# jmhb0/view_neti

Hardware: AMD Instinct MI355X
Metric: TI train steps/sec (SD-1.5 512^2 bs=4 per GPU) (higher is better)
Workload: dtype f16; 1 GPU; learnable_mode 0, sd15 shapes, 512x512 fp16, bs=4/GPU, grad_accum 1, full train step (VAE+16xCLIP+UNet fwd/bwd+AdamW); global_batch=4, parallelism=dp1, rccl_ranks=1, hipgraph=True

## Files before the change

### include/vneti.h

```cpp
#ifndef VNETI_H
#define VNETI_H
#include <stddef.h>
#include <stdint.h>

#ifdef __cplusplus
extern "C" {
#endif

#define VNETI_ABI_VERSION 1

int vneti_version(void);
int vneti_precision(void);
int vneti_last_error(char* buf, size_t n);

typedef struct vneti_gemm_desc {
  const void* A;
  const void* B;
  void* C;
  long long lda, ldb, ldc;
  int M, N, K;
  int batch;
  long long strideA, strideB, strideC;
  const float* bias;
  const void* rowadd;
  long long ld_rowadd;
  int rows_per_group;
  const void* resid;
  long long ldr;
  float alpha;
  int act;
  int out_f32;
  int conv_mode;
  int Hi, Wi, Ci, Ho, Wo, stride, pad_t, pad_l, ups;
  long long ldx;
  int tile_hint;
  void* workspace;
  long long workspace_bytes;
  int split_k;
  const void* gate_src;
  long long ld_gate;
  int gate_act;
  void* C2;
  long long ldc2;
  int act2;
  void* gn_sums;
  int gn_hw, gn_cpg, gn_groups, gn_slots;
  int geglu;
  int conv_korder;
} vneti_gemm_desc;

int vneti_gemm_f16(const vneti_gemm_desc* d, void* stream);
int vneti_gemm_select_tile(int M, int N, int batch);
int vneti_gemm_select_split(int M, int N, int K, int batch, int tile_hint, long long workspace_bytes);

int vneti_im2col3x3_small(const void* x, int x_is_f32, long long sb, long long sc, long long sy,
                          long long sx, void* out, int Bn, int C, int Hi, int Wi, int Ho, int Wo,
                          int stride, int pad_t, int pad_l, void* stream);

int vneti_conv3x3_in(const void* x, int x_is_f32, long long sb, long long sc, long long sy, long long sx,
                     const void* w_packed, const float* bias, void* out, long long ldo, int Bn, int C, int H, int W,
                     int Co, void* gn_sums, int gn_groups, int gn_slots, void* stream);

int vneti_transpose_f16(const void* in, long long ld_in, long long stride_in, void* out,
                        long long ld_out, long long stride_out, int rows, int cols, int batch,
                        void* stream);
#define VNETI_TRANSPOSE_MAX 4
typedef struct vneti_transpose_desc {
  const void* inp;
  long long ld_in, stride_in;
  void* out;
  long long ld_out, stride_out;
  int rows, cols, batch, _pad;
} vneti_transpose_desc;
int vneti_transpose_f16_multi(const vneti_transpose_desc* descs, int n, void* stream);

long long vneti_groupnorm_ws_floats(int Bn, int HW, int C, int G);
int vneti_groupnorm_fwd(const void* x, long long ldx, void* y, long long ldy, const float* gamma,
                        const float* beta, float* mean, float* rstd, float* ws, int Bn, int HW,
                        int C, int G, float eps, int silu, void* stream);
int vneti_groupnorm_fwd_sums(const void* x, long long ldx, void* y, long long ldy, const float* gamma,
                             const float* beta, const void* sums, int slots, float* mean, float* rstd,
                             int Bn, int HW, int C, int G, float eps, int silu, void* stream);
int vneti_groupnorm_fwd_2l(const void* x, long long ldx, void* y, long long ldy, const float* gamma,
                           const float* beta, void* sums, int slots, float* mean, float* rstd, int Bn, int HW,
                           int C, int G, float eps, int silu, void* stream);
int vneti_groupnorm_bwd_2l(const void* dy, long long lddy, const void* x, long long ldx, const float* gamma,
                           const float* beta, const float* mean, const float* rstd, void* dx, long long lddx,
                           const void* dx_accum, long long ldacc, void* sums, int slots, float* ws, int Bn,
                           int HW, int C, int G, int silu, void* stream);
int vneti_groupnorm_bwd(const void* dy, long long lddy, const void* x, long long ldx,
                        const float* gamma, const float* beta, const float* mean,
                        const float* rstd, void* dx, long long lddx, const void* dx_accum,
                        long long ldacc, float* ws, int Bn, int HW, int C, int G, int silu,
                        void* stream);

int vneti_layernorm_fwd(const void* x, int x_is_f32, long long ldx, void* y, long long ldy,
                        const float* gamma, const float* beta, float* mean, float* rstd, int rows,
                        int C, float eps, void* stream);
int vneti_layernorm_bwd(const void* dy, int dy_is_f32, long long lddy, const void* x,
                        int x_is_f32, long long ldx, const float* gamma, const float* mean,
                        const float* rstd, void* dx, int dx_is_f32, long long lddx,
                        const void* dx_accum, long long ldacc, void* dx_f16_copy, long long ldcopy,
                        int rows, int C, void* stream);

int vneti_attn_fwd(const void* Q, long long ldq, const void* K, long long ldk, const void* V,
                   long long ldv, void* O, long long ldo, float* lse, int Bn, int H, int Nq,
                   int Nk, int D, float scale, int causal, void* stream);
int vneti_attn_bwd_delta(const void* dO, long long lddo, const void* O, long long ldo,
                         float* delta, int Bn, int H, int Nq, int D, void* stream);
int vneti_attn_bwd_dq(const void* Q, long long ldq, const void* K, long long ldk, const void* V,
                      long long ldv, const void* dO, long long lddo, const float* lse, float* delta,
                      const void* O, long long ldo, void* dQ, long long lddq, int Bn, int H, int Nq,
                      int Nk, int D, float scale, int causal, void* stream);
int vneti_attn_bwd_dkv(const void* Q, long long ldq, const void* K, long long ldk, const void* V,
                       long long ldv, const void* dO, long long lddo, const float* lse,
                       const float* delta, void* dK, long long lddk, void* dV, long long lddv,
                       int Bn, int H, int Nq, int Nk, int D, float scale, int causal, float* ws,
                       long long ws_floats, void* stream);
int vneti_attn_bwd_small(const void* Q, long long ldq, const void* K, long long ldk, const void* V, long long ldv,
                         const void* dO, long long lddo, const void* O, long long ldo, const float* lse, void* dQ,
                         long long lddq, void* dK, long long lddk, void* dV, long long lddv, int Bn, int H, int N, int D,
                         float scale, int causal, void* stream);
int vneti_softmax_rows_f16(void* x, long long ld, int rows, int cols, void* stream);

int vneti_add_f16(const void* a, long long lda, const void* b, long long ldb, void* out,
                  long long ldo, int rows, int cols, void* stream);
int vneti_geglu_fwd(const void* p, long long ldp, void* out, long long ldo, int rows, int C4,
                    void* stream);
int vneti_geglu_bwd(const void* dy, long long lddy, const void* p, long long ldp, void* dp,
                    long long lddp, int rows, int C4, void* stream);
int vneti_act_fwd_f16(const void* x, void* y, long long n, int act, void* stream);
int vneti_act_bwd_f16(const void* dy, const void* x, void* dx, long long n, int act, void* stream);
int vneti_timestep_embedding(const void* t, void* out, int Bn, int dim, void* stream);
int vneti_sum2x2_f16(const void* in, long long ldi, void* out, long long ldo, int Bn, int H, int W,
                     int C, void* stream);
int vneti_rng_fill_normal(void* out_f32, long long n, const void* state, unsigned stream_id,
                          void* stream);
int vneti_rng_fill_randint(void* out_i64, int n, int high, const void* state, unsigned stream_id,
                           void* stream);
int vneti_rng_advance(void* state, void* stream);
int vneti_nested_dropout_mask(float* mask, int nl, int Bn, int hidden, float prob, const void* state,
                              unsigned stream_id, void* stream);
int vneti_sample_add_noise(const void* moments, long long ldm, const float* eps,
                           const float* noise, const void* timesteps_i64,
                           const float* alphas_cumprod, float scaling, int v_prediction,
                           float* latents, float* noisy, float* target, int Bn, int Lc, int HW,
                           void* stream);
int vneti_latent_sample(const void* moments, long long ldm, const float* eps, float scaling, float* latents, int Bn,
                        int Lc, int HW, void* stream);
int vneti_add_noise(const float* latents, const float* noise, const void* timesteps_i64, const float* alphas_cumprod,
                    int v_prediction, float* noisy, float* target, int Bn, int Lc, int HW, void* stream);
int vneti_cfg_sampler_step(const void* pred, long long ldp, float* x, float* m_prev, float* x_in, int Bn,
                           int Lc, int HW, float guidance, float alpha_t, float sigma_t, float cx,
                           float c0, float c1, int v_prediction, void* stream);
int vneti_cfg_sampler_step_table(const void* pred, long long ldp, float* x, float* m_prev, float* x_in,
                                 int Bn, int Lc, int HW, float guidance, const float* coef_table,
                                 const int* step, int v_prediction, void* stream);
int vneti_cfg_sampler_step_noise(const void* pred, long long ldp, float* x, float* m_prev, float* x_in,
                                 const float* noise, int Bn, int Lc, int HW, float guidance, float alpha_t,
                                 float sigma_t, float cx, float c0, float c1, float cn, int v_prediction, void* stream);
int vneti_cfg_sampler_step_noise_table(const void* pred, long long ldp, float* x, float* m_prev, float* x_in, int Bn,
                                       int Lc, int HW, float guidance, const float* coef_table,
                                       const float* noise_table, const int* step, int v_prediction, void* stream);
int vneti_table_fill_i64(void* dst_i64, int n, const void* table_i64, const int* step, void* stream);
int vneti_counter_advance(int* counter, void* stream);
int vneti_conv1x1_nchw_f32(const float* x, const float* W, const float* bias, float* out, int Bn, int Ci,
                           int Co, int HW, float in_scale, void* stream);
int vneti_image_postprocess(const void* img, long long ldi, float* out, long long n_pix, int channels,
                            void* stream);
int vneti_mse_loss_grad(const void* pred, long long ldp, const float* target, void* dpred,
                        long long lddp, float* loss_sum, const float* loss_scale, int Bn, int Lc,
                        int HW, void* stream);
#define VNETI_OPT_CHECK 1
#define VNETI_OPT_APPLY 2
#define VNETI_OPT_FINISH 4
#define VNETI_OPT_ALL 7
int vneti_adamw_flat(float* p, const float* g, float* m, float* v, long long n, const float* hyper,
                     float* scaler, int* step, int growth_interval, int phases, void* stream);
int vneti_adamw_segments(float* p, const float* g, float* m, float* v, long long seg_len, int n_seg,
                         int* seg_step, const int* active, int n_active, const float* hyper,
                         float* scaler, int* step, int growth_interval, int phases, void* stream);

long long vneti_mapper_num_params(int enc_dim, int hidden, int D, int has_bypass);
long long vneti_mapper_save_floats(int R, int enc_dim, int hidden);
long long vneti_mapper_rowgrad_floats(int R, int hidden, int D, int has_bypass);
int vneti_mapper_fwd(const float* params, const int* slot, long long slot_stride, const float* data,
                     int nfeat, const float* w_enc,
                     const float* hidden_mask, float norm_scale, float* word, float* bypass,
                     float* save, int R, int enc_dim, int hidden, int D, int has_bypass, const float* enc_in,
                     void* stream);
int vneti_mapper_fwd_slots(const float* params, const int* slots, long long slot_stride, int Bn, const float* data,
                           int nfeat, const float* w_enc, const float* hidden_mask, float norm_scale, float* word,
                           float* bypass, float* save, int R, int enc_dim, int hidden, int D, int has_bypass,
                           const float* enc_in, void* stream);
int vneti_mapper_bwd(const float* params, const int* slot, long long slot_stride,
                     const float* hidden_mask, float norm_scale,
                     const float* word, const float* dword_src, const int* dword_rows,
                     long long ld_src, const float* dbypass, const float* save, float* rowgrads,
                     float* grads, int accumulate, int R, int enc_dim, int hidden, int D,
                     int has_bypass, float* denc, void* stream);
long long vneti_mapper_legacy_input_params(int enc_dim, int pe_dim);
int vneti_mapper_legacy_input_fwd(const float* params_in, const int* slot, long long slot_stride,
                                  const void* timesteps_i64, const float* w_pe, float* enc_out, int nl, int Bn,
                                  int enc_dim, int pe_dim, void* stream);
int vneti_mapper_legacy_input_fwd_slots(const float* params_in, const int* slots, long long slot_stride,
                                        const void* timesteps_i64, const float* w_pe, float* enc_out, int nl, int Bn,
                                        int enc_dim, int pe_dim, void* stream);
int vneti_mapper_legacy_input_bwd(const void* timesteps_i64, const float* w_pe, const float* denc, float* grads_in,
                                  const int* slot, long long slot_stride, int accumulate, int nl, int Bn, int enc_dim,
                                  int pe_dim, void* stream);
int vneti_text_embed(const float* tok_emb, const float* pos_emb, const void* ids_i64,
                     const int* pos_obj, const float* word_obj, const int* pos_view,
                     const float* word_view, float* X, int nl, int Bn, int L, int D, void* stream);
int vneti_text_final_fwd(const float* last, const float* gamma, const float* beta, float eps,
                         const int* pos_obj, const float* bypass_obj, float alpha_obj,
                         int unconstrained_obj, const int* pos_view, const float* bypass_view,
                         float alpha_view, int unconstrained_view, float* norm_terms, void* ctx_k,
                         void* ctx_v, int nl, int Bn, int L, int D, void* stream);
int vneti_text_final_bwd(const float* last, const float* gamma, float eps, const int* pos_obj,
                         const float* bypass_obj, float alpha_obj, int unconstrained_obj,
                         float* dbypass_obj, const int* pos_view, const float* bypass_view,
                         float alpha_view, int unconstrained_view, float* dbypass_view,
                         const float* norm_terms, const void* dctx_k, const void* dctx_v, float* dX,
                         int nl, int Bn, int L, int D, void* stream);
int vneti_mapper_inputs(const void* timesteps_i64, const float* view_params, int nv, float* data,
                        int nl, int Bn, void* stream);
int vneti_cast_f32_f16(const float* x, void* y, long long n, void* stream);


int vneti_img_resample_ksize(int in_size, int out_size, int filter);
int vneti_img_resample_coeffs(int in_size, int out_size, int filter, int* bounds, int* kk, void* stream);
int vneti_img_resample_pass(const void* in, int in_w, void* out, int out_h, int out_w, const int* bounds,
                            const int* kk, int ksize, int horizontal, void* stream);
int vneti_img_crop(const void* in, int in_w, int top, int left, void* out, int h, int w, int flip, void* stream);
int vneti_img_enhance(void* img, int h, int w, int mode, float alpha, void* scratch8, void* stream);
int vneti_img_hue(void* img, int h, int w, int shift, void* stream);
int vneti_img_blur5(const void* in, void* out, float* tmp, int h, int w, const float* k5_host, void* stream);
int vneti_img_affine_nearest(const void* in, void* out, int h, int w, const int* a6_host, int fill, void* stream);
int vneti_img_to_f32_chw(const void* img, float* out, int h, int w, void* stream);

int vneti_comm_unique_id(void* id128);
int vneti_comm_init(const void* id128, int rank, int world, void** comm);
// ... 20 lines not shown
```

### view_neti_amd/csrc/gemm8.hip

```cpp
#include <type_traits>

#include "common.h"
#include "gemm_args.h"

namespace {

constexpr int BM = 256, NT = 512;
constexpr int HALF_BYTES = 128 * 128;
constexpr int GN_IMG = 5;

#define VN_WAIT_VM(n) asm volatile("s_waitcnt vmcnt(" #n ")" ::: "memory")
#define VN_WAIT_LGKM0() asm volatile("s_waitcnt lgkmcnt(0)" ::: "memory")

template <int BN, int EPI, bool CONV, bool HALO = false>
__global__ __launch_bounds__(NT) void gemm8_kernel(GemmArgs g) {
  static_assert(BN == 256 || BN == 128, "tile width");
  static_assert(!HALO || (BN == 128 && CONV), "the halo-patch loop exists for the 256x128 convolution tile");
  constexpr int PATCH_STRIDE = 41 * 1024;
  constexpr bool H42 = HALO && BN == 128;
  constexpr int NJB = BN / 128;
  constexpr int HB_BYTES = (BN / 2) * 128;
  constexpr int HB_DMA = BN / 128;
  constexpr int NBUF = BN == 256 ? 2 : 3;
  constexpr int BUF_BYTES = 2 * HALF_BYTES + 2 * HB_BYTES;
  constexpr int CS_LD = BN + 8;
  constexpr int CS_BYTES = BM * CS_LD * 2;
  constexpr int LOOP_BYTES = HALO ? 2 * PATCH_STRIDE + 3 * 2 * HB_BYTES : NBUF * BUF_BYTES;
  constexpr int LDS_BYTES = CS_BYTES > LOOP_BYTES ? CS_BYTES : LOOP_BYTES;
  constexpr int GN_NG = BN / 4 + 2;
  const half_t* const e_gate = EPI == 2 ? g.gate_src : nullptr;
  half_t* const e_C2 = EPI == 2 ? g.C2 : nullptr;
  const int e_geglu = EPI == 2 ? g.geglu : 0;
  const int e_act = EPI == 2 ? g.act : 0;
  float* const e_gn_sums = EPI >= 1 ? g.gn_sums : nullptr;
  const half_t* const e_rowadd = EPI >= 1 ? g.rowadd : nullptr;
  const int e_conv = CONV ? g.conv_mode : 0;
  constexpr int GN_BYTES = EPI == 0 ? 0 : GN_IMG * GN_NG * 4 * 8;
  __shared__ __attribute__((aligned(16))) char smem[LDS_BYTES + GN_BYTES];

  const int tid = threadIdx.x;
  const int lane = tid & 63;
  const int wave = __builtin_amdgcn_readfirstlane(tid >> 6);
  const int wr = wave >> 2, wc = wave & 3;

  int nblk = g.tiles_m * g.tiles_n;
  int bid = blockIdx.x;
  {
    int q = nblk >> 3, r = nblk & 7, xcd = bid & 7, idx = bid >> 3;
    bid = (xcd < r ? xcd * (q + 1) : r * (q + 1) + (xcd - r) * q) + idx;
  }
  const int tile_m = bid / g.tiles_n;
  const int tile_n = bid - tile_m * g.tiles_n;
  const int m0 = tile_m * BM;
  const int n0 = tile_n * BN;
  const int bz = blockIdx.y;
  const int kz = blockIdx.z;
  int hb = 0, hty = 0, htx = 0, row0 = m0;
  if constexpr (HALO) {
    const int tpr = g.Wo >> 4, tpi = (g.Ho >> 4) * tpr;
    hb = tile_m / tpi;
    const int rem = tile_m - hb * tpi;
    hty = rem / tpr;
    htx = rem - hty * tpr;
    row0 = (hb * g.Ho + hty * 16) * g.Wo + htx * 16;
  }
  auto rowmem = [&](const int r) { return HALO ? row0 + (r >> 4) * g.Wo + (r & 15) : m0 + r; };

  const half_t* Ab = g.A + (long long)bz * g.strideA;
  const half_t* Bb = g.B + (long long)bz * g.strideB;
  const __amdgpu_buffer_rsrc_t rsA = vn_make_rsrc(Ab, g.a_bytes);
  const __amdgpu_buffer_rsrc_t rsB = vn_make_rsrc(Bb, g.b_bytes);

  const int lrow = tid >> 3;
  const int gchunk = (tid & 7) ^ ((lrow >> 1) & 7);
  const float rcp_hw = CONV ? 1.0f / (float)(g.Ho * g.Wo) : 0.f, rcp_wo = CONV ? 1.0f / (float)g.Wo : 0.f;
  int a_base[4];
  uint32_t a_mask[4];
#pragma unroll
  for (int r = 0; r < (HALO ? 0 : 4); ++r) {
    const int m = m0 + (r >> 1) * 128 + (r & 1) * 64 + lrow;
    const bool ok = m < g.M;
    if constexpr (!CONV) {
      a_base[r] = (int)((long long)m * g.lda * 2) + gchunk * 16;
      a_mask[r] = ok ? 1u : 0u;
    } else {
      const int hw = g.Ho * g.Wo;
      int b = (int)((float)m * rcp_hw);
      int rem = m - b * hw;
      if (rem < 0) { b -= 1; rem += hw; } else if (rem >= hw) { b += 1; rem -= hw; }
      int oy = (int)((float)rem * rcp_wo);
      int ox = rem - oy * g.Wo;
      if (ox < 0) { oy -= 1; ox += g.Wo; } else if (ox >= g.Wo) { oy += 1; ox -= g.Wo; }
      const int py = e_conv == 1 ? oy * g.stride - g.pad_t : oy + g.pad_t;
      const int px = e_conv == 1 ? ox * g.stride - g.pad_l : ox + g.pad_l;
      a_base[r] = ((b * g.Hi + py) * g.Wi + px) * g.ldx2 + gchunk * 16;
      const int sgn = e_conv == 1 ? 1 : -1;
      uint32_t colbits = 0, mask = 0;
#pragma unroll
      for (int d = 0; d < 3; ++d) colbits |= ((unsigned)(px + sgn * d) < (unsigned)g.Wi ? 1u : 0u) << d;
#pragma unroll
      for (int d = 0; d < 3; ++d) mask |= ((unsigned)(py + sgn * d) < (unsigned)g.Hi ? colbits : 0u) << (3 * d);
      a_mask[r] = ok ? mask : 0u;
    }
  }
  uint32_t b_base[4];
#pragma unroll
  for (int r = 0; r < 4; ++r) {
    const int n = n0 + (r >> 1) * (BN / 2) + (r & 1) * 64 + lrow;
    b_base[r] = (n < g.N) ? (uint32_t)((long long)n * g.ldb * 2) + gchunk * 16 : VN_OOB;
  }

  const int nk_total = g.K / 64;
  const int kt_begin = kz * g.kt_per_split;
  const int kt_end = min(nk_total, kt_begin + g.kt_per_split);
  const int T = kt_end - kt_begin;

  int a_kt[2] = {kt_begin, kt_begin}, b_kt[2] = {kt_begin, kt_begin};
  int a_tap[2], a_ci0[2];
  {
    int tap = 0, ci0 = 0;
    if constexpr (CONV) {
      if (g.korder) {
        ci0 = (kt_begin / 9) * 64;
        tap = kt_begin - (kt_begin / 9) * 9;
      } else {
        tap = (kt_begin * 64) / g.Ci;
        ci0 = kt_begin * 64 - tap * g.Ci;
      }
    }
    a_tap[0] = a_tap[1] = tap;
    a_ci0[0] = a_ci0[1] = ci0;
  }
  const int tap_step = (e_conv == 2 ? -1 : 1) * g.ldx2;
  uint32_t nxt[4];
  auto prepA = [&](const int h) {
    const bool live = a_kt[h] < kt_end;
    int soff;
    uint32_t tapbit;
    if constexpr (!CONV) {
      soff = a_kt[h] * 128;
      tapbit = live ? 1u : 0u;
    } else {
      const int tap = a_tap[h];
      const int dy = (tap * 11) >> 5;
      const int dx = tap - 3 * dy;
      soff = (dy * g.Wi + dx) * tap_step + a_ci0[h] * 2;
      tapbit = live ? (1u << tap) : 0u;
      if (g.korder) {
        a_tap[h] += 1;
        if (a_tap[h] == 9) {
          a_tap[h] = 0;
          a_ci0[h] += 64;
        }
      } else {
        a_ci0[h] += 64;
        if (a_ci0[h] == g.Ci) {
          a_ci0[h] = 0;
          a_tap[h] += 1;
        }
      }
    }
#pragma unroll
    for (int j = 0; j < 2; ++j) {
      nxt[j] = (a_mask[2 * h + j] & tapbit) ? (uint32_t)(a_base[2 * h + j] + soff) : VN_OOB;
    }
    a_kt[h] += 1;
  };
  auto prepB = [&](const int h) {
    const bool live = b_kt[h] < kt_end;
    const uint32_t soff = (uint32_t)b_kt[h] * 128u, dead = live ? 0u : VN_OOB;
    if constexpr (BN == 256) {
#pragma unroll
      for (int j = 0; j < 2; ++j) nxt[j] = (b_base[2 * h + j] + soff) | dead;
    } else {
      nxt[2 + h] = (b_base[2 * h] + soff) | dead;
    }
    b_kt[h] += 1;
  };
  auto issueA = [&](const int h, const int buf) {
    char* dst = smem + buf * BUF_BYTES + h * HALF_BYTES + wave * 1024;
#pragma unroll
    for (int j = 0; j < 2; ++j)
      dma16(rsA, dst + j * 8192, nxt[j]);
  };
  auto issueB = [&](const int h, const int buf) {
    char* dst = smem + buf * BUF_BYTES + 2 * HALF_BYTES + h * HB_BYTES + wave * 1024;
    if constexpr (BN == 256) {
#pragma unroll
// ... 254 lines not shown
    issueB(0, 1);
    prepA(0);
    issueA(0, 1);
    prepB(1);
    issueB(1, 1);
    prepA(1);
    VN_WAIT_VM(10);
    __builtin_amdgcn_s_barrier();
    __builtin_amdgcn_sched_barrier(0);
    readB0(0);
    VN_WAIT_LGKM0();
    __builtin_amdgcn_sched_barrier(0);
    if (wr == 1) __builtin_amdgcn_s_barrier();
    __builtin_amdgcn_sched_barrier(0);

    int cur = 0;
    for (int t = 0; t < T; ++t) {
      readA(0);
      issueA(1, cur ^ 1);
      VN_PHASE_SYNC();
      VN_MMA(0, 0, bf0, prepB(0));
      VN_PHASE_END();
      readB1();
      issueB(0, cur);
      VN_PHASE_SYNC();
      VN_MMA(0, 1, bf1, prepA(0));
      VN_PHASE_END();
      readA(1);
      issueA(0, cur);
      VN_PHASE_SYNC();
      VN_MMA(1, 0, bf0, prepB(1));
      VN_PHASE_END();
      readB0(BUF_BYTES);
      issueB(1, cur);
      VN_PHASE_SYNC();
      VN_MMA(1, 1, bf1, prepA(1));
      VN_PHASE_END();
      cur ^= 1;
#pragma unroll
      for (int s = 0; s < 2; ++s) {
        rdA[s] ^= BUF_BYTES;
        rdB[s] ^= BUF_BYTES;
      }
    }
  } else {
#pragma unroll
    for (int t0 = 0; t0 < 2; ++t0) {
      prepA(0);
      prepB(0);
      prepB(1);
      issueA(0, t0);
      issueB(0, t0);
      issueB(1, t0);
      prepA(1);
      issueA(1, t0);
    }
    prepA(0);
    prepB(0);
    prepB(1);
    VN_WAIT_VM(8);
    __builtin_amdgcn_s_barrier();
    __builtin_amdgcn_sched_barrier(0);
    if (wr == 1) __builtin_amdgcn_s_barrier();
    __builtin_amdgcn_sched_barrier(0);
    int stg = 2;
    for (int t = 0; t < T; ++t) {
      readB0(0);
      readB1();
      readA(0);
      issueA(0, stg);
      issueB(0, stg);
      issueB(1, stg);
      VN_SYNC(10);
      VN_MMA2(0, prepA(1));
      VN_PHASE_END();
      readA(1);
      issueA(1, stg);
      VN_SYNC(8);
      VN_MMA2(1, (prepA(0), prepB(0), prepB(1)));
      VN_PHASE_END();
      stg = stg == 2 ? 0 : stg + 1;
#pragma unroll
      for (int s = 0; s < 2; ++s) {
        rdA[s] = rdA[s] >= 2 * BUF_BYTES ? rdA[s] - 2 * BUF_BYTES : rdA[s] + BUF_BYTES;
        rdB[s] = rdB[s] >= 2 * BUF_BYTES ? rdB[s] - 2 * BUF_BYTES : rdB[s] + BUF_BYTES;
      }
    }
#undef VN_MMA2
#undef VN_SYNC
  }
  if (wr == 0) __builtin_amdgcn_s_barrier();
  asm volatile("s_waitcnt vmcnt(0) lgkmcnt(0)" ::: "memory");
  __syncthreads();
#undef VN_MMA
#undef VN_PHASE_SYNC
#undef VN_PHASE_END

  if (g.ksplit > 1) {
    float* ws = g.ws + ((long long)(kz * g.batch + bz) * g.M) * g.N;
    const __amdgpu_buffer_rsrc_t rsW = vn_make_rsrc(ws, 0x7fffffffu);
#pragma unroll
    for (int h = 0; h < 2; ++h)
#pragma unroll
      for (int j = 0; j < 2; ++j)
#pragma unroll
        for (int i = 0; i < 4; ++i)
#pragma unroll
          for (int jb = 0; jb < NJB; ++jb) {
            const int m = rowmem(acc_row(h, i));
            const int n = n0 + acc_col(h, j, jb);
            if (m < g.M && n < g.N) {
              float* p = ws + (long long)m * g.N + n;
              if (n + 4 <= g.N && (g.N & 3) == 0) {
                vn_st16_wt(rsW, (uint32_t)(((long long)m * g.N + n) * 4), acc[h][j][i][jb]);
              } else {
                for (int e = 0; e < 4 && n + e < g.N; ++e) p[e] = acc[h][j][i][jb][e];
              }
            }
          }
    return;
  }

  if (e_gn_sums && !(HALO && g.gn_hw == g.Ho * g.Wo)) {
    vn_u64* gacc = reinterpret_cast<vn_u64*>(smem + LDS_BYTES);
    for (int i = tid; i < GN_IMG * GN_NG * 4; i += NT) gacc[i] = 0;
  }
  {
    const int nsw = ((frow >> 3) & 1) << 2;
#pragma unroll
    for (int h = 0; h < 2; ++h)
#pragma unroll
      for (int i = 0; i < 4; ++i)
#pragma unroll
        for (int j = 0; j < 2; ++j)
#pragma unroll
          for (int jb = 0; jb < NJB; ++jb) {
            const int ml = acc_row(h, i);
            const int nl = acc_col(h, j, jb) ^ nsw;
            half4 o;
#pragma unroll
            for (int e = 0; e < 4; ++e)
              o[e] = (half_t)apply_act(acc[h][j][i][jb][e] * g.alpha + bv[H42 ? h : 0][j][jb][e], e_act);
            *reinterpret_cast<half4*>(smem + ((size_t)ml * CS_LD + nl) * 2) = o;
          }
  }
  __syncthreads();

  half_t* Cb = reinterpret_cast<half_t*>(g.C) + (long long)bz * g.strideC;
  const __amdgpu_buffer_rsrc_t rsC = vn_make_rsrc(Cb, 0x7fffffffu);
  const __amdgpu_buffer_rsrc_t rsC2 = vn_make_rsrc(e_C2, e_C2 ? 0x7fffffffu : 0u);
  const half_t* Rb = reinterpret_cast<const half_t*>(g.resid);
  if (Rb) Rb += (long long)bz * g.strideC;
  constexpr int CPR = BN / 8;
  constexpr int U = EPI == 2 ? 2 : (EPI == 1 ? 4 : (BN == 256 ? 8 : 4));
  static_assert(NT % CPR == 0 && CPR <= 32 && (BM * CPR) % NT == 0, "a thread keeps one 8-column chunk over all its rows");
  vn_u64* gacc = reinterpret_cast<vn_u64*>(smem + LDS_BYTES);
  const bool gn = e_gn_sums != nullptr;
  const float rcp_gnhw = gn ? 1.0f / (float)g.gn_hw : 0.f, rcp_rpg = e_rowadd ? 1.0f / (float)g.rows_per_group : 0.f;
  const int gn_img0 = gn ? row0 / g.gn_hw : 0, gn_g0t = gn ? n0 / g.gn_cpg : 0;
  const int c = (tid % CPR) * 8;
  const int n = n0 + c;
  const int gn_glo = gn ? n / g.gn_cpg : 0;
  const int gn_split = gn ? (gn_glo + 1) * g.gn_cpg - n : 8;
  int gn_img = -1;
  float s_lo = 0.f, q_lo = 0.f, s_hi = 0.f, q_hi = 0.f;
  auto gn_flush = [&]() {
    const int iref = __builtin_amdgcn_readfirstlane(gn_img);
    const bool uni = __all(gn_img == iref) && iref >= 0;
    if (uni) {
#pragma unroll
      for (int off = 32; off >= CPR; off >>= 1) {
        s_lo += __shfl_xor(s_lo, off);
        q_lo += __shfl_xor(q_lo, off);
        s_hi += __shfl_xor(s_hi, off);
        q_hi += __shfl_xor(q_hi, off);
      }
    }
    if (gn_img >= 0 && (!uni || lane < CPR)) {
      vn_u64* a = gacc + ((gn_img - gn_img0) * GN_NG + (gn_glo - gn_g0t)) * 4;
      vn_fx_add2(a, s_lo, q_lo);
      if (gn_split < 8) vn_fx_add2(a + 4, s_hi, q_hi);
    }
    s_lo = q_lo = s_hi = q_hi = 0.f;
  };
  const bool full_chunk = n + 8 <= g.N;
  const bool swap_halves = ((tid / CPR) >> 3) & 1;
  const __amdgpu_buffer_rsrc_t rsR = vn_make_rsrc(Rb, Rb ? 0x7fffffffu : 0u);
  const __amdgpu_buffer_rsrc_t rsRA = vn_make_rsrc(e_rowadd, e_rowadd ? 0x7fffffffu : 0u);
  const __amdgpu_buffer_rsrc_t rsG = vn_make_rsrc(e_gate, e_gate ? 0x7fffffffu : 0u);
  const int r_first = tid / CPR;
  constexpr int RPP = NT / CPR;
  const bool gn_one = HALO && gn && g.gn_hw == g.Ho * g.Wo;
  const bool ra_one = HALO && EPI >= 1 && e_rowadd && g.rows_per_group == g.Ho * g.Wo;
  half8 av_tile = half8{0, 0, 0, 0, 0, 0, 0, 0};
  if (ra_one) av_tile = as_half8(vn_buf_load16(rsRA, full_chunk ? (uint32_t)(((long long)hb * g.ld_rowadd + n) * 2) : VN_OOB));
  if (gn_one) gn_img = hb;
  for (int it0 = 0; it0 < BM / RPP; it0 += U) {
    half8 cv[U], rv[U], av[U], gv[U], gv2[U];
#pragma unroll
    for (int u = 0; u < U; ++u) {
      const int r = r_first + RPP * (it0 + u);
      const int m = rowmem(r);
      const bool ok = m < g.M && full_chunk;
      u32x4 t = *reinterpret_cast<const u32x4*>(smem + ((size_t)r * CS_LD + c) * 2);
      if (swap_halves) t = u32x4{t[2], t[3], t[0], t[1]};
      cv[u] = as_half8(t);
      if (Rb) rv[u] = as_half8(vn_buf_load16(rsR, ok ? (uint32_t)(((long long)m * g.ldr + n) * 2) : VN_OOB));
      if (EPI >= 1) {
        if (ra_one) {
          av[u] = av_tile;
        } else if (e_rowadd) {
          int grp = (int)((float)m * rcp_rpg);
          const int rem = m - grp * g.rows_per_group;
          grp += rem >= g.rows_per_group ? 1 : (rem < 0 ? -1 : 0);
          av[u] = as_half8(vn_buf_load16(rsRA, ok ? (uint32_t)(((long long)grp * g.ld_rowadd + n) * 2) : VN_OOB));
        }
      }
      if (EPI == 2 && e_gate) {
        const long long go = (long long)m * g.ld_gate + (e_geglu == 2 ? 2 * n : n);
        gv[u] = as_half8(vn_buf_load16_once(rsG, ok ? (uint32_t)(go * 2) : VN_OOB));
        gv2[u] = as_half8(vn_buf_load16_once(rsG, (ok && e_geglu == 2) ? (uint32_t)(go * 2 + 16) : VN_OOB));
      }
    }
#pragma unroll
    for (int u = 0; u < U; ++u) {
      const int r = r_first + RPP * (it0 + u);
      const int m = rowmem(r);
      const bool valid = m < g.M && n < g.N;
      if (gn && !gn_one) {
        int img = gn_img;
        if (valid) {
          img = (int)((float)m * rcp_gnhw);
          const int rem = m - img * g.gn_hw;
          img += rem >= g.gn_hw ? 1 : (rem < 0 ? -1 : 0);
        }
        if (__any(img != gn_img)) {
          gn_flush();
          gn_img = img;
        }
      }
      if (!valid) continue;
      half8 v = cv[u];
      if (full_chunk) {
        if (EPI >= 1 && e_rowadd) {
          v = vn_add8(v, av[u]);
        }
        if (Rb) {
          v = vn_add8(v, rv[u]);
        }
        if (e_geglu == 2) {
#pragma unroll
          for (int c2 = 0; c2 < 2; ++c2) {
            const half8 pre = c2 == 0 ? gv[u] : gv2[u];
            half8 o;
#pragma unroll
            for (int e = 0; e < 4; ++e) {
              const float d = (float)v[4 * c2 + e], hh = (float)pre[e], gg = (float)pre[4 + e];
              float cdf, xpdf;
              vn_gelu_parts(gg, cdf, xpdf);
              o[e] = (half_t)(d * gg * cdf);
              o[4 + e] = (half_t)(d * hh * (cdf + xpdf));
            }
            vn_st16_wt(rsC, (uint32_t)(((long long)m * g.ldc + 2 * n + 8 * c2) * 2), o);
          }
          continue;
        }
        if (e_gate) {
#pragma unroll
          for (int e = 0; e < 8; ++e) v[e] = (half_t)((float)v[e] * act_grad((float)gv[u][e], g.gate_act));
        }
        if (e_geglu == 1 || (e_C2 && e_geglu == 0)) vn_st16_wt_saved(rsC, (uint32_t)(((long long)m * g.ldc + n) * 2), v);
        else vn_st16_wt(rsC, (uint32_t)(((long long)m * g.ldc + n) * 2), v);
        if (e_geglu == 1) {
          half4 o2;
#pragma unroll
          for (int e = 0; e < 4; ++e) o2[e] = (half_t)((float)v[e] * vn_gelu_erf((float)v[4 + e]));
          *reinterpret_cast<half4*>(e_C2 + (long long)m * g.ldc2 + (n >> 1)) = o2;
        }
        if (gn) {
          {
            const half2v one2 = {(half_t)1.f, (half_t)1.f};
#pragma unroll
            for (int e = 0; e < 8; e += 2) {
              const half2v p2 = {v[e], v[e + 1]};
              if (e < gn_split) {
                s_lo = VN_FDOT2(p2, one2, s_lo);
                q_lo = VN_FDOT2(p2, p2, q_lo);
              } else {
                s_hi = VN_FDOT2(p2, one2, s_hi);
                q_hi = VN_FDOT2(p2, p2, q_hi);
              }
            }
          }
        }
        if (e_C2 && e_geglu == 0) {
          half8 o2;
#pragma unroll
          for (int e = 0; e < 8; ++e) o2[e] = (half_t)apply_act((float)v[e], g.act2);
          vn_st16_wt(rsC2, (uint32_t)(((long long)m * g.ldc2 + n) * 2), o2);
        }
      } else {
        const half_t* radd = e_rowadd ? e_rowadd + (long long)(m / g.rows_per_group) * g.ld_rowadd + n : nullptr;
        for (int e = 0; e < 8 && n + e < g.N; ++e) {
          float x = (float)v[e];
          if (radd) x = (float)(half_t)(x + (float)radd[e]);
          if (Rb) x = (float)(half_t)(x + (float)Rb[(long long)m * g.ldr + n + e]);
          if (e_gate) x = (float)(half_t)(x * act_grad((float)e_gate[(long long)m * g.ld_gate + n + e], g.gate_act));
          Cb[(long long)m * g.ldc + n + e] = (half_t)x;
          if (e_C2) e_C2[(long long)m * g.ldc2 + n + e] = (half_t)apply_act((float)(half_t)x, g.act2);
          if (gn) {
            const float xs = (float)(half_t)x;
            if (e < gn_split) {
              s_lo += xs;
              q_lo += xs * xs;
            } else {
              s_hi += xs;
              q_hi += xs * xs;
            }
          }
        }
      }
    }
  }
  if (gn_one) {
    float v4[4] = {s_lo, q_lo, s_hi, q_hi};
#pragma unroll
    for (int k = 0; k < 4; ++k) {
      v4[k] += __shfl_xor(v4[k], 32);
      v4[k] += __shfl_xor(v4[k], 16);
    }
    static_assert(CPR == 16 || !HALO, "the halo tile is 128 columns wide");
    float* tab = reinterpret_cast<float*>(smem + LDS_BYTES);
    if (lane < 16) *reinterpret_cast<f32x4*>(tab + (wave * 16 + lane) * 4) = f32x4{v4[0], v4[1], v4[2], v4[3]};
    __syncthreads();
    if (tid < 32) {
      const int col = tid >> 1, half = tid & 1;
      float sv = 0.f, qv = 0.f;
#pragma unroll
      for (int w8 = 0; w8 < 8; ++w8) {
        sv += tab[(w8 * 16 + col) * 4 + 2 * half];
        qv += tab[(w8 * 16 + col) * 4 + 2 * half + 1];
      }
      const int nc = n0 + col * 8;
      const int glo = nc / g.gn_cpg;
      const int split = (glo + 1) * g.gn_cpg - nc;
      if (nc < g.N && (half == 0 || split < 8)) {
        const int slot = tile_m % g.gn_slots;
        vn_u64* dst = reinterpret_cast<vn_u64*>(e_gn_sums) + (((long long)hb * g.gn_slots + slot) * g.gn_G + glo + half) * 4;
        vn_fx_add2(dst, sv, qv);
      }
    }
  } else if (gn) {
    gn_flush();
    __syncthreads();
    const int slot = tile_m % g.gn_slots;
    for (int i = tid; i < GN_IMG * GN_NG; i += NT) {
      const vn_u64* src = gacc + 4 * i;
      if ((src[0] | src[1] | src[2] | src[3]) == 0) continue;
      const int img = gn_img0 + i / GN_NG, grp = gn_g0t + i % GN_NG;
      vn_u64* dst = reinterpret_cast<vn_u64*>(e_gn_sums) + (((long long)img * g.gn_slots + slot) * g.gn_G + grp) * 4;
#pragma unroll
      for (int w = 0; w < 4; ++w) atomicAdd(dst + w, src[w]);
    }
  }
}

inline int epilogue_level8(const GemmArgs& g) {
  if (g.gate_src || g.C2 || g.geglu || g.act) return 2;
  return (g.gn_sums || g.rowadd) ? 1 : 0;
}

}

int vneti_launch_gemm8(void* gemm_args, int bn, int halo, hipStream_t st) {
  GemmArgs& g = *reinterpret_cast<GemmArgs*>(gemm_args);
  if (g.out_f32 || (g.conv_mode && (g.ups || (g.conv_mode == 2 && g.stride == 2))) ||
      (g.M >= (1 << 24) && (g.conv_mode || g.rowadd || g.gn_sums)))
    return VNETI_EUNSUP;
  if (halo && (bn != 128 || g.conv_mode < 1 || g.conv_mode > 2 || g.stride != 1 || g.pad_t != 1 || g.pad_l != 1 || g.Hi != g.Ho ||
               g.Wi != g.Wo || (g.Ho & 15) || (g.Wo & 15) || (g.Ci & 63) || g.K != 9 * g.Ci || !g.korder ||
               g.batch != 1 || g.M != (g.M / (g.Ho * g.Wo)) * g.Ho * g.Wo))
    return VNETI_EUNSUP;
  if (halo && g.ksplit > 1) {
    const int nchunk = g.Ci / 64, cps = cdiv(nchunk, g.ksplit);
    g.kt_per_split = 9 * cps;
    g.ksplit = cdiv(nchunk, cps);
  }
  g.tiles_m = cdiv(g.M, BM);
  g.tiles_n = cdiv(g.N, bn);
  const dim3 grid(g.tiles_m * g.tiles_n, g.batch, g.ksplit), block(NT);
  const int epi = epilogue_level8(g);
#define VN_GO(E, C)                                                                        \
  do {                                                                                     \
    if (bn == 256) hipLaunchKernelGGL((gemm8_kernel<256, E, C>), grid, block, 0, st, g);   \
    else hipLaunchKernelGGL((gemm8_kernel<128, E, C>), grid, block, 0, st, g);             \
  } while (0)
#define VN_GO_HALO(E) hipLaunchKernelGGL((gemm8_kernel<128, E, true, true>), grid, block, 0, st, g)
  if (halo) {
    if (epi == 2) VN_GO_HALO(2); else if (epi == 1) VN_GO_HALO(1); else VN_GO_HALO(0);
  } else if (g.conv_mode) {
    if (epi == 2) VN_GO(2, true); else if (epi == 1) VN_GO(1, true); else VN_GO(0, true);
  } else {
    if (epi == 2) VN_GO(2, false); else if (epi == 1) VN_GO(1, false); else VN_GO(0, false);
  }
#undef VN_GO
#undef VN_GO_HALO
  return vneti_check_launch("gemm8_kernel");
}
```

### view_neti_amd/csrc/gemm_args.h

```cpp
#pragma once
#include "common.h"

namespace {

struct GemmArgs {
  const half_t* A;
  const half_t* B;
  void* C;
  const float* bias;
  const half_t* rowadd;
  const void* resid;
  float* ws;
  const half_t* gate_src;
  half_t* C2;
  long long ld_gate, ldc2;
  int gate_act, act2;
  float* gn_sums;
  int gn_hw, gn_cpg, gn_G, gn_slots;
  int geglu;
  long long lda, ldb, ldc, ld_rowadd, ldr;
  long long strideA, strideB, strideC;
  uint32_t a_bytes, b_bytes;
  int M, N, K;
  int rows_per_group;
  float alpha;
  int act;
  int out_f32;
  int batch, ksplit, kt_per_split;
  int conv_mode;
  int Hi, Wi, Ci, Ho, Wo, stride, pad_t, pad_l, ups;
  int ldx2;
  int korder;
  int tiles_m, tiles_n;
};

__device__ __forceinline__ float apply_act(float v, int act) {
  switch (act) {
    case 1: return vn_silu(v);
    case 2: return vn_quick_gelu(v);
    case 3: return vn_gelu_erf(v);
    default: return v;
  }
}
__device__ __forceinline__ float act_grad(float f, int act) {
  if (act == 2) {
    float s = vn_sigmoid(1.702f * f);
    return s * (1.f + 1.702f * f * (1.f - s));
  } else if (act == 3) {
    return vn_gelu_erf_grad(f);
  }
  float s = vn_sigmoid(f);
  return s * (1.f + f * (1.f - s));
}

__device__ __forceinline__ int lds_off(int row, int chunk) {
  return row * 128 + ((chunk ^ ((row >> 1) & 7)) << 4);
}

__device__ __forceinline__ void dma16(__amdgpu_buffer_rsrc_t rs, char* lds_dst, uint32_t off) {
#if defined(__HIP_DEVICE_COMPILE__)
  __builtin_amdgcn_raw_ptr_buffer_load_lds(rs, (__attribute__((address_space(3))) void*)lds_dst, 16, off, 0, 0, 0);
#else
  (void)rs; (void)lds_dst; (void)off;
#endif
}

}

int vneti_launch_gemm8(void* gemm_args, int bn, int halo, hipStream_t st);
```

### view_neti_amd/csrc/gemm_conv.hip

```cpp
#include "common.h"
#include "gemm_args.h"
#include "../../include/vneti.h"

namespace {

template <int BM, int BN, int WM, int WN, bool F32OUT, bool DMA, int NSTG = 2, int EPI = 2, bool CONV = true>
__global__ __launch_bounds__((BM / WM) * (BN / WN) * 64) void gemm_kernel(
    const half_t* pA, const half_t* pB, uint32_t p_a_bytes, uint32_t p_b_bytes, int p_lda, int p_ldb, int pM, int pN, int pK,
    int p_tiles_m, int p_tiles_n, int p_split_conv , const GemmArgs gfull) {
  GemmArgs g = gfull;
  g.A = pA;
  g.B = pB;
  g.a_bytes = p_a_bytes;
  g.b_bytes = p_b_bytes;
  g.lda = p_lda;
  g.ldb = p_ldb;
  g.M = pM;
  g.N = pN;
  g.K = pK;
  g.tiles_m = p_tiles_m;
  g.tiles_n = p_tiles_n;
  g.kt_per_split = p_split_conv & 0xffff;
  g.ksplit = (p_split_conv >> 16) & 0xff;
  g.conv_mode = p_split_conv >> 24;
  static_assert(NSTG == 2 || ((NSTG == 3 || NSTG == 4) && DMA), "the LDS rings are LDS-DMA only");
  const half_t* const e_gate = EPI == 2 ? g.gate_src : nullptr;
  half_t* const e_C2 = EPI == 2 ? g.C2 : nullptr;
  const int e_geglu = EPI == 2 ? g.geglu : 0;
  const int e_act = EPI == 2 ? g.act : 0;
  float* const e_gn_sums = EPI >= 1 ? g.gn_sums : nullptr;
  const half_t* const e_rowadd = EPI >= 1 ? g.rowadd : nullptr;
  const int e_conv = CONV ? g.conv_mode : 0;
  constexpr int NWM = BM / WM, NWN = BN / WN;
  constexpr int NT = NWM * NWN * 64;
  constexpr int RSTEP = NT / 8;
  constexpr int A_IT = BM / RSTEP, B_IT = BN / RSTEP;
  constexpr int STAGE_BYTES = (BM + BN) * 128;
  constexpr int CS_LD = F32OUT ? (BN + 4) : (BN + 8);
  constexpr int CS_BYTES = BM * CS_LD * (F32OUT ? 4 : 2);
  constexpr int LDS_BYTES = (NSTG * STAGE_BYTES > CS_BYTES) ? NSTG * STAGE_BYTES : CS_BYTES;
  constexpr int GN_IMG = 5, GN_NG = BN / 4 + 2;
  constexpr int GN_BYTES = (F32OUT || EPI == 0) ? 0 : GN_IMG * GN_NG * 4 * 8;
  __shared__ __attribute__((aligned(16))) char smem[LDS_BYTES + GN_BYTES];

  const int tid = threadIdx.x;
  const int lane = tid & 63;
  const int wave = __builtin_amdgcn_readfirstlane(tid >> 6);
  const int wm0 = (wave / NWN) * WM;
  const int wn0 = (wave % NWN) * WN;

  int nblk = g.tiles_m * g.tiles_n;
  int bid = blockIdx.x;
  {
    int q = nblk >> 3, r = nblk & 7, xcd = bid & 7, idx = bid >> 3;
    bid = (xcd < r ? xcd * (q + 1) : r * (q + 1) + (xcd - r) * q) + idx;
  }
  const int tile_m = bid / g.tiles_n;
  const int tile_n = bid - tile_m * g.tiles_n;
  const int m0 = tile_m * BM;
  const int n0 = tile_n * BN;
  const int bz = blockIdx.y;
  const int kz = blockIdx.z;

  const half_t* Ab = g.A + (long long)bz * g.strideA;
  const half_t* Bb = g.B + (long long)bz * g.strideB;
  __amdgpu_buffer_rsrc_t rsA = vn_make_rsrc(Ab, g.a_bytes);
  __amdgpu_buffer_rsrc_t rsB = vn_make_rsrc(Bb, g.b_bytes);

  const int lrow = tid >> 3;
  const int gchunk = DMA ? ((tid & 7) ^ ((lrow >> 1) & 7)) : (tid & 7);

  const float rcp_hw = CONV ? __builtin_amdgcn_rcpf((float)(g.Ho * g.Wo)) : 0.f, rcp_wo = CONV ? __builtin_amdgcn_rcpf((float)g.Wo) : 0.f;
  int a_off[A_IT];
  int a_py[A_IT], a_px[A_IT], a_bh[A_IT];
#pragma unroll
  for (int i = 0; i < A_IT; ++i) {
    int m = m0 + lrow + RSTEP * i;
    bool ok = m < g.M;
    if (e_conv == 0) {
      a_off[i] = ok ? (int)((long long)m * g.lda * 2) + gchunk * 16 : -1;
      a_py[i] = a_px[i] = a_bh[i] = 0;
    } else {
      int rem, ox;
      const int b = vn_divmod(m, g.Ho * g.Wo, rcp_hw, rem);
      const int oy = vn_divmod(rem, g.Wo, rcp_wo, ox);
      a_bh[i] = ok ? b * g.Hi : -1;
      if (e_conv == 1) {
        a_py[i] = oy * g.stride - g.pad_t;
        a_px[i] = ox * g.stride - g.pad_l;
      } else {
        a_py[i] = oy + g.pad_t;
        a_px[i] = ox + g.pad_l;
      }
      a_off[i] = ((b * g.Hi + a_py[i]) * g.Wi + a_px[i]) * g.ldx2 + gchunk * 16;
    }
  }
  int b_off[B_IT];
#pragma unroll
  for (int i = 0; i < B_IT; ++i) {
    int n = n0 + lrow + RSTEP * i;
    b_off[i] = (n < g.N) ? (int)((long long)n * g.ldb * 2) + gchunk * 16 : -1;
  }

  u32x4 ra[DMA ? 1 : A_IT], rb[DMA ? 1 : B_IT];

  auto a_offset = [&](int i, int k0, int dy, int dx, int tapoff) -> uint32_t {
    if (e_conv == 0) return a_off[i] < 0 ? VN_OOB : (uint32_t)(a_off[i] + k0 * 2);
    bool ok = a_bh[i] >= 0;
    if (e_conv == 1 && !g.ups) {
      int iy = a_py[i] + dy, ix = a_px[i] + dx;
      ok = ok && (unsigned)iy < (unsigned)g.Hi && (unsigned)ix < (unsigned)g.Wi;
      return ok ? (uint32_t)(a_off[i] + tapoff) : VN_OOB;
    }
    int iy, ix;
    if (e_conv == 1) {
      iy = a_py[i] + dy;
      ix = a_px[i] + dx;
      ok = ok && (unsigned)iy < (unsigned)(2 * g.Hi) && (unsigned)ix < (unsigned)(2 * g.Wi);
      iy >>= 1;
      ix >>= 1;
    } else {
      int ty = a_py[i] - dy, tx = a_px[i] - dx;
      ok = ok && ty >= 0 && tx >= 0;
      if (g.stride == 2) {
        ok = ok && ((ty | tx) & 1) == 0;
        ty >>= 1;
        tx >>= 1;
      }
      iy = ty;
      ix = tx;
      ok = ok && iy < g.Hi && ix < g.Wi;
    }
    return ok ? (uint32_t)(((a_bh[i] + iy) * g.Wi + ix) * g.ldx2 + tapoff) : VN_OOB;
  };

  uint32_t a_cur[A_IT], b_cur[B_IT];
#pragma unroll
  for (int i = 0; i < B_IT; ++i) b_cur[i] = b_off[i] < 0 ? VN_OOB : (uint32_t)b_off[i];

  auto issue = [&](int kt, int stage, bool first) {
    const int k0 = kt * 64;
    bool recompute = first;
    int dy = 0, dx = 0, tapoff = 0;
    if (e_conv != 0) {
      int tap, ci0;
      if (g.korder) {
        const int chunk = kt / 9;
        tap = kt - chunk * 9;
        ci0 = chunk << 6;
        recompute = true;
      } else {
        tap = k0 / g.Ci;
        ci0 = k0 - tap * g.Ci;
        recompute = recompute || ci0 == 0;
      }
      if (recompute) {
        dy = tap / 3;
        dx = tap - dy * 3;
        tapoff = (e_conv == 1 && !g.ups) ? ((dy * g.Wi + dx) * g.ldx2 + ci0 * 2) : (ci0 * 2 + gchunk * 16);
      }
    }
    if (recompute) {
#pragma unroll
      for (int i = 0; i < A_IT; ++i) a_cur[i] = a_offset(i, k0, dy, dx, tapoff);
      if (first) {
#pragma unroll
        for (int i = 0; i < B_IT; ++i) b_cur[i] += (uint32_t)k0 * 2;
      }
    }
    if constexpr (DMA) {
      char* As = smem + stage * STAGE_BYTES;
      char* Bs = As + BM * 128;
#pragma unroll
      for (int i = 0; i < A_IT; ++i) dma16(rsA, As + (wave * 8 + RSTEP * i) * 128, a_cur[i]);
#pragma unroll
      for (int i = 0; i < B_IT; ++i) dma16(rsB, Bs + (wave * 8 + RSTEP * i) * 128, b_cur[i]);
    } else {
#pragma unroll
      for (int i = 0; i < A_IT; ++i) ra[i] = vn_buf_load16(rsA, a_cur[i]);
#pragma unroll
      for (int i = 0; i < B_IT; ++i) rb[i] = vn_buf_load16(rsB, b_cur[i]);
    }
#pragma unroll
    for (int i = 0; i < A_IT; ++i) a_cur[i] += 128;
// ... 73 lines not shown
    for (int kt = kt_begin; kt < kt_end; ++kt) {
      const int st_next = st == 2 ? 0 : st + 1;
      const int st_new = st_next == 2 ? 0 : st_next + 1;
      if (kt + 2 < kt_end) issue(kt + 2, st_new, false);
      load_frags(1, st, 1);
      mma(0);
      if (kt + 2 < kt_end) asm volatile("s_waitcnt vmcnt(%0) lgkmcnt(0)" ::"n"(PER) : "memory");
      else asm volatile("s_waitcnt vmcnt(0) lgkmcnt(0)" ::: "memory");
      __builtin_amdgcn_s_barrier();
      if (kt + 1 < kt_end) load_frags(0, st_next, 0);
      mma(1);
      st = st_next;
    }
    __syncthreads();
  } else if constexpr (NSTG == 4) {
    constexpr int PER = A_IT + B_IT;
    auto wait_landed = [&](int later) {
      if (later >= 2) asm volatile("s_waitcnt vmcnt(%0) lgkmcnt(0)" ::"n"(2 * PER) : "memory");
      else if (later == 1) asm volatile("s_waitcnt vmcnt(%0) lgkmcnt(0)" ::"n"(PER) : "memory");
      else asm volatile("s_waitcnt vmcnt(0) lgkmcnt(0)" ::: "memory");
    };
    issue(kt_begin, 0, true);
    if (kt_begin + 1 < kt_end) issue(kt_begin + 1, 1, false);
    if (kt_begin + 2 < kt_end) issue(kt_begin + 2, 2, false);
    wait_landed(kt_end - kt_begin - 1);
    __builtin_amdgcn_s_barrier();
    load_frags(0, 0, 0);
    int st = 0;
    for (int kt = kt_begin; kt < kt_end; ++kt) {
      const int st_next = (st + 1) & 3;
      if (kt + 3 < kt_end) issue(kt + 3, (st + 3) & 3, false);
      load_frags(1, st, 1);
      mma(0);
      wait_landed(kt_end - kt - 2);
      __builtin_amdgcn_s_barrier();
      if (kt + 1 < kt_end) load_frags(0, st_next, 0);
      mma(1);
      st = st_next;
    }
    __syncthreads();
  } else {
    issue(kt_begin, 0, true);
    store_lds(0);
    if constexpr (DMA) asm volatile("s_waitcnt vmcnt(0)" ::: "memory");
    __syncthreads();

    for (int kt = kt_begin; kt < kt_end; ++kt) {
      const int cur = (kt - kt_begin) & 1;
      if (kt + 1 < kt_end) issue(kt + 1, cur ^ 1, false);
      load_frags(0, cur, 0);
      load_frags(1, cur, 1);
      mma(0);
      mma(1);
      if (kt + 1 < kt_end) store_lds(cur ^ 1);
      if constexpr (DMA) asm volatile("s_waitcnt vmcnt(0)" ::: "memory");
      __syncthreads();
    }
  }

  if (g.ksplit > 1) {
    float* ws = g.ws + ((long long)(kz * g.batch + bz) * g.M) * g.N;
    const __amdgpu_buffer_rsrc_t rsW = vn_make_rsrc(ws, 0x7fffffffu);
#pragma unroll
    for (int i = 0; i < MI16; ++i)
#pragma unroll
      for (int j = 0; j < NI16; ++j) {
        const int m = m0 + wm0 + i * 16 + frow;
        const int n = n0 + wn0 + j * 16 + 4 * fq;
        if (m < g.M && n < g.N) {
          float* p = ws + (long long)m * g.N + n;
          if (n + 4 <= g.N && (g.N & 3) == 0) {
            vn_st16_wt(rsW, (uint32_t)(((long long)m * g.N + n) * 4), acc[i][j]);
          } else {
            for (int e = 0; e < 4 && n + e < g.N; ++e) p[e] = acc[i][j][e];
          }
        }
      }
    return;
  }

  if constexpr (!F32OUT) {
    if (e_gn_sums) {
      vn_u64* gacc = reinterpret_cast<vn_u64*>(smem + LDS_BYTES);
      for (int i = tid; i < GN_IMG * GN_NG * 4; i += NT) gacc[i] = 0;
    }
  }
  if constexpr (!BIAS_EARLY) load_bias();
#pragma unroll
  for (int i = 0; i < MI16; ++i) {
#pragma unroll
    for (int j = 0; j < NI16; ++j) {
      const int ml = wm0 + i * 16 + frow;
      const int nl = wn0 + j * 16 + 4 * fq;
      float v[4];
#pragma unroll
      for (int e = 0; e < 4; ++e) {
        float x = acc[i][j][e] * g.alpha + bv[j][e];
        v[e] = apply_act(x, e_act);
      }
      if constexpr (F32OUT) {
        f32x4 o = {v[0], v[1], v[2], v[3]};
        *reinterpret_cast<f32x4*>(smem + ((size_t)ml * CS_LD + nl) * 4) = o;
      } else {
        half4 o = {(half_t)v[0], (half_t)v[1], (half_t)v[2], (half_t)v[3]};
        *reinterpret_cast<half4*>(smem + ((size_t)ml * CS_LD + nl) * 2) = o;
      }
    }
  }
  __syncthreads();

  if constexpr (F32OUT) {
    float* Cb = reinterpret_cast<float*>(g.C) + (long long)bz * g.strideC;
    const __amdgpu_buffer_rsrc_t rsC = vn_make_rsrc(Cb, 0x7fffffffu);
    const float* Rb = reinterpret_cast<const float*>(g.resid);
    if (Rb) Rb += (long long)bz * g.strideC;
    constexpr int CPR = BN / 4;
    for (int idx = tid; idx < BM * CPR; idx += NT) {
      int r = idx / CPR, c = (idx - r * CPR) * 4;
      int m = m0 + r, n = n0 + c;
      if (m >= g.M || n >= g.N) continue;
      f32x4 v = *reinterpret_cast<const f32x4*>(smem + ((size_t)r * CS_LD + c) * 4);
      if (n + 4 <= g.N) {
        if (Rb) {
          f32x4 rr = *reinterpret_cast<const f32x4*>(Rb + (long long)m * g.ldr + n);
          v += rr;
        }
        vn_st16_wt(rsC, (uint32_t)(((long long)m * g.ldc + n) * 4), v);
      } else {
        for (int e = 0; e < 4 && n + e < g.N; ++e) {
          float x = v[e];
          if (Rb) x += Rb[(long long)m * g.ldr + n + e];
          Cb[(long long)m * g.ldc + n + e] = x;
        }
      }
    }
  } else {
    half_t* Cb = reinterpret_cast<half_t*>(g.C) + (long long)bz * g.strideC;
    const __amdgpu_buffer_rsrc_t rsC = vn_make_rsrc(Cb, 0x7fffffffu);
    const __amdgpu_buffer_rsrc_t rsC2 = vn_make_rsrc(e_C2, e_C2 ? 0x7fffffffu : 0u);
    const half_t* Rb = reinterpret_cast<const half_t*>(g.resid);
    if (Rb) Rb += (long long)bz * g.strideC;
    constexpr int CPR = BN / 8;
    static_assert(NT % CPR == 0 && CPR <= 32 && (BM * CPR) % NT == 0, "a thread keeps one 8-column chunk over all its rows");
    vn_u64* gacc = reinterpret_cast<vn_u64*>(smem + LDS_BYTES);
    const bool gn = e_gn_sums != nullptr;
    const float rcp_gnhw = gn ? __builtin_amdgcn_rcpf((float)g.gn_hw) : 0.f;
    const float rcp_rpg = e_rowadd ? __builtin_amdgcn_rcpf((float)g.rows_per_group) : 0.f;
    const int gn_img0 = gn ? m0 / g.gn_hw : 0, gn_g0t = gn ? n0 / g.gn_cpg : 0;
    const int gn_c = n0 + (tid % CPR) * 8;
    const int gn_glo = gn ? gn_c / g.gn_cpg : 0;
    const int gn_split = gn ? (gn_glo + 1) * g.gn_cpg - gn_c : 8;
    int gn_img = -1;
    float s_lo = 0.f, q_lo = 0.f, s_hi = 0.f, q_hi = 0.f;
    auto gn_flush = [&]() {
      const int iref = __builtin_amdgcn_readfirstlane(gn_img);
      const bool uni = __all(gn_img == iref) && iref >= 0;
      if (uni) {
#pragma unroll
        for (int off = 32; off >= CPR; off >>= 1) {
          s_lo += __shfl_xor(s_lo, off);
          q_lo += __shfl_xor(q_lo, off);
          s_hi += __shfl_xor(s_hi, off);
          q_hi += __shfl_xor(q_hi, off);
        }
      }
      if (gn_img >= 0 && (!uni || lane < CPR)) {
        vn_u64* a = gacc + ((gn_img - gn_img0) * GN_NG + (gn_glo - gn_g0t)) * 4;
        vn_fx_add2(a, s_lo, q_lo);
        if (gn_split < 8) vn_fx_add2(a + 4, s_hi, q_hi);
      }
      s_lo = q_lo = s_hi = q_hi = 0.f;
    };
    for (int idx = tid; idx < BM * CPR; idx += NT) {
      int r = idx / CPR, c = (idx - r * CPR) * 8;
      int m = m0 + r, n = n0 + c;
      const bool valid = m < g.M && n < g.N;
      if (gn) {
        int gn_rem;
        const int img = valid ? vn_divmod(m, g.gn_hw, rcp_gnhw, gn_rem) : gn_img;
        if (__any(img != gn_img)) {
          gn_flush();
          gn_img = img;
        }
      }
      if (!valid) continue;
      half8 v = as_half8(*reinterpret_cast<const u32x4*>(smem + ((size_t)r * CS_LD + c) * 2));
      int ra_rem;
      const half_t* radd = e_rowadd ? e_rowadd + (long long)vn_divmod(m, g.rows_per_group, rcp_rpg, ra_rem) * g.ld_rowadd + n : nullptr;
      if (n + 8 <= g.N) {
        if (radd) {
          half8 t = *reinterpret_cast<const half8*>(radd);
          v = vn_add8(v, t);
        }
        if (Rb) {
          half8 rr = *reinterpret_cast<const half8*>(Rb + (long long)m * g.ldr + n);
          v = vn_add8(v, rr);
        }
        if (e_geglu == 2) {
          const half_t* pp = e_gate + (long long)m * g.ld_gate + 2 * n;
#pragma unroll
          for (int c2 = 0; c2 < 2; ++c2) {
            const half8 pre = *reinterpret_cast<const half8*>(pp + 8 * c2);
            half8 o;
#pragma unroll
            for (int e = 0; e < 4; ++e) {
              const float d = (float)v[4 * c2 + e], hh = (float)pre[e], gg = (float)pre[4 + e];
              float cdf, xpdf;
              vn_gelu_parts(gg, cdf, xpdf);
              o[e] = (half_t)(d * gg * cdf);
              o[4 + e] = (half_t)(d * hh * (cdf + xpdf));
            }
            vn_st16_wt(rsC, (uint32_t)(((long long)m * g.ldc + 2 * n + 8 * c2) * 2), o);
          }
          continue;
        }
        if (e_gate) {
          half8 pre = *reinterpret_cast<const half8*>(e_gate + (long long)m * g.ld_gate + n);
#pragma unroll
          for (int e = 0; e < 8; ++e) v[e] = (half_t)((float)v[e] * act_grad((float)pre[e], g.gate_act));
        }
        if (e_geglu == 1 || (e_C2 && e_geglu == 0)) vn_st16_wt_saved(rsC, (uint32_t)(((long long)m * g.ldc + n) * 2), v);
        else vn_st16_wt(rsC, (uint32_t)(((long long)m * g.ldc + n) * 2), v);
        if (e_geglu == 1) {
          half4 o2;
#pragma unroll
          for (int e = 0; e < 4; ++e) o2[e] = (half_t)((float)v[e] * vn_gelu_erf((float)v[4 + e]));
          *reinterpret_cast<half4*>(e_C2 + (long long)m * g.ldc2 + (n >> 1)) = o2;
        }
        if (gn) {
#pragma unroll
          for (int e = 0; e < 8; ++e) {
            const float x = (float)v[e];
            if (e < gn_split) {
              s_lo += x;
              q_lo += x * x;
            } else {
              s_hi += x;
              q_hi += x * x;
            }
          }
        }
        if (e_C2 && e_geglu == 0) {
          half8 o2;
#pragma unroll
          for (int e = 0; e < 8; ++e) o2[e] = (half_t)apply_act((float)v[e], g.act2);
          vn_st16_wt(rsC2, (uint32_t)(((long long)m * g.ldc2 + n) * 2), o2);
        }
      } else {
        for (int e = 0; e < 8 && n + e < g.N; ++e) {
          float x = (float)v[e];
          if (radd) x = (float)(half_t)(x + (float)radd[e]);
          if (Rb) x = (float)(half_t)(x + (float)Rb[(long long)m * g.ldr + n + e]);
          if (e_gate) x = (float)(half_t)(x * act_grad((float)e_gate[(long long)m * g.ld_gate + n + e], g.gate_act));
          Cb[(long long)m * g.ldc + n + e] = (half_t)x;
          if (e_C2) e_C2[(long long)m * g.ldc2 + n + e] = (half_t)apply_act((float)(half_t)x, g.act2);
          if (gn) {
            const float xs = (float)(half_t)x;
            if (e < gn_split) {
              s_lo += xs;
              q_lo += xs * xs;
            } else {
              s_hi += xs;
              q_hi += xs * xs;
            }
          }
        }
      }
    }
    if (gn) {
      gn_flush();
      __syncthreads();
      const int slot = tile_m % g.gn_slots;
      for (int i = tid; i < GN_IMG * GN_NG; i += NT) {
        const vn_u64* src = gacc + 4 * i;
        if ((src[0] | src[1] | src[2] | src[3]) == 0) continue;
        const int img = gn_img0 + i / GN_NG, grp = gn_g0t + i % GN_NG;
        vn_u64* dst = reinterpret_cast<vn_u64*>(e_gn_sums) + (((long long)img * g.gn_slots + slot) * g.gn_G + grp) * 4;
#pragma unroll
        for (int w = 0; w < 4; ++w) atomicAdd(dst + w, src[w]);
      }
    }
  }
}

__global__ __launch_bounds__(256) void splitk_reduce_kernel(
    float* p_ws, void* pC, const float* p_bias, const void* p_resid, const half_t* p_rowadd, int pM, int pN, int p_batch,
    int p_ksplit, int p_ldc, int p_ldr, const GemmArgs gfull) {
  GemmArgs g = gfull;
  g.ws = p_ws;
  g.C = pC;
  g.bias = p_bias;
  g.resid = p_resid;
  g.rowadd = p_rowadd;
  g.M = pM;
  g.N = pN;
  g.batch = p_batch;
  g.ksplit = p_ksplit;
  g.ldc = p_ldc;
  g.ldr = p_ldr;
  const unsigned n4 = (unsigned)(g.N + 3) / 4;
  const unsigned gid = blockIdx.x * 256u + threadIdx.x;
  const unsigned total = (unsigned)g.batch * (unsigned)g.M * n4;
  if (gid >= total) return;
  const unsigned row = gid / n4;
  const int c = (int)(gid - row * n4) * 4;
  const int bz = g.batch > 1 ? (int)(row / (unsigned)g.M) : 0;
  const int m = (int)(row - (unsigned)bz * (unsigned)g.M);
  const int ne = min(4, g.N - c);
  const long long zstride = (long long)g.batch * g.M * g.N;
  const float* p0 = g.ws + ((long long)bz * g.M + m) * g.N + c;
  if ((g.N & 3) == 0 && ((g.ldc | g.ldr | g.ld_rowadd | g.ld_gate | g.ldc2) & 3) == 0) {
    const long long co = (long long)bz * g.strideC + (long long)m * g.ldc + c;
    const long long ro = (long long)bz * g.strideC + (long long)m * g.ldr + c;
    f32x4 bv = {0.f, 0.f, 0.f, 0.f}, rf = {0.f, 0.f, 0.f, 0.f};
    half4 rh = {0, 0, 0, 0}, ra = {0, 0, 0, 0}, gt = {0, 0, 0, 0};
    if (g.bias) bv = *reinterpret_cast<const f32x4*>(g.bias + c);
    if (g.resid) {
      if (g.out_f32) rf = *reinterpret_cast<const f32x4*>(reinterpret_cast<const float*>(g.resid) + ro);
      else rh = *reinterpret_cast<const half4*>(reinterpret_cast<const half_t*>(g.resid) + ro);
    }
    if (g.rowadd) ra = *reinterpret_cast<const half4*>(g.rowadd + (long long)(m / g.rows_per_group) * g.ld_rowadd + c);
    if (g.gate_src) gt = *reinterpret_cast<const half4*>(g.gate_src + (long long)m * g.ld_gate + c);
    f32x4 v = {0.f, 0.f, 0.f, 0.f};
    int z = 0;
    for (; z + 4 <= g.ksplit; z += 4) {
      const f32x4 t0 = *reinterpret_cast<const f32x4*>(p0 + (z + 0) * zstride);
      const f32x4 t1 = *reinterpret_cast<const f32x4*>(p0 + (z + 1) * zstride);
      const f32x4 t2 = *reinterpret_cast<const f32x4*>(p0 + (z + 2) * zstride);
      const f32x4 t3 = *reinterpret_cast<const f32x4*>(p0 + (z + 3) * zstride);
      v += t0;
      v += t1;
      v += t2;
      v += t3;
    }
    for (; z < g.ksplit; ++z) v += *reinterpret_cast<const f32x4*>(p0 + z * zstride);
    float x[4];
#pragma unroll
    for (int e = 0; e < 4; ++e) {
      x[e] = v[e] * g.alpha;
      if (g.bias) x[e] += bv[e];
      x[e] = apply_act(x[e], g.act);
    }
    if (g.out_f32) {
      f32x4 o = {x[0], x[1], x[2], x[3]};
      if (g.resid) o += rf;
      vn_st16_wt(vn_make_rsrc(g.C, 0x7fffffffu), (uint32_t)(co * 4), o);
    } else {
      half4 o, o2;
#pragma unroll
      for (int e = 0; e < 4; ++e) {
        float y = (float)(half_t)x[e];
        if (g.rowadd) y = (float)(half_t)(y + (float)ra[e]);
        if (g.resid) y = (float)(half_t)(y + (float)rh[e]);
        if (g.gate_src) y = (float)(half_t)(y * act_grad((float)gt[e], g.gate_act));
        o[e] = (half_t)y;
        o2[e] = (half_t)apply_act((float)(half_t)y, g.act2);
      }
      *reinterpret_cast<half4*>(reinterpret_cast<half_t*>(g.C) + co) = o;
      if (g.C2) *reinterpret_cast<half4*>(g.C2 + (long long)m * g.ldc2 + c) = o2;
    }
    return;
  }
  float v[4] = {0.f, 0.f, 0.f, 0.f};
  for (int z = 0; z < g.ksplit; ++z) {
    const float* p = p0 + z * zstride;
    for (int e = 0; e < ne; ++e) v[e] += p[e];
  }
  for (int e = 0; e < ne; ++e) {
    float x = v[e] * g.alpha;
    if (g.bias) x += g.bias[c + e];
    x = apply_act(x, g.act);
    if (g.out_f32) {
      if (g.resid) x += reinterpret_cast<const float*>(g.resid)[(long long)bz * g.strideC + (long long)m * g.ldr + c + e];
      reinterpret_cast<float*>(g.C)[(long long)bz * g.strideC + (long long)m * g.ldc + c + e] = x;
    } else {
      x = (float)(half_t)x;
      if (g.rowadd) x = (float)(half_t)(x + (float)g.rowadd[(long long)(m / g.rows_per_group) * g.ld_rowadd + c + e]);
      if (g.resid)
        x = (float)(half_t)(x + (float)reinterpret_cast<const half_t*>(g.resid)[(long long)bz * g.strideC + (long long)m * g.ldr + c + e]);
      if (g.gate_src) x = (float)(half_t)(x * act_grad((float)g.gate_src[(long long)m * g.ld_gate + c + e], g.gate_act));
      reinterpret_cast<half_t*>(g.C)[(long long)bz * g.strideC + (long long)m * g.ldc + c + e] = (half_t)x;
      if (g.C2) g.C2[(long long)m * g.ldc2 + c + e] = (half_t)apply_act((float)(half_t)x, g.act2);
    }
  }
}

inline int epilogue_level(const GemmArgs& g) {
  if (g.gate_src || g.C2 || g.geglu || g.act) return 2;
  return (g.gn_sums || g.rowadd) ? 1 : 0;
}

template <int BM, int BN, int WM, int WN, bool F32OUT, bool DMA, int NSTG>
void launch_variant(const GemmArgs& g, dim3 grid, hipStream_t st) {
  const dim3 block((BM / WM) * (BN / WN) * 64);
#define VN_GO(E, C)                                                                                                        \
  hipLaunchKernelGGL((gemm_kernel<BM, BN, WM, WN, F32OUT, DMA, NSTG, E, C>), grid, block, 0, st, g.A, g.B, g.a_bytes, g.b_bytes, \
                     (int)g.lda, (int)g.ldb, g.M, g.N, g.K, g.tiles_m, g.tiles_n, g.kt_per_split | (g.ksplit << 16) | (g.conv_mode << 24), g)
  if constexpr (F32OUT) {
    if (g.conv_mode) { if (g.act) VN_GO(2, true); else VN_GO(0, true); }
    else { if (g.act) VN_GO(2, false); else VN_GO(0, false); }
  } else {
    const int epi = epilogue_level(g);
    if (g.conv_mode) { if (epi == 2) VN_GO(2, true); else if (epi == 1) VN_GO(1, true); else VN_GO(0, true); }
    else { if (epi == 2) VN_GO(2, false); else if (epi == 1) VN_GO(1, false); else VN_GO(0, false); }
  }
#undef VN_GO
}

inline void launch_reduce(const GemmArgs& g, hipStream_t st) {
  if (g.ksplit > 1) {
    long long total = (long long)g.batch * g.M * ((g.N + 3) / 4);
    hipLaunchKernelGGL(splitk_reduce_kernel, dim3((unsigned)cdivl(total, 256)), dim3(256), 0, st, g.ws, g.C, g.bias, g.resid,
                       g.rowadd, g.M, g.N, g.batch, g.ksplit, (int)g.ldc, (int)g.ldr, g);
  }
}

template <int BM, int BN, int WM, int WN, bool DMA>
int launch_cfg(GemmArgs& g, bool f32out, hipStream_t st) {
  g.tiles_m = cdiv(g.M, BM);
  g.tiles_n = cdiv(g.N, BN);
  dim3 grid(g.tiles_m * g.tiles_n, g.batch, g.ksplit);
  if (f32out) launch_variant<BM, BN, WM, WN, true, DMA, 2>(g, grid, st);
  else launch_variant<BM, BN, WM, WN, false, DMA, 2>(g, grid, st);
  launch_reduce(g, st);
  return vneti_check_launch("gemm_kernel");
}

template <int BM, int BN, int WM, int WN, int NSTG = 3>
int launch_cfg_ring(GemmArgs& g, bool f32out, hipStream_t st) {
  g.tiles_m = cdiv(g.M, BM);
  g.tiles_n = cdiv(g.N, BN);
  dim3 grid(g.tiles_m * g.tiles_n, g.batch, g.ksplit);
  if (f32out) launch_variant<BM, BN, WM, WN, true, true, NSTG>(g, grid, st);
  else launch_variant<BM, BN, WM, WN, false, true, NSTG>(g, grid, st);
  launch_reduce(g, st);
  return vneti_check_launch("gemm_kernel");
}

template <int BM, int BN, int WM, int WN, bool DMA>
int launch_cfg_f16(GemmArgs& g, hipStream_t st) {
  g.tiles_m = cdiv(g.M, BM);
  g.tiles_n = cdiv(g.N, BN);
  dim3 grid(g.tiles_m * g.tiles_n, g.batch, g.ksplit);
  launch_variant<BM, BN, WM, WN, false, DMA, 2>(g, grid, st);
  launch_reduce(g, st);
  return vneti_check_launch("gemm_kernel");
}

struct TileDims {
  int bm, bn;
};
constexpr int kMaxTile = 18;
constexpr TileDims kTiles[kMaxTile + 1] = {{0, 0},     {128, 128}, {128, 64},  {64, 64},  {256, 128}, {256, 256}, {256, 128}, {256, 128},
                                          {256, 128}, {128, 128}, {128, 128}, {128, 64},  {64, 64},   {128, 128}, {128, 64},  {64, 64},
                                          {256, 256}, {256, 128}, {256, 128}};

int select_tile(int M, int N, int batch) {
  long long t256 = (long long)cdiv(M, 256) * cdiv(N, 128) * batch;
  long long t128 = (long long)cdiv(M, 128) * cdiv(N, 128) * batch;
  long long t12864 = (long long)cdiv(M, 128) * cdiv(N, 64) * batch;
  if (N <= 64) return (M >= 2048) ? 2 : 3;
  (void)t256;
  if (t128 >= 384) return 1;
  if (t12864 >= 384) return 2;
  return 3;
}

int select_ksplit(int M, int N, int K, int batch, int tile, long long ws_floats) {
  if (ws_floats <= 0) return 1;
  const int nk = K / 64;
  long long tiles = (long long)cdiv(M, kTiles[tile].bm) * cdiv(N, kTiles[tile].bn) * batch;
  if (tiles >= 256 || nk < 16) return 1;
  int s = (int)(512 / tiles);
  if (s > nk / 8) s = nk / 8;
  if (s > 16) s = 16;
  while (s > 1 && (long long)s * batch * M * N > ws_floats) --s;
  return s < 2 ? 1 : s;
}

}

extern "C" int vneti_gemm_select_tile(int M, int N, int batch) { return select_tile(M, N, batch > 0 ? batch : 1); }

extern "C" int vneti_gemm_select_split(int M, int N, int K, int batch, int tile_hint, long long workspace_bytes) {
  if (batch <= 0) batch = 1;
  int cfg = tile_hint >= 100 ? tile_hint - 100 : tile_hint;
  if (cfg == 0) cfg = select_tile(M, N, batch);
  if (cfg < 1 || cfg > kMaxTile || K % 64 != 0) return -1;
  int ks = select_ksplit(M, N, K, batch, cfg, workspace_bytes / 4);
  const int nk = K / 64;
  if (ks > nk) ks = nk;
  if (ks < 1) ks = 1;
  return cdiv(nk, cdiv(nk, ks));
}

extern "C" int vneti_gemm_f16(const vneti_gemm_desc* d, void* stream) {
  VN_REQUIRE(d != nullptr, "gemm: null descriptor");
  VN_REQUIRE(d->A && d->B && d->C, "gemm: null operand pointer");
  VN_REQUIRE(d->M > 0 && d->N > 0 && d->K > 0, "gemm: bad shape M=%d N=%d K=%d", d->M, d->N, d->K);
  VN_REQUIRE(d->K % 64 == 0, "gemm: K=%d must be a multiple of 64", d->K);
  VN_REQUIRE(d->ldb % 8 == 0, "gemm: ldb=%lld must be a multiple of 8", d->ldb);
  int batch = d->batch > 0 ? d->batch : 1;
  GemmArgs g;
  memset(&g, 0, sizeof(g));
  g.A = (const half_t*)d->A;
  g.B = (const half_t*)d->B;
  g.C = d->C;
  g.bias = d->bias;
  g.rowadd = (const half_t*)d->rowadd;
  g.resid = d->resid;
  g.gate_src = (const half_t*)d->gate_src;
  g.ld_gate = d->ld_gate;
  g.gate_act = d->gate_act;
  g.C2 = (half_t*)d->C2;
  g.ldc2 = d->ldc2;
  g.act2 = d->act2;
  g.gn_sums = (float*)d->gn_sums;
  g.gn_hw = d->gn_hw;
  g.gn_cpg = d->gn_cpg;
  g.gn_G = d->gn_groups;
  g.gn_slots = d->gn_slots;
  g.geglu = d->geglu;
  g.lda = d->lda;
  g.ldb = d->ldb;
  g.ldc = d->ldc;
  g.ld_rowadd = d->ld_rowadd;
  g.ldr = d->ldr;
  g.strideA = d->strideA;
  g.strideB = d->strideB;
  g.strideC = d->strideC;
  g.M = d->M;
  g.N = d->N;
  g.K = d->K;
  g.batch = batch;
  g.rows_per_group = d->rows_per_group > 0 ? d->rows_per_group : 1;
  g.alpha = d->alpha;
  g.act = d->act;
  g.out_f32 = d->out_f32 ? 1 : 0;
  g.conv_mode = d->conv_mode;
  long long a_bytes;
  if (d->conv_mode == 0) {
    VN_REQUIRE(d->lda % 8 == 0, "gemm: lda=%lld must be a multiple of 8", d->lda);
    a_bytes = ((long long)(d->M - 1) * d->lda + d->K) * 2;
  } else {
    VN_REQUIRE(d->conv_mode == 1 || d->conv_mode == 2, "gemm: bad conv_mode %d", d->conv_mode);
    VN_REQUIRE(d->Ci > 0 && d->Ci % 64 == 0, "conv: Ci=%d must be a multiple of 64", d->Ci);
    VN_REQUIRE(d->K == 9 * d->Ci, "conv: K=%d must equal 9*Ci=%d", d->K, 9 * d->Ci);
    VN_REQUIRE(d->stride == 1 || d->stride == 2, "conv: stride %d unsupported", d->stride);
    VN_REQUIRE(d->Ho > 0 && d->Wo > 0 && d->M % (d->Ho * d->Wo) == 0, "conv: M=%d not a multiple of Ho*Wo", d->M);
    VN_REQUIRE(d->ldx % 8 == 0, "conv: ldx must be a multiple of 8");
    VN_REQUIRE(!(d->ups && d->conv_mode != 1), "conv: fused upsample only in forward gather mode");
    VN_REQUIRE(!(d->ups && d->stride != 1), "conv: fused upsample needs stride 1");
    g.Hi = d->Hi;
    g.Wi = d->Wi;
    g.Ci = d->Ci;
    g.Ho = d->Ho;
    g.Wo = d->Wo;
    g.stride = d->stride;
    g.pad_t = d->pad_t;
    g.pad_l = d->pad_l;
    g.ups = d->ups;
    g.ldx2 = (int)(d->ldx * 2);
    VN_REQUIRE(!d->conv_korder || d->Ci % 64 == 0, "conv: conv_korder=1 needs Ci=%d to be a multiple of 64", d->Ci);
    g.korder = d->conv_korder ? 1 : 0;
    long long nb = d->M / (d->Ho * d->Wo);
    a_bytes = nb * d->Hi * d->Wi * d->ldx * 2;
  }
  long long b_bytes = ((long long)(d->N - 1) * d->ldb + d->K) * 2;
  VN_REQUIRE(a_bytes < 0x7fffffffLL && b_bytes < 0x7fffffffLL, "gemm: operand larger than 2 GiB");
  g.a_bytes = (uint32_t)a_bytes;
  g.b_bytes = (uint32_t)b_bytes;
  if (!d->out_f32) {
    VN_REQUIRE(d->ldc % 8 == 0 || d->N < 8, "gemm: ldc=%lld must be a multiple of 8", d->ldc);
  }
  VN_REQUIRE_OUT("gemm C", vn_out_bytes(d->M, d->ldc, d->N, d->out_f32 ? 4 : 2, batch, d->strideC));
  if (d->C2) VN_REQUIRE_OUT("gemm C2", vn_out_bytes(d->M, d->ldc2, d->geglu == 1 ? d->N / 2 : d->N, 2));
  hipStream_t st = (hipStream_t)stream;
  bool f32 = d->out_f32 != 0;
  VN_REQUIRE(!(f32 && d->rowadd), "gemm: rowadd is only supported for f16 output");
  if (d->gate_src || d->C2) {
    VN_REQUIRE(!f32 && batch == 1, "gemm: gate/C2 epilogues need f16 output and batch 1");
    VN_REQUIRE(!d->gate_src || (d->gate_act >= 1 && d->gate_act <= 3 && d->ld_gate % 8 == 0), "gemm: bad gate arguments");
    VN_REQUIRE(!d->C2 || (d->act2 >= 0 && d->act2 <= 3 && d->ldc2 % 8 == 0), "gemm: bad C2 arguments");
  }

  if (d->geglu) {
    VN_REQUIRE(d->geglu == 1 || d->geglu == 2, "gemm: geglu must be 0, 1 or 2");
    VN_REQUIRE(!f32 && batch == 1 && d->N % 8 == 0, "gemm: geglu needs f16 output, batch 1 and N %% 8 == 0");
    VN_REQUIRE(d->split_k == 1, "gemm: geglu needs split_k = 1 (it lives in the fused epilogue)");
    VN_REQUIRE(!d->gn_sums, "gemm: geglu and gn_sums are exclusive");
    if (d->geglu == 1) {
      VN_REQUIRE(d->C2 && d->ldc2 % 4 == 0 && !d->gate_src, "gemm: geglu forward needs C2 ([M][N/2]) and no gate");
    } else {
      VN_REQUIRE(d->gate_src && d->ld_gate % 8 == 0 && !d->C2 && !d->resid && !d->rowadd,
                 "gemm: geglu backward needs gate_src ([M][2N] saved pre-activation) and a plain epilogue");
      VN_REQUIRE(d->ldc % 8 == 0, "gemm: geglu backward writes [M][2N]: ldc %% 8");
    }
  }
  if (d->gn_sums) {
    VN_REQUIRE(!f32 && batch == 1, "gemm: gn_sums needs f16 output and batch 1");
    VN_REQUIRE(d->gn_hw >= 64 && d->gn_cpg >= 4 && d->gn_groups > 0 && d->gn_slots > 0 && d->N == d->gn_cpg * d->gn_groups &&
                   d->M % d->gn_hw == 0 && (d->gn_cpg >= 8 || d->gn_cpg == 4),
               "gemm: bad gn_sums geometry hw=%d cpg=%d G=%d", d->gn_hw, d->gn_cpg, d->gn_groups);
    VN_REQUIRE(d->split_k == 1, "gemm: gn_sums needs split_k = 1 (the statistics live in the fused epilogue)");
  }

  int cfg = d->tile_hint;
  bool dma = true;
  if (cfg >= 100) {
    dma = false;
    cfg -= 100;
  }
  if (cfg == 0) cfg = select_tile(d->M, d->N, batch);
  VN_REQUIRE(cfg >= 1 && cfg <= kMaxTile, "gemm: unknown tile_hint %d", d->tile_hint);
  if (cfg == 18 &&
      (d->conv_mode < 1 || d->conv_mode > 2 || d->stride != 1 || d->ups || d->pad_t != 1 || d->pad_l != 1 || d->Hi != d->Ho ||
       d->Wi != d->Wo || (d->Ho & 15) || (d->Wo & 15) || (d->Ci & 63) || !d->conv_korder || batch != 1 || f32))
    cfg = 17;
  if (cfg == 18 && d->gn_sums && (d->gn_cpg & 1)) cfg = 17;
  if ((cfg == 16 || cfg == 17) && (!dma || (d->conv_mode && (d->ups || (d->conv_mode == 2 && d->stride == 2))) ||
                    (d->gn_sums && (d->gn_cpg & 1)) ||
                    (d->M >= (1 << 24) && (d->conv_mode || d->rowadd || d->gn_sums)))) cfg = cfg == 16 ? 5 : 7;
  if ((cfg == 5 || cfg == 16) && f32) cfg = 4;
  if (cfg == 17 && f32) cfg = 7;
  if ((cfg == 6 || cfg == 7) && !dma) cfg = 4;
  if (cfg >= 10 && !dma) cfg = kTiles[cfg].bm == 128 ? (kTiles[cfg].bn == 128 ? 1 : 2) : 3;
  long long ws_floats = d->workspace ? d->workspace_bytes / 4 : 0;
  int ks = d->split_k;
  if (ks == 0) ks = select_ksplit(d->M, d->N, d->K, batch, cfg, ws_floats);
  if (ks < 1) ks = 1;
  const int nk = d->K / 64;
  if (ks > nk) ks = nk;
  if (ks > 1) {
    VN_REQUIRE(d->workspace && (long long)ks * batch * d->M * d->N <= ws_floats,
               "gemm: split_k=%d needs %lld workspace bytes", ks, (long long)ks * batch * d->M * d->N * 4);
    VN_REQUIRE(batch == 1 || (d->strideC != 0), "gemm: batched split-K needs strideC");
    VN_REQUIRE((long long)batch * d->M * ((d->N + 3) / 4) < 0x7fffffffLL, "gemm: split-K output larger than 2^31 chunks");
    VN_REQUIRE_OUT("gemm split-K workspace", (long long)ks * batch * d->M * d->N * 4);
  }
  if (cfg == 18 && ks > d->Ci / 64) ks = d->Ci / 64;
  g.ksplit = ks;
  g.kt_per_split = cdiv(nk, ks);
  g.ksplit = cdiv(nk, g.kt_per_split);
  VN_REQUIRE(g.ksplit <= 255 && g.kt_per_split <= 0xffff, "gemm: split_k=%d / K=%d out of range", g.ksplit, d->K);
  g.ws = (float*)d->workspace;

#define LAUNCH(BM, BN, WM, WN) \
  return dma ? launch_cfg<BM, BN, WM, WN, true>(g, f32, st) : launch_cfg<BM, BN, WM, WN, false>(g, f32, st)
  switch (cfg) {
    case 1: LAUNCH(128, 128, 64, 64);
    case 2: LAUNCH(128, 64, 64, 32);
    case 3: LAUNCH(64, 64, 32, 32);
    case 4: LAUNCH(256, 128, 64, 64);
    case 6: return launch_cfg_ring<256, 128, 64, 64>(g, f32, st);
    case 7: return launch_cfg_ring<256, 128, 64, 32>(g, f32, st);
    case 8: LAUNCH(256, 128, 64, 32);
    case 9: LAUNCH(128, 128, 64, 32);
    case 10: return launch_cfg_ring<128, 128, 64, 32>(g, f32, st);
    case 11: return launch_cfg_ring<128, 64, 64, 32>(g, f32, st);
    case 12: return launch_cfg_ring<64, 64, 32, 32>(g, f32, st);
    case 13: return launch_cfg_ring<128, 128, 64, 32, 4>(g, f32, st);
    case 14: return launch_cfg_ring<128, 64, 64, 32, 4>(g, f32, st);
    case 15: return launch_cfg_ring<64, 64, 32, 32, 4>(g, f32, st);
    case 16:
    case 17:
    case 18: {
      const int rc = vneti_launch_gemm8(&g, cfg == 16 ? 256 : 128, cfg == 18 ? 1 : 0, st);
      if (rc != VNETI_OK) return rc;
      launch_reduce(g, st);
      return vneti_check_launch("gemm8_kernel");
    }
    default:
      return dma ? launch_cfg_f16<256, 256, 64, 64, true>(g, st) : launch_cfg_f16<256, 256, 64, 64, false>(g, st);
  }
#undef LAUNCH
}
```

### view_neti_amd/csrc/norms.hip

```cpp
#include "common.h"
#include "../../include/vneti.h"

namespace {

#ifndef GN_APPLY_U
#define GN_APPLY_U 4
#endif
struct GNGeom {
  int Bn, HW, C, G, cpg, CC, TX, TY, rps, nslab;
  double inv_n;
};

__device__ __forceinline__ void vn_mean_rstd(double s0, double s1, double inv_n, float eps, float& m, float& r) {
  const double mu = s0 * inv_n;
  const double var = s1 * inv_n - mu * mu;
  const float v = fmaxf((float)var, 0.f) + eps;
  float y = __builtin_amdgcn_rsqf(v);
  y = y * (1.5f - 0.5f * v * y * y);
  m = (float)mu;
  r = y;
}

__device__ __forceinline__ void gn_thread_coords(const GNGeom& g, int& tx, int& ty, bool& active) {
  int tid = threadIdx.x;
// ... 748 lines not shown
                                   const float* beta, float* mean, float* rstd, float* ws, int Bn, int HW,
                                   int C, int G, float eps, int silu, void* stream) {
  GNGeom g;
  VN_REQUIRE(gn_geom(g, Bn, HW, C, G) == 0, "groupnorm: unsupported shape B=%d HW=%d C=%d G=%d", Bn, HW, C, G);
  VN_REQUIRE(x && y && gamma && beta && mean && rstd && ws, "groupnorm_fwd: null pointer");
  VN_REQUIRE(ldx % 8 == 0 && ldy % 8 == 0, "groupnorm_fwd: ld must be a multiple of 8");
  VN_REQUIRE_OUT("groupnorm_fwd", vn_out_bytes((long long)Bn * HW, ldy, C, 2));
  hipStream_t st = (hipStream_t)stream;
  if (gn_use_small(Bn, HW, C, G, false)) {
    if (silu)
      hipLaunchKernelGGL((gn_small_kernel<false, true>), dim3(G, Bn), dim3(512), 0, st, HW, C, G, (const half_t*)x, ldx,
                         (const half_t*)nullptr, 0LL, gamma, beta, mean, rstd, eps, (half_t*)y, ldy,
                         (const half_t*)nullptr, 0LL, g.inv_n);
    else
      hipLaunchKernelGGL((gn_small_kernel<false, false>), dim3(G, Bn), dim3(512), 0, st, HW, C, G, (const half_t*)x, ldx,
                         (const half_t*)nullptr, 0LL, gamma, beta, mean, rstd, eps, (half_t*)y, ldy,
                         (const half_t*)nullptr, 0LL, g.inv_n);
    return vneti_check_launch("groupnorm_fwd");
  }
  dim3 grid(g.nslab, Bn);
  hipLaunchKernelGGL((gn_stats_kernel<false, false>), grid, dim3(256), 0, st, g, (const half_t*)x, ldx,
                     (const half_t*)nullptr, 0LL, gamma, beta, (const float*)nullptr, (const float*)nullptr, ws);
  hipLaunchKernelGGL((gn_finalize_kernel<false>), dim3(Bn), dim3(256), 0, st, g, (const float*)ws, eps, mean, rstd);
  if (silu)
    hipLaunchKernelGGL((gn_apply_kernel<false, true>), grid, dim3(256), 0, st, g, (const half_t*)x, ldx,
                       (const half_t*)nullptr, 0LL, gamma, beta, (const float*)mean, (const float*)rstd,
                       (const float*)nullptr, (const float*)nullptr, (half_t*)y, ldy, (const half_t*)nullptr, 0LL);
  else
    hipLaunchKernelGGL((gn_apply_kernel<false, false>), grid, dim3(256), 0, st, g, (const half_t*)x, ldx,
                       (const half_t*)nullptr, 0LL, gamma, beta, (const float*)mean, (const float*)rstd,
                       (const float*)nullptr, (const float*)nullptr, (half_t*)y, ldy, (const half_t*)nullptr, 0LL);
  return vneti_check_launch("groupnorm_fwd");
}

extern "C" int vneti_groupnorm_fwd_sums(const void* x, long long ldx, void* y, long long ldy, const float* gamma,
                                        const float* beta, const void* sums_v, int slots, float* mean, float* rstd,
                                        int Bn, int HW, int C, int G, float eps, int silu, void* stream) {
  const float* sums = reinterpret_cast<const float*>(sums_v);
  GNGeom g;
  VN_REQUIRE(gn_geom(g, Bn, HW, C, G) == 0, "groupnorm: unsupported shape B=%d HW=%d C=%d G=%d", Bn, HW, C, G);
  VN_REQUIRE(x && y && gamma && beta && sums && mean && rstd && slots > 0, "groupnorm_fwd_sums: null pointer");
  VN_REQUIRE(ldx % 8 == 0 && ldy % 8 == 0, "groupnorm_fwd_sums: ld % 8 != 0");
  VN_REQUIRE_OUT("groupnorm_fwd_sums", vn_out_bytes((long long)Bn * HW, ldy, C, 2));
  hipStream_t st = (hipStream_t)stream;
  dim3 grid(g.nslab, Bn);
  if (silu)
    hipLaunchKernelGGL((gn_apply_kernel<false, true, true>), grid, dim3(256), 0, st, g, (const half_t*)x, ldx,
                       (const half_t*)nullptr, 0LL, gamma, beta, (const float*)nullptr, (const float*)nullptr,
                       (const float*)nullptr, (const float*)nullptr, (half_t*)y, ldy, (const half_t*)nullptr, 0LL,
                       sums, slots, eps, mean, rstd);
  else
    hipLaunchKernelGGL((gn_apply_kernel<false, false, true>), grid, dim3(256), 0, st, g, (const half_t*)x, ldx,
                       (const half_t*)nullptr, 0LL, gamma, beta, (const float*)nullptr, (const float*)nullptr,
                       (const float*)nullptr, (const float*)nullptr, (half_t*)y, ldy, (const half_t*)nullptr, 0LL,
                       sums, slots, eps, mean, rstd);
  return vneti_check_launch("groupnorm_fwd_sums");
}

extern "C" int vneti_groupnorm_fwd_2l(const void* x, long long ldx, void* y, long long ldy, const float* gamma,
                                      const float* beta, void* sums_v, int slots, float* mean, float* rstd, int Bn, int HW,
                                      int C, int G, float eps, int silu, void* stream) {
  float* sums = reinterpret_cast<float*>(sums_v);
  GNGeom g;
  VN_REQUIRE(gn_geom(g, Bn, HW, C, G) == 0, "groupnorm: unsupported shape B=%d HW=%d C=%d G=%d", Bn, HW, C, G);
  VN_REQUIRE(x && y && gamma && beta && mean && rstd && sums && slots > 0, "groupnorm_fwd_2l: null pointer");
  VN_REQUIRE(ldx % 8 == 0 && ldy % 8 == 0, "groupnorm_fwd_2l: ld must be a multiple of 8");
  VN_REQUIRE_OUT("groupnorm_fwd_2l", vn_out_bytes((long long)Bn * HW, ldy, C, 2));
  if (gn_use_small(Bn, HW, C, G, false))
    return vneti_groupnorm_fwd(x, ldx, y, ldy, gamma, beta, mean, rstd, sums, Bn, HW, C, G, eps, silu, stream);
  hipStream_t st = (hipStream_t)stream;
  dim3 grid(g.nslab, Bn);
  hipLaunchKernelGGL((gn_stats_kernel<false, false, true>), grid, dim3(256), 0, st, g, (const half_t*)x, ldx,
                     (const half_t*)nullptr, 0LL, gamma, beta, (const float*)nullptr, (const float*)nullptr, sums, slots);
  return vneti_groupnorm_fwd_sums(x, ldx, y, ldy, gamma, beta, sums, slots, mean, rstd, Bn, HW, C, G, eps, silu, stream);
}

extern "C" int vneti_groupnorm_bwd_2l(const void* dy, long long lddy, const void* x, long long ldx, const float* gamma,
                                      const float* beta, const float* mean, const float* rstd, void* dx, long long lddx,
                                      const void* dx_accum, long long ldacc, void* sums_v, int slots, float* ws, int Bn,
                                      int HW, int C, int G, int silu, void* stream);

extern "C" int vneti_groupnorm_bwd(const void* dy, long long lddy, const void* x, long long ldx,
                                   const float* gamma, const float* beta, const float* mean, const float* rstd,
                                   void* dx, long long lddx, const void* dx_accum, long long ldacc, float* ws,
                                   int Bn, int HW, int C, int G, int silu, void* stream) {
  GNGeom g;
  VN_REQUIRE(gn_geom(g, Bn, HW, C, G) == 0, "groupnorm: unsupported shape B=%d HW=%d C=%d G=%d", Bn, HW, C, G);
  VN_REQUIRE(dy && x && gamma && beta && mean && rstd && dx && ws, "groupnorm_bwd: null pointer");
  VN_REQUIRE(ldx % 8 == 0 && lddy % 8 == 0 && lddx % 8 == 0 && ldacc % 8 == 0, "groupnorm_bwd: ld % 8 != 0");
  VN_REQUIRE_OUT("groupnorm_bwd", vn_out_bytes((long long)Bn * HW, lddx, C, 2));
  hipStream_t st = (hipStream_t)stream;
  if (gn_use_small(Bn, HW, C, G, true)) {
    if (silu)
      hipLaunchKernelGGL((gn_small_kernel<true, true>), dim3(G, Bn), dim3(512), 0, st, HW, C, G, (const half_t*)x, ldx,
                         (const half_t*)dy, lddy, gamma, beta, const_cast<float*>(mean), const_cast<float*>(rstd), 0.f,
                         (half_t*)dx, lddx, (const half_t*)dx_accum, ldacc, g.inv_n);
    else
      hipLaunchKernelGGL((gn_small_kernel<true, false>), dim3(G, Bn), dim3(512), 0, st, HW, C, G, (const half_t*)x, ldx,
                         (const half_t*)dy, lddy, gamma, beta, const_cast<float*>(mean), const_cast<float*>(rstd), 0.f,
                         (half_t*)dx, lddx, (const half_t*)dx_accum, ldacc, g.inv_n);
    return vneti_check_launch("groupnorm_bwd");
  }
  dim3 grid(g.nslab, Bn);
  float* c1 = ws + (long long)Bn * g.nslab * 2 * G;
  float* c2 = c1 + (long long)Bn * G;
  if (silu)
    hipLaunchKernelGGL((gn_stats_kernel<true, true>), grid, dim3(256), 0, st, g, (const half_t*)x, ldx,
                       (const half_t*)dy, lddy, gamma, beta, mean, rstd, ws);
  else
    hipLaunchKernelGGL((gn_stats_kernel<true, false>), grid, dim3(256), 0, st, g, (const half_t*)x, ldx,
                       (const half_t*)dy, lddy, gamma, beta, mean, rstd, ws);
  hipLaunchKernelGGL((gn_finalize_kernel<true>), dim3(Bn), dim3(256), 0, st, g, (const float*)ws, 0.f, c1, c2);
  if (silu)
    hipLaunchKernelGGL((gn_apply_kernel<true, true>), grid, dim3(256), 0, st, g, (const half_t*)x, ldx,
                       (const half_t*)dy, lddy, gamma, beta, mean, rstd, (const float*)c1, (const float*)c2,
                       (half_t*)dx, lddx, (const half_t*)dx_accum, ldacc);
  else
    hipLaunchKernelGGL((gn_apply_kernel<true, false>), grid, dim3(256), 0, st, g, (const half_t*)x, ldx,
                       (const half_t*)dy, lddy, gamma, beta, mean, rstd, (const float*)c1, (const float*)c2,
                       (half_t*)dx, lddx, (const half_t*)dx_accum, ldacc);
  return vneti_check_launch("groupnorm_bwd");
}

extern "C" int vneti_groupnorm_bwd_2l(const void* dy, long long lddy, const void* x, long long ldx, const float* gamma,
                                      const float* beta, const float* mean, const float* rstd, void* dx, long long lddx,
                                      const void* dx_accum, long long ldacc, void* sums_v, int slots, float* ws, int Bn,
                                      int HW, int C, int G, int silu, void* stream) {
  float* sums = reinterpret_cast<float*>(sums_v);
  GNGeom g;
  VN_REQUIRE(gn_geom(g, Bn, HW, C, G) == 0, "groupnorm: unsupported shape B=%d HW=%d C=%d G=%d", Bn, HW, C, G);
  VN_REQUIRE(dy && x && gamma && beta && mean && rstd && dx && sums && slots > 0, "groupnorm_bwd_2l: null pointer");
  VN_REQUIRE(ldx % 8 == 0 && lddy % 8 == 0 && lddx % 8 == 0 && ldacc % 8 == 0, "groupnorm_bwd_2l: ld % 8 != 0");
  VN_REQUIRE_OUT("groupnorm_bwd_2l", vn_out_bytes((long long)Bn * HW, lddx, C, 2));
  if (gn_use_small(Bn, HW, C, G, true))
    return vneti_groupnorm_bwd(dy, lddy, x, ldx, gamma, beta, mean, rstd, dx, lddx, dx_accum, ldacc, ws, Bn, HW, C, G, silu,
                               stream);
  hipStream_t st = (hipStream_t)stream;
  dim3 grid(g.nslab, Bn);
#define GN_BWD_2L(S)                                                                                                     \
  hipLaunchKernelGGL((gn_stats_kernel<true, S, true>), grid, dim3(256), 0, st, g, (const half_t*)x, ldx, (const half_t*)dy, \
                     lddy, gamma, beta, mean, rstd, sums, slots);                                                         \
  hipLaunchKernelGGL((gn_apply_kernel<true, S, true>), grid, dim3(256), 0, st, g, (const half_t*)x, ldx, (const half_t*)dy, \
                     lddy, gamma, beta, mean, rstd, (const float*)nullptr, (const float*)nullptr, (half_t*)dx, lddx,      \
                     (const half_t*)dx_accum, ldacc, (const float*)sums, slots, 0.f, (float*)nullptr, (float*)nullptr)
  if (silu) {
    GN_BWD_2L(true);
  } else {
    GN_BWD_2L(false);
  }
#undef GN_BWD_2L
  return vneti_check_launch("groupnorm_bwd_2l");
}

extern "C" int vneti_layernorm_fwd(const void* x, int x_is_f32, long long ldx, void* y, long long ldy,
                                   const float* gamma, const float* beta, float* mean, float* rstd, int rows,
                                   int C, float eps, void* stream) {
  VN_REQUIRE(x && y && gamma && beta, "layernorm_fwd: null pointer");
  VN_REQUIRE(rows > 0 && C > 0 && C % 8 == 0 && C <= 8 * 64 * LN_MAXC, "layernorm: unsupported C=%d", C);
  VN_REQUIRE(ldx % 8 == 0 && ldy % 8 == 0, "layernorm_fwd: ld % 8 != 0");
  VN_REQUIRE_OUT("layernorm_fwd", vn_out_bytes(rows, ldy, C, 2));
  hipStream_t st = (hipStream_t)stream;
  dim3 grid(cdiv(rows, 4));
#define LN_FWD(F, NCH)                                                                                        \
  hipLaunchKernelGGL((ln_fwd_kernel<F, NCH>), grid, dim3(256), 0, st, x, ldx, (half_t*)y, ldy, gamma, beta, mean, \
                     rstd, rows, C, eps)
  const int nc = cdiv(C / 8, 64);
  if (x_is_f32) {
    switch (nc) {
      case 1: LN_FWD(true, 1); break;
      case 2: LN_FWD(true, 2); break;
      case 3: LN_FWD(true, 3); break;
      default: LN_FWD(true, 4); break;
    }
  } else {
    switch (nc) {
      case 1: LN_FWD(false, 1); break;
      case 2: LN_FWD(false, 2); break;
      case 3: LN_FWD(false, 3); break;
      default: LN_FWD(false, 4); break;
    }
  }
#undef LN_FWD
  return vneti_check_launch("layernorm_fwd");
}

extern "C" int vneti_layernorm_bwd(const void* dy, int dy_is_f32, long long lddy, const void* x, int x_is_f32,
                                   long long ldx, const float* gamma, const float* mean, const float* rstd,
                                   void* dx, int dx_is_f32, long long lddx, const void* dx_accum, long long ldacc,
                                   void* dx_f16_copy, long long ldcopy, int rows, int C, void* stream) {
  VN_REQUIRE(dy && x && gamma && mean && rstd && dx, "layernorm_bwd: null pointer");
  VN_REQUIRE(ldcopy % 8 == 0, "layernorm_bwd: ldcopy % 8 != 0");
  VN_REQUIRE(rows > 0 && C > 0 && C % 8 == 0 && C <= 8 * 64 * LN_MAXC, "layernorm: unsupported C=%d", C);
  VN_REQUIRE(ldx % 8 == 0 && lddy % 8 == 0 && lddx % 8 == 0 && ldacc % 8 == 0, "layernorm_bwd: ld % 8 != 0");
  VN_REQUIRE_OUT("layernorm_bwd", vn_out_bytes(rows, lddx, C, dx_is_f32 ? 4 : 2));
  if (dx_f16_copy) VN_REQUIRE_OUT("layernorm_bwd f16 copy", vn_out_bytes(rows, ldcopy, C, 2));
  hipStream_t st = (hipStream_t)stream;
  dim3 grid(cdiv(rows, 4));
  const int nc = cdiv(C / 8, 64);
#define LN_BWD_N(A, B, Cc, NCH)                                                                                         \
  hipLaunchKernelGGL((ln_bwd_kernel<A, B, Cc, NCH>), grid, dim3(256), 0, st, dy, lddy, x, ldx, gamma, mean, rstd, dx, \
                     lddx, dx_accum, ldacc, (half_t*)dx_f16_copy, ldcopy, rows, C)
#define LN_BWD(A, B, Cc)                      \
  switch (nc) {                               \
    case 1: LN_BWD_N(A, B, Cc, 1); break;     \
    case 2: LN_BWD_N(A, B, Cc, 2); break;     \
    case 3: LN_BWD_N(A, B, Cc, 3); break;     \
    default: LN_BWD_N(A, B, Cc, 4); break;    \
  }
  int key = (dy_is_f32 ? 4 : 0) | (x_is_f32 ? 2 : 0) | (dx_is_f32 ? 1 : 0);
  switch (key) {
    case 0: LN_BWD(false, false, false); break;
    case 1: LN_BWD(false, false, true); break;
    case 2: LN_BWD(false, true, false); break;
    case 3: LN_BWD(false, true, true); break;
    case 4: LN_BWD(true, false, false); break;
    case 5: LN_BWD(true, false, true); break;
    case 6: LN_BWD(true, true, false); break;
    default: LN_BWD(true, true, true); break;
  }
#undef LN_BWD
#undef LN_BWD_N
  return vneti_check_launch("layernorm_bwd");
}

extern "C" int vneti_softmax_rows_f16(void* x, long long ld, int rows, int cols, void* stream) {
  VN_REQUIRE(x && rows > 0 && cols > 0 && cols % 8 == 0 && cols <= 8 * 256 * SM_MAXC && ld % 8 == 0,
             "softmax_rows: unsupported cols=%d ld=%lld", cols, ld);
  hipLaunchKernelGGL(softmax_rows_kernel, dim3(rows), dim3(256), 0, (hipStream_t)stream, (half_t*)x, ld, cols);
  return vneti_check_launch("softmax_rows");
}
```

### view_neti_amd/engine/schedule.py

```python
from __future__ import annotations

from functools import partial
from typing import Dict, List

import torch

from .. import lib, ops, packing


class T:

    __slots__ = ("v", "g", "gw", "rows", "cols", "children", "need_grad", "producer")

    def __init__(self, v, g=None, need_grad=True):
        self.v = v
        self.g = g
        self.gw = False
        self.rows, self.cols = v.shape
        self.children: List["T"] = []
        self.need_grad = need_grad
        self.producer = None


def rup(x, m):
    return (x + m - 1) // m * m


class Schedule:
    def __init__(self, batch: int, groups: int, eps: float, device: str = "cuda", need_backward: bool = True):
        self.B = batch
        self.groups = groups
        self.eps = eps
        self.dev = device
        self.need_backward = need_backward
        self.fwd_pre: List = []
        self.fwd: List = []
        self.bwd: List = []
        self.tape: List = []
        self.bytes = 0
        self._scratch: Dict[str, torch.Tensor] = {}
        self.temb_off: Dict[str, tuple] = {}
        self.temb_all = None
        self.gn_ws = self._buf((batch * 256 * 2 * groups + 2 * batch * groups,), torch.float32)
        self.ws = self._buf((16 * 2 ** 20,), torch.float32)
        self.ws_side = None
        self._side_stream = None
        self._gn_fusable: List[dict] = []
        self.gn_sums = None
        if ops._default_ws is None or ops._default_ws.device != torch.device(device, torch.cuda.current_device()):
            ops.set_default_gemm_workspace(torch.empty(16 * 2 ** 20, dtype=torch.float32, device=device))

    def _buf(self, shape, dtype=None, zero=False):
        dtype = dtype or lib.act_dtype()
        t = (torch.zeros if zero else torch.empty)(shape, dtype=dtype, device=self.dev)
        self.bytes += t.numel() * t.element_size()
        return t

    def _tmp(self, name, rows, cols, dtype=None):
        dtype = dtype or lib.act_dtype()
        """reusable scratch for backward temporaries (single stream => sequential lifetimes)."""
        key = f"{name}:{dtype}"
        n = rows * cols
        cur = self._scratch.get(key)
        if cur is None or cur.numel() < n:
            self._scratch[key] = self._buf((n,), dtype)
            cur = self._scratch[key]
        return cur[:n].view(rows, cols)

    def _w16(self, t):
        w = t.to(device=self.dev, dtype=lib.act_dtype()).contiguous()
        self.bytes += w.numel() * 2
        return w

    def _w32(self, t):
        w = t.to(device=self.dev, dtype=torch.float32).contiguous()
        self.bytes += w.numel() * 4
        return w

    def _grad(self, t: T):
        if t.g is None:
            t.g = self._buf((t.rows, t.cols))
        return t.g

    def _contrib(self, t: T, fn, extra=None):
        g = self._grad(t)
        if t.gw:
            if extra is not None:
                self.bwd.append(partial(ops.add, g, extra, g))
            self.bwd.append(self._tagged(partial(fn, g, g), fn))
        else:
            self.bwd.append(self._tagged(partial(fn, g, extra), fn))
            t.gw = True
            for c in t.children:
                c.gw = True

    @staticmethod
    def _tagged(p, fn):
        if hasattr(fn, "vn_cost"):
            p.vn_cost = fn.vn_cost
        return p

    def _contrib_gemm(self, t: T, A, Bm, **kw):
        g = self._grad(t)
        resid = g if t.gw else None
        self.bwd.append(partial(ops.gemm, A, Bm, g, resid=resid, **kw))
        if not t.gw:
            t.gw = True
            for c in t.children:
                c.gw = True

    _tile_cache: Dict[tuple, int] = {}
    _TILE_DIMS = {1: (128, 128), 2: (128, 64), 3: (64, 64), 4: (256, 128), 5: (256, 256), 6: (256, 128), 7: (256, 128),
                  8: (256, 128), 9: (128, 128), 10: (128, 128), 11: (128, 64), 12: (64, 64), 13: (128, 128), 14: (128, 64),
                  15: (64, 64), 16: (256, 256), 17: (256, 128), 18: (256, 128)}

    @staticmethod
    def _gemm_key(f):
        kw = f.keywords
        A, Bm, out = f.args[:3]
        conv = kw.get("conv")
        M = kw.get("M") or A.shape[-2]
        N = kw.get("N") or Bm.shape[-2]
        K = kw.get("K") or Bm.shape[-1]
        ck = (conv["mode"], conv["stride"], conv["ups"], conv["Hi"], conv["Wi"]) if conv else None
        return (M, N, K, kw.get("batch") or 1, ck, out.dtype == torch.float32, kw.get("geglu") or 0)

    def autotune(self, candidates=(1, 2, 3, 5, 6, 7, 8, 9, 10, 11, 12, 13, 14, 15, 16, 17, 18), reps=8):
        if not torch.cuda.is_available():
            return
        import os
        cold = None if os.environ.get("VNETI_AUTOTUNE_HOT") else torch.empty(160 * 2 ** 20, dtype=torch.float32, device=self.dev)
        if os.environ.get("VNETI_AUTOTUNE_CANDS"):
            candidates = tuple(int(x) for x in os.environ["VNETI_AUTOTUNE_CANDS"].split(","))
        cold_reps = int(os.environ.get("VNETI_AUTOTUNE_REPS", "9"))
        warm_a = bool(int(os.environ.get("VNETI_AUTOTUNE_WARM_A", "1")))
        cache = Schedule._tile_cache
        cache_path = os.environ.get("VNETI_AUTOTUNE_CACHE")
        if cache_path and os.path.exists(cache_path) and not cache:
            import ast
            import json
            for k, v in json.load(open(cache_path)).items():
                cache[ast.literal_eval(k)] = tuple(v)
        n_before = len(cache)
        from .. import parallel
        share = parallel.sharing_picks() and parallel._dist() is not None
        rank0 = (not share) or parallel._dist().get_rank() == 0
        if share and not rank0:
            cache.update(parallel.share_from_rank0(None))
        for lst in (self.fwd_pre, self.fwd, self.bwd):
            for idx, f in enumerate(lst):
                if getattr(f, "func", None) is not ops.gemm or f.keywords.get("tile_hint"):
                    continue
                key = self._gemm_key(f)
                conv = f.keywords.get("conv")
                try_cm = bool(conv) and not conv.get("ups") and not conv.get("korder") and \
                    not (conv["mode"] == 2 and conv["stride"] == 2) and conv["Ci"] % 64 == 0 and conv["Ci"] >= 128
                B_cm = None
                if key not in cache:
                    best, best_t = (0, 0, 0), float("inf")
                    M_, N_, K_ = key[:3]
                    halo_ok = try_cm and conv["mode"] in (1, 2) and conv["stride"] == 1 and conv["pad_t"] == 1 and conv["pad_l"] == 1 \
                        and conv["Ho"] % 16 == 0 and conv["Wo"] % 16 == 0 and conv["Hi"] == conv["Ho"] and conv["Wi"] == conv["Wo"]
                    variants = [(h, 0) for h in candidates if h != 18] + \
                        ([(h, 1) for h in candidates if h in (16, 17) or (h == 18 and halo_ok)] if try_cm else [])
                    if try_cm:
                        B_cm = packing._chunk_major(f.args[1], f.args[1].shape[0], conv["Ci"])
                    for h, ko in variants:
                        bm, bn = self._TILE_DIMS[h % 100]
                        tiles = -(-M_ // bm) * -(-N_ // bn) * key[3]
                        sks = (0, 1) + (tuple(x for x in (2, 3, 4, 6, 8, 12)
                                              if x * 8 <= K_ // 64 and tiles * x <= 1024 and x * key[3] * M_ * N_ <= 16 * 2 ** 20)
                                        if tiles < 256 else ())
                        if f.keywords.get("geglu"):
                            sks = (1,)
                        for sk in sks:
                            kw = dict(f.keywords)
                            kw["tile_hint"], kw["split_k"] = h, sk
                            args = f.args
                            if ko:
                                kw["conv"] = dict(conv, korder=1)
                                args = (f.args[0], B_cm) + tuple(f.args[2:])
                            ops.gemm(*args, **kw)
                            ops.gemm(*args, **kw)
                            if cold is None:
                                s, e = torch.cuda.Event(enable_timing=True), torch.cuda.Event(enable_timing=True)
                                s.record()
                                for _ in range(reps):
                                    ops.gemm(*args, **kw)
                                e.record()
                                e.synchronize()
                                t = s.elapsed_time(e)
                            else:
                                ts = []
                                for _ in range(cold_reps):
                                    cold.fill_(0)
                                    if warm_a:
                                        args[0].add_(0)
                                    s, e = torch.cuda.Event(enable_timing=True), torch.cuda.Event(enable_timing=True)
                                    s.record()
                                    ops.gemm(*args, **kw)
                                    e.record()
                                    e.synchronize()
                                    ts.append(s.elapsed_time(e))
                                t = sorted(ts)[len(ts) // 2]
                            if t < best_t:
                                best, best_t = (h, sk, ko), t
                    cache[key] = best
                pick = tuple(cache[key]) + (0,) * (3 - len(cache[key]))
                kw = dict(f.keywords)
                kw["tile_hint"], kw["split_k"] = pick[0], pick[1]
                if pick[2] and try_cm:
                    if B_cm is None:
                        B_cm = packing._chunk_major(f.args[1], f.args[1].shape[0], conv["Ci"])
                    kw["conv"] = dict(conv, korder=1)
                    self.bytes += B_cm.numel() * B_cm.element_size()
                    f_cm = partial(ops.gemm, f.args[0], B_cm, *f.args[2:], **f.keywords)
                    if getattr(f, "side", False):
                        f_cm.side = True
                    f = f_cm
                lst[idx] = self._rebound(f, ops.gemm, kw)
        if share and rank0:
            parallel.share_from_rank0(dict(cache))
        if cache_path and len(cache) != n_before and parallel.world_info()[0] == 0:
            import json
            tmp = f"{cache_path}.{os.getpid()}.tmp"
            with open(tmp, "w") as fh:
                json.dump({repr(k): list(v) for k, v in cache.items()}, fh)
            os.replace(tmp, cache_path)

    def bind_workspace(self):
        for lst in (self.fwd_pre, self.fwd, self.bwd):
            for idx, f in enumerate(lst):
                fn = getattr(f, "func", None)
                if fn is ops.gemm or fn is ops.attn_bwd_dkv:
                    kw = dict(f.keywords)
                    kw["workspace"] = self.ws_side if getattr(f, "side", False) else self.ws
                    lst[idx] = self._rebound(f, fn, kw)

    @staticmethod
    def _rebound(f, fn, kw):
        p = partial(fn, *f.args, **kw)
        if getattr(f, "side", False):
            p.side = True
        return p

    def _side(self, launch):
        launch.side = True
        if self.ws_side is None:
            self.ws_side = self._buf((4 * 2 ** 20,), torch.float32)
        return launch

    GN_SLOTS = 8

    def _produced(self, t: T):
        t.producer = len(self.fwd) - 1
        return t

    GN2_MAX = 512

    def _gn2_slice(self):
        if not hasattr(self, "_gn2_arena"):
            self._gn2_arena = self._buf((self.GN2_MAX, self.B, self.GN_SLOTS, self.groups, 4), torch.int64, zero=True)
            self._gn2_used = 0
        assert self._gn2_used < self.GN2_MAX
        self._gn2_used += 1
        return self._gn2_arena[self._gn2_used - 1]

    def fuse_gn_stats(self, fuse: bool = True):
        n = self._fuse_gn_stats() if fuse else 0
        if getattr(self, "_gn2_used", 0):
            self.fwd.insert(0, self._gn2_arena[:self._gn2_used].zero_)
        return n

    def _fuse_gn_stats(self):
        import os
        if os.environ.get("VNETI_NO_GN_FUSE"):
            return 0
        S, G, B = self.GN_SLOTS, self.groups, self.B
        todo = []
        for rec in self._gn_fusable:
            f = self.fwd[rec["prod"]]
            kw = f.keywords
            hw, Cc = rec["hw"], rec["C"]
            cpg = Cc // G
            if getattr(f, "func", None) is ops.conv3x3_in:
                if hw % 256 == 0 and cpg % 4 == 0 and 128 % cpg == 0 and kw.get("gn_sums") is None:
                    todo.append(rec)
                continue
            if getattr(f, "func", None) is not ops.gemm or kw.get("batch"):
                continue
            if kw.get("split_k") != 1:
                M_, N_, K_ = self._gemm_key(f)[:3]
                ws = kw.get("workspace")
                wsb = ws.numel() * ws.element_size() if ws is not None else 0
                if ops.gemm_select_split(M_, N_, K_, 1, kw.get("tile_hint") or 0, wsb) != 1:
                    continue
            if hw < 64 or not (cpg >= 8 or cpg == 4) or kw.get("gn_sums") is not None:
                continue
            todo.append(rec)
        if not todo:
            return 0
        self.gn_sums = self._buf((len(todo), B, S, G, 4), torch.int64, zero=True)
        for i, rec in enumerate(todo):
            sums = self.gn_sums[i]
            f = self.fwd[rec["prod"]]
            kw = dict(f.keywords)
            kw.update(gn_sums=sums, gn_hw=rec["hw"], gn_groups=G, gn_slots=S)
            if f.func is ops.gemm:
                kw.update(split_k=1)
            self.fwd[rec["prod"]] = self._rebound(f, f.func, kw)
            g = rec["gn"]
            self.fwd[rec["idx"]] = partial(ops.groupnorm_fwd_sums, rec["x"], rec["y"], g["gamma"], g["beta"], sums, S,
                                           g["mean"], g["rstd"], B, rec["hw"], rec["C"], G, rec["eps"], rec["silu"])
        arena = self.gn_sums
        self.fwd.insert(0, arena.zero_)
        self._gn_fusable = []
        return len(todo)

    def _gn(self, x: T, name, w, eps, silu):
        Cc = x.cols
        hw = x.rows // self.B
        rec = dict(kind="gn", x=x, gamma=self._w32(w[name + ".weight"]), beta=self._w32(w[name + ".bias"]),
                   mean=self._buf((self.B * self.groups,), torch.float32),
                   rstd=self._buf((self.B * self.groups,), torch.float32), silu=silu, hw=hw)
        y = self._buf((x.rows, Cc))
        import os
        if os.environ.get("VNETI_GN_3L"):
            self.fwd.append(partial(ops.groupnorm_fwd, x.v, y, rec["gamma"], rec["beta"], rec["mean"], rec["rstd"],
                                    self.gn_ws, self.B, hw, Cc, self.groups, eps, silu))
        else:
            self.fwd.append(partial(ops.groupnorm_fwd_2l, x.v, y, rec["gamma"], rec["beta"], self._gn2_slice(),
                                    self.GN_SLOTS, rec["mean"], rec["rstd"], self.B, hw, Cc, self.groups, eps, silu))
            if self.need_backward:
                rec["bsums"] = self._gn2_slice()
        if x.producer is not None:
            self._gn_fusable.append(dict(idx=len(self.fwd) - 1, prod=x.producer, gn=rec, x=x.v, y=y, hw=hw, C=Cc,
                                         eps=eps, silu=silu))
        return y, rec

    def _gn_bwd_fn(self, rec, dy):
        x = rec["x"]
        if "bsums" not in rec:
            fn = lambda out, accum: ops.groupnorm_bwd(dy, x.v, rec["gamma"], rec["beta"], rec["mean"], rec["rstd"], out,
                                                      self.gn_ws, self.B, rec["hw"], x.cols, self.groups,
                                                      rec["silu"], accum=accum)
        else:
            fn = lambda out, accum: ops.groupnorm_bwd_2l(dy, x.v, rec["gamma"], rec["beta"], rec["mean"], rec["rstd"], out,
                                                         rec["bsums"], self.GN_SLOTS, self.gn_ws, self.B, rec["hw"], x.cols,
                                                         self.groups, rec["silu"], accum=accum)
        fn.vn_cost = ("GroupNorm(+SiLU) bwd", 5.0 * self.B * rec["hw"] * x.cols * 2)
        return fn

    def _conv_desc(self, Hi, Wi, Ci, Ho, Wo, stride, pad, ups, ldx, mode=1):
        return dict(mode=mode, Hi=Hi, Wi=Wi, Ci=Ci, Ho=Ho, Wo=Wo, stride=stride, pad_t=pad, pad_l=pad, ups=ups,
                    ldx=ldx, korder=1 if (packing.KORDER_CM and Ci % 64 == 0) else 0)

    def _resnet(self, x: T, cin, cout, name, w, out_view, h, wd, need_dx=True):
        M = x.rows
        n1, gn1 = self._gn(x, name + "norm1", w, self.eps, True)
        w1 = self._w16(packing.conv3x3_fwd(w[name + "conv1.weight"]))
        b1 = self._w32(w[name + "conv1.bias"])
        radd = None
        if name in self.temb_off:
            off, n = self.temb_off[name]
            radd = self.temb_all[:, off:off + n]
        h1 = T(self._buf((M, cout)))
        self.fwd.append(partial(ops.gemm, n1, w1, h1.v, bias=b1, rowadd=radd, rows_per_group=h * wd, M=M,
                                conv=self._conv_desc(h, wd, cin, h, wd, 1, 1, 0, cin)))
        self._produced(h1)
        n2, gn2 = self._gn(h1, name + "norm2", w, self.eps, True)
        w2 = self._w16(packing.conv3x3_fwd(w[name + "conv2.weight"]))
        b2 = self._w32(w[name + "conv2.bias"])
        out = T(out_view if out_view is not None else self._buf((M, cout)))
        wsc = None
        if cin != cout:
            wsc = self._w16(w[name + "conv_shortcut.weight"].reshape(cout, cin))
            bsc = self._w32(w[name + "conv_shortcut.bias"])
            sc_buf = self._buf((M, cout))
            self.fwd.append(partial(ops.gemm, x.v, wsc, sc_buf, bias=bsc))
            resid = sc_buf
        else:
            resid = x.v
        self.fwd.append(partial(ops.gemm, n2, w2, out.v, bias=b2, resid=resid, M=M,
                                conv=self._conv_desc(h, wd, cout, h, wd, 1, 1, 0, cout)))
        self._produced(out)
        rec = dict(kind="resnet", x=x, out=out, h1=h1, gn1=gn1, gn2=gn2, cin=cin, cout=cout, h=h, wd=wd,
                   need_dx=need_dx, name=name)
        if self.need_backward and need_dx:
            rec["w2d"] = self._w16(packing.conv3x3_dgrad(w[name + "conv2.weight"]))
            rec["w1d"] = self._w16(packing.conv3x3_dgrad(w[name + "conv1.weight"]))
            if wsc is not None:
                rec["wscd"] = self._w16(w[name + "conv_shortcut.weight"].reshape(cout, cin).t())
        self.tape.append(rec)
        return out

    def _resnet_bwd(self, r):
        if not r["need_dx"]:
            return
        x, out, h, wd, cin, cout = r["x"], r["out"], r["h"], r["wd"], r["cin"], r["cout"]
        M = x.rows
        dout = out.g
        assert out.gw, f"resnet {r['name']}: output gradient was never produced"
        dn2 = self._tmp("dA", M, cout)
        self.bwd.append(partial(ops.gemm, dout, r["w2d"], dn2, M=M,
                                conv=self._conv_desc(h, wd, cout, h, wd, 1, 1, 0, dout.stride(0), mode=2)))
        dh1 = self._tmp("dB", M, cout)
        self.bwd.append(partial(self._gn_bwd_fn(r["gn2"], dn2), dh1, None))
        dn1 = self._tmp("dC", M, cin)
        self.bwd.append(partial(ops.gemm, dh1, r["w1d"], dn1, M=M,
                                conv=self._conv_desc(h, wd, cout, h, wd, 1, 1, 0, cout, mode=2)))
        if "wscd" in r:
            self._contrib_gemm(x, dout, r["wscd"])
            self._contrib(x, self._gn_bwd_fn(r["gn1"], dn1))
        else:
            self._contrib(x, self._gn_bwd_fn(r["gn1"], dn1), extra=dout)

    def _ln(self, xv, name, w):
        rows, Cc = xv.shape
        rec = dict(x=xv, gamma=self._w32(w[name + ".weight"]), beta=self._w32(w[name + ".bias"]),
                   mean=self._buf((rows,), torch.float32), rstd=self._buf((rows,), torch.float32))
        y = self._buf((rows, Cc))
        self.fwd.append(partial(ops.layernorm_fwd, xv, y, rec["gamma"], rec["beta"], rec["mean"], rec["rstd"], 1e-5))
        return y, rec

    def _ln_bwd(self, rec, dy, dx, accum, f16_copy=None):
        ops.layernorm_bwd(dy, rec["x"], rec["gamma"], rec["mean"], rec["rstd"], dx, accum=accum, f16_copy=f16_copy)

    def _downsample(self, x: T, Cc, name, w, out_view, h, wd, pad=1):
        M = x.rows // 4
        wf = self._w16(packing.conv3x3_fwd(w[name + "weight"]))
        b = self._w32(w[name + "bias"])
        out = T(out_view if out_view is not None else self._buf((M, Cc)))
        self.fwd.append(partial(ops.gemm, x.v, wf, out.v, bias=b, M=M,
                                conv=self._conv_desc(h, wd, Cc, h // 2, wd // 2, 2, pad, 0, x.v.stride(0))))
        self._produced(out)
        rec = dict(kind="down", x=x, out=out, C=Cc, h=h, wd=wd, pad=pad)
        if self.need_backward:
            rec["wd_"] = self._w16(packing.conv3x3_dgrad(w[name + "weight"]))
        self.tape.append(rec)
        return out

    def _downsample_bwd(self, r):
        x, out, Cc, h, wd = r["x"], r["out"], r["C"], r["h"], r["wd"]
        assert out.gw
        desc = self._conv_desc(h // 2, wd // 2, Cc, h, wd, 2, r["pad"], 0, out.g.stride(0), mode=2)
        self._contrib_gemm(x, out.g, r["wd_"], M=x.rows, conv=desc)

    def forward_pre(self):
        for f in self.fwd_pre:
            f()

    def forward_main(self):
        for f in self.fwd:
            f()

    def forward(self):
        self.forward_pre()
        self.forward_main()

    def _run(self, lst):
        side = None
        main = None
        for f in lst:
            if getattr(f, "side", False):
                if side is None:
                    if self._side_stream is None:
                        self._side_stream = torch.cuda.Stream()
                    side, main = self._side_stream, torch.cuda.current_stream()
                side.wait_stream(main)
                with torch.cuda.stream(side):
                    f()
            else:
                f()
        if side is not None:
            main.wait_stream(side)

    def backward(self):
        self._run(self.bwd)
```

### view_neti_amd/engine/unet.py

```python
from __future__ import annotations

from functools import partial
from typing import Dict

import torch

from .. import ops, packing
from .. import sd_config as sc
from .schedule import Schedule, T, rup as _rup


class UNetEngine(Schedule):
    def __init__(self, cfg: sc.UNetConfig, weights: Dict[str, torch.Tensor], batch: int, height: int, width: int,
                 ctx_len: int = 77, device: str = "cuda", need_backward: bool = True, autotune: bool = True,
                 fuse_gn: bool = True):
        super().__init__(batch, cfg.norm_num_groups, cfg.norm_eps, device, need_backward)
        self.cfg = cfg
        self.H, self.W = height, width
        self.L = ctx_len
        self.nl = cfg.n_cross_layers
        B, L, Dc = batch, ctx_len, cfg.cross_attention_dim
        self.x_in = self._buf((B, cfg.in_channels, height, width), torch.float32)
        self.timesteps = torch.zeros(B, dtype=torch.int64, device=device)
        self.ctx_k = self._buf((self.nl, B * L, Dc))
# ... 65 lines not shown
        while l0 < len(ws):
            n = 1
            while l0 + n < len(ws) and ws[l0 + n] == ws[l0]:
                n += 1
            Cc = ws[l0]
            run = dict(l0=l0, n=n, C=Cc, wk=self._buf((n, Cc, Dc)), wv=self._buf((n, Cc, Dc)),
                       k=self._buf((n, B * L, Cc)), v=self._buf((n, B * L, Cc)))
            if self.need_backward:
                run.update(wkd=self._buf((n, Dc, Cc)), wvd=self._buf((n, Dc, Cc)),
                           dk=self._buf((n, B * L, Cc)), dv=self._buf((n, B * L, Cc)))
            for j in range(n):
                self.kv_slot[l0 + j] = (run, j)
            self.kv_runs.append(run)
            l0 += n

    def _kv_fwd_ops(self):
        B, L, Dc = self.B, self.L, self.cfg.cross_attention_dim
        for run in self.kv_runs:
            l0, n, Cc = run["l0"], run["n"], run["C"]
            for ctx, wgt, out in ((self.ctx_k, run["wk"], run["k"]), (self.ctx_v, run["wv"], run["v"])):
                self.fwd_pre.append(partial(ops.gemm, ctx[l0], wgt[0], out[0], batch=n, strideA=B * L * Dc,
                                            strideB=Cc * Dc, strideC=B * L * Cc))

    def _kv_bwd_ops(self):
        B, L, Dc = self.B, self.L, self.cfg.cross_attention_dim
        for run in self.kv_runs:
            l0, n, Cc = run["l0"], run["n"], run["C"]
            for dsrc, wgt, dctx in ((run["dk"], run["wkd"], self.dctx_k), (run["dv"], run["wvd"], self.dctx_v)):
                self.bwd.append(partial(ops.gemm, dsrc[0], wgt[0], dctx[l0], batch=n, strideA=B * L * Cc,
                                        strideB=Dc * Cc, strideC=B * L * Dc))

    def _transformer(self, x: T, Cc, heads, name, w, layer_idx, out_view, h, wd, need_dx=True):
        cfg = self.cfg
        B, L, Dc = self.B, self.L, cfg.cross_attention_dim
        M, N = x.rows, h * wd
        D = Cc // heads
        scale = D ** -0.5
        t = name + "transformer_blocks.0."
        r = dict(kind="transformer", x=x, C=Cc, heads=heads, D=D, N=N, name=name, layer=layer_idx, need_dx=need_dx,
                 scale=scale)
        g, r["gn"] = self._gn(x, name + "norm", w, 1e-6, False)
        w_in = w[name + "proj_in.weight"].reshape(Cc, Cc)
        r["w_in"], b_in = self._w16(w_in), self._w32(w[name + "proj_in.bias"])
        h0 = self._buf((M, Cc))
        self.fwd.append(partial(ops.gemm, g, r["w_in"], h0, bias=b_in))
        n1, r["ln1"] = self._ln(h0, t + "norm1", w)
        wqkv = torch.cat([w[t + "attn1.to_q.weight"], w[t + "attn1.to_k.weight"], w[t + "attn1.to_v.weight"]], 0)
        r["wqkv"] = self._w16(wqkv)
        qkv = self._buf((M, 3 * Cc))
        self.fwd.append(partial(ops.gemm, n1, r["wqkv"], qkv))
        q, k, v = qkv[:, :Cc], qkv[:, Cc:2 * Cc], qkv[:, 2 * Cc:]
        o1 = self._buf((M, Cc))
        lse1 = self._buf((B, heads, N), torch.float32)
        self.fwd.append(partial(ops.attn_fwd, q, k, v, o1, lse1, B, heads, N, N, D, scale, False))
        r["wo1"], bo1 = self._w16(w[t + "attn1.to_out.0.weight"]), self._w32(w[t + "attn1.to_out.0.bias"])
        h1 = self._buf((M, Cc))
        self.fwd.append(partial(ops.gemm, o1, r["wo1"], h1, bias=bo1, resid=h0))
        n2, r["ln2"] = self._ln(h1, t + "norm2", w)
        r["wq2"] = self._w16(w[t + "attn2.to_q.weight"])
        run, slot = self.kv_slot[layer_idx]
        assert run["C"] == Cc, (name, layer_idx, Cc, run["C"])
        run["wk"][slot].copy_(w[t + "attn2.to_k.weight"])
        run["wv"][slot].copy_(w[t + "attn2.to_v.weight"])
        q2 = self._buf((M, Cc))
        k2, v2 = run["k"][slot], run["v"][slot]
        self.fwd.append(partial(ops.gemm, n2, r["wq2"], q2))
        o2 = self._buf((M, Cc))
        lse2 = self._buf((B, heads, N), torch.float32)
        self.fwd.append(partial(ops.attn_fwd, q2, k2, v2, o2, lse2, B, heads, N, L, D, scale, False))
        r["wo2"], bo2 = self._w16(w[t + "attn2.to_out.0.weight"]), self._w32(w[t + "attn2.to_out.0.bias"])
        h2 = self._buf((M, Cc))
        self.fwd.append(partial(ops.gemm, o2, r["wo2"], h2, bias=bo2, resid=h1))
        n3, r["ln3"] = self._ln(h2, t + "norm3", w)
        wff1_il = packing.geglu_interleave(w[t + "ff.net.0.proj.weight"])
        r["wff1"], bff1 = self._w16(wff1_il), self._w32(packing.geglu_interleave(w[t + "ff.net.0.proj.bias"]))
        r["wff2"], bff2 = self._w16(w[t + "ff.net.2.weight"]), self._w32(w[t + "ff.net.2.bias"])
        p = self._buf((M, 8 * Cc))
        gg = self._buf((M, 4 * Cc))
        self.fwd.append(partial(ops.gemm, n3, r["wff1"], p, bias=bff1, out2=gg, geglu=1, split_k=1))
        h3 = self._buf((M, Cc))
        self.fwd.append(partial(ops.gemm, gg, r["wff2"], h3, bias=bff2, resid=h2))
        r["w_out"], b_out = self._w16(w[name + "proj_out.weight"].reshape(Cc, Cc)), self._w32(w[name + "proj_out.bias"])
        out = T(out_view if out_view is not None else self._buf((M, Cc)))
        self.fwd.append(partial(ops.gemm, h3, r["w_out"], out.v, bias=b_out, resid=x.v))
        self._produced(out)
        r.update(out=out, h0=h0, h1=h1, h2=h2, qkv=qkv, o1=o1, lse1=lse1, q2=q2, k2=k2, v2=v2, o2=o2, lse2=lse2,
                 p=p)
        if self.need_backward:
            tr = lambda a: self._w16(a.t())
            run["wkd"][slot].copy_(w[t + "attn2.to_k.weight"].t())
            run["wvd"][slot].copy_(w[t + "attn2.to_v.weight"].t())
            r["w_outd"] = tr(w[name + "proj_out.weight"].reshape(Cc, Cc))
            r["wff2d"], r["wff1d"] = tr(w[t + "ff.net.2.weight"]), tr(wff1_il)
            r["wo2d"] = tr(w[t + "attn2.to_out.0.weight"])
            if need_dx:
                r["wq2d"] = tr(w[t + "attn2.to_q.weight"])
                r["wo1d"] = tr(w[t + "attn1.to_out.0.weight"])
                r["wqkvd"] = tr(wqkv)
                r["w_ind"] = tr(w_in)
        self.tape.append(r)
        return out

    def _transformer_bwd(self, r):
        B, L, Cc, heads, D, N = self.B, self.L, r["C"], r["heads"], r["D"], r["N"]
        x, out = r["x"], r["out"]
        M = x.rows
        dout = out.g
        assert out.gw, f"transformer {r['name']}: output gradient was never produced"
        li = r["layer"]
        bw = self.bwd
        dh3 = self._tmp("tA", M, Cc)
        bw.append(partial(ops.gemm, dout, r["w_outd"], dh3))
        dp = self._tmp("tC", M, 8 * Cc)
        bw.append(partial(ops.gemm, dh3, r["wff2d"], dp, gate=r["p"], gate_act=ops.ACT_GELU, geglu=2, split_k=1))
        dn3 = self._tmp("tD", M, Cc)
        bw.append(partial(ops.gemm, dp, r["wff1d"], dn3))
        dh2 = self._tmp("tE", M, Cc)
        bw.append(partial(self._ln_bwd, r["ln3"], dn3, dh2, dh3))
        do2 = self._tmp("tA", M, Cc)
        bw.append(partial(ops.gemm, dh2, r["wo2d"], do2))
        delta = self._tmp("tdelta", B * heads, N, torch.float32)
        dq2 = self._tmp("tD", M, Cc)
        if r["need_dx"]:
            bw.append(partial(ops.attn_bwd_dq, r["q2"], r["k2"], r["v2"], do2, r["lse2"], delta, dq2, B, heads, N, L, D,
                              r["scale"], False, O=r["o2"]))
        else:
            bw.append(partial(ops.attn_bwd_delta, do2, r["o2"], delta, B, heads, N, D))
        run, slot = self.kv_slot[li]
        dk2, dv2 = run["dk"][slot], run["dv"][slot]
        bw.append(partial(ops.attn_bwd_dkv, r["q2"], r["k2"], r["v2"], do2, r["lse2"], delta, dk2, dv2, B, heads, N, L,
                          D, r["scale"], False))
        if not r["need_dx"]:
            return
        dn2 = self._tmp("tA", M, Cc)
        bw.append(partial(ops.gemm, dq2, r["wq2d"], dn2))
        dh1 = self._tmp("tF", M, Cc)
        bw.append(partial(self._ln_bwd, r["ln2"], dn2, dh1, dh2))
        do1 = self._tmp("tA", M, Cc)
        bw.append(partial(ops.gemm, dh1, r["wo1d"], do1))
        qkv = r["qkv"]
        q, k, v = qkv[:, :Cc], qkv[:, Cc:2 * Cc], qkv[:, 2 * Cc:]
        dqkv = self._tmp("tC", M, 3 * Cc)
        dq, dk, dv = dqkv[:, :Cc], dqkv[:, Cc:2 * Cc], dqkv[:, 2 * Cc:]
        bw.append(partial(ops.attn_bwd_dq, q, k, v, do1, r["lse1"], delta, dq, B, heads, N, N, D, r["scale"], False,
                          O=r["o1"]))
        bw.append(partial(ops.attn_bwd_dkv, q, k, v, do1, r["lse1"], delta, dk, dv, B, heads, N, N, D, r["scale"],
                          False))
        dn1 = self._tmp("tD", M, Cc)
        bw.append(partial(ops.gemm, dqkv, r["wqkvd"], dn1))
        dh0 = self._tmp("tE", M, Cc)
        bw.append(partial(self._ln_bwd, r["ln1"], dn1, dh0, dh1))
        dg = self._tmp("tA", M, Cc)
        bw.append(partial(ops.gemm, dh0, r["w_ind"], dg))
        self._contrib(x, self._gn_bwd_fn(r["gn"], dg), extra=dout)

    def _upsample(self, x: T, Cc, name, w, out_view, h, wd):
        M = x.rows * 4
        wf = self._w16(packing.conv3x3_fwd(w[name + "weight"]))
        b = self._w32(w[name + "bias"])
        out = T(out_view if out_view is not None else self._buf((M, Cc)))
        self.fwd.append(partial(ops.gemm, x.v, wf, out.v, bias=b, M=M,
                                conv=self._conv_desc(h, wd, Cc, 2 * h, 2 * wd, 1, 1, 1, x.v.stride(0))))
        self._produced(out)
        rec = dict(kind="up", x=x, out=out, C=Cc, h=h, wd=wd)
        if self.need_backward:
            rec["wd_"] = self._w16(packing.conv3x3_dgrad(w[name + "weight"]))
        self.tape.append(rec)
        return out

    def _upsample_bwd(self, r):
        x, out, Cc, h, wd = r["x"], r["out"], r["C"], r["h"], r["wd"]
        assert out.gw and not x.gw
        M = out.rows
        dup = self._tmp("dA", M, Cc)
        self.bwd.append(partial(ops.gemm, out.g, r["wd_"], dup, M=M,
                                conv=self._conv_desc(2 * h, 2 * wd, Cc, 2 * h, 2 * wd, 1, 1, 0, out.g.stride(0), mode=2)))
        g = self._grad(x)
        self.bwd.append(partial(ops.sum2x2, dup, g, self.B, h, wd, Cc))
        x.gw = True

    def _build(self, w):
        cfg = self.cfg
        B, H, W = self.B, self.H, self.W
        boc = cfg.block_out_channels
        nlev = len(boc)
        nres = cfg.layers_per_block + 1
        self._time_ops()
        catT = {}
        for i in range(nlev):
            lvl = nlev - 1 - i
            m = B * (H >> lvl) * (W >> lvl)
            for j in range(nres):
                rin, skip, _ = sc.up_block_channels(cfg, i, j)
                catT[(i, j)] = T(self._buf((m, rin + skip)),
                                 self._buf((m, rin + skip)) if self.need_backward else None)

        def h_slot(key):
            rin = sc.up_block_channels(cfg, *key)[0]
            return catT[key].v[:, :rin]

        def adopt(t: T, key, part):
            rin = sc.up_block_channels(cfg, *key)[0]
            cat = catT[key]
            if cat.g is not None:
                t.g = cat.g[:, :rin] if part == "h" else cat.g[:, rin:]
            cat.children.append(t)
            return t

        skip_targets = list(reversed([(i, j) for i in range(nlev) for j in range(nres)]))
        nskip = [0]

        def next_skip():
            key = skip_targets[nskip[0]]
            nskip[0] += 1
            rin = sc.up_block_channels(cfg, *key)[0]
            return key, catT[key].v[:, rin:]

        M0 = B * H * W
        col = self._buf((M0, 64))
        w_in = self._w16(packing.pad_rows(packing.conv3x3_fwd(w["conv_in.weight"]), 64))
        b_in = self._w32(w["conv_in.bias"])
        key, sv = next_skip()
        self.fwd.append(partial(ops.im2col3x3_small, self.x_in, col, B, cfg.in_channels, H, W, H, W, 1, 1, 1,
                                self.x_in.stride()))
        self.fwd.append(partial(ops.gemm, col, w_in, sv, bias=b_in))
        hcur = adopt(self._produced(T(sv, need_grad=False)), key, "skip")
        layer = 0
        first = True
        cin = boc[0]
        for i, cout in enumerate(boc):
            h, wd = H >> i, W >> i
            for j in range(cfg.layers_per_block):
                name = f"down_blocks.{i}.resnets.{j}."
                key, sv = next_skip()
                if cfg.down_has_attn[i]:
                    r_out = self._resnet(hcur, cin if j == 0 else cout, cout, name, w, None, h, wd, need_dx=not first)
                    hcur = self._transformer(r_out, cout, cfg.num_heads[i], f"down_blocks.{i}.attentions.{j}.", w,
                                             layer, sv, h, wd, need_dx=not first)
                    layer += 1
                else:
                    hcur = self._resnet(hcur, cin if j == 0 else cout, cout, name, w, sv, h, wd, need_dx=not first)
                adopt(hcur, key, "skip")
                first = False
            if i < nlev - 1:
                key, sv = next_skip()
                hcur = self._downsample(hcur, cout, f"down_blocks.{i}.downsamplers.0.conv.", w, sv, h, wd)
                adopt(hcur, key, "skip")
            cin = cout
        assert nskip[0] == len(skip_targets)
        lvl = nlev - 1
        h, wd = H >> lvl, W >> lvl
        cm = boc[-1]
        hcur = self._resnet(hcur, cm, cm, "mid_block.resnets.0.", w, None, h, wd)
        hcur = self._transformer(hcur, cm, cfg.num_heads[-1], "mid_block.attentions.0.", w, layer, None, h, wd)
        layer += 1
        hcur = self._resnet(hcur, cm, cm, "mid_block.resnets.1.", w, h_slot((0, 0)), h, wd)
        adopt(hcur, (0, 0), "h")
        up_has_attn = tuple(reversed(cfg.down_has_attn))
        up_heads = tuple(reversed(cfg.num_heads))
        for i in range(nlev):
            lvl = nlev - 1 - i
            h, wd = H >> lvl, W >> lvl
            for j in range(nres):
                rin, skip, out_c = sc.up_block_channels(cfg, i, j)
                nxt = (i, j + 1) if j < nres - 1 else None
                nxt_view = h_slot(nxt) if nxt is not None else None
                name = f"up_blocks.{i}.resnets.{j}."
                if up_has_attn[i]:
                    r_out = self._resnet(catT[(i, j)], rin + skip, out_c, name, w, None, h, wd)
                    hcur = self._transformer(r_out, out_c, up_heads[i], f"up_blocks.{i}.attentions.{j}.", w, layer,
                                             nxt_view, h, wd)
                    layer += 1
                else:
                    hcur = self._resnet(catT[(i, j)], rin + skip, out_c, name, w, nxt_view, h, wd)
                if nxt is not None:
                    adopt(hcur, nxt, "h")
            if i < nlev - 1:
                out_c = tuple(reversed(boc))[i]
                hcur = self._upsample(hcur, out_c, f"up_blocks.{i}.upsamplers.0.conv.", w, h_slot((i + 1, 0)), h, wd)
                adopt(hcur, (i + 1, 0), "h")
        assert layer == self.nl
        c0 = boc[0]
        n, gn = self._gn(hcur, "conv_norm_out", w, cfg.norm_eps, True)
        w_o = self._w16(packing.conv3x3_fwd(w["conv_out.weight"]))
        b_o = self._w32(w["conv_out.bias"])
        self.fwd.append(partial(ops.gemm, n, w_o, self.pred, bias=b_o, M=M0,
                                conv=self._conv_desc(H, W, c0, H, W, 1, 1, 0, c0)))
        rec = dict(kind="head", x=hcur, gn=gn)
        if self.need_backward:
            wt = w["conv_out.weight"].flip(2, 3).transpose(0, 1).contiguous()
            rec["wd_"] = self._w16(packing.pad_rows(packing.conv3x3_fwd(wt), 64))
        self.tape.append(rec)

    def _head_bwd(self, r):
        x = r["x"]
        M0 = self.B * self.H * self.W
        col = self._tmp("hcol", M0, 64)
        dp = self.dpred
        ld = dp.stride(0)
        self.bwd.append(partial(ops.im2col3x3_small, dp, col, self.B, self.cfg.out_channels, self.H, self.W, self.H,
                                self.W, 1, 1, 1, (self.H * self.W * ld, 1, self.W * ld, ld)))
        dn = self._tmp("dA", M0, x.cols)
        self.bwd.append(partial(ops.gemm, col, r["wd_"], dn))
        self._contrib(x, self._gn_bwd_fn(r["gn"], dn))

    def _build_backward(self):
        for r in reversed(self.tape):
            k = r["kind"]
            if k == "head":
                self._head_bwd(r)
            elif k == "resnet":
                self._resnet_bwd(r)
            elif k == "transformer":
                self._transformer_bwd(r)
            elif k == "down":
                self._downsample_bwd(r)
            elif k == "up":
                self._upsample_bwd(r)
```

### view_neti_amd/lib.py

```python
from __future__ import annotations

import ctypes as C
import keyword
import os
import re

_HERE = os.path.dirname(os.path.abspath(__file__))
HEADER_PATH = os.path.join(os.path.dirname(_HERE), "include", "vneti.h")

_PRECISIONS = {"fp16": ("libvneti_hip.so", 0), "bf16": ("libvneti_hip_bf16.so", 1)}
_precision = os.environ.get("VNETI_PRECISION", "fp16")
if _precision not in _PRECISIONS:
    raise RuntimeError(f"VNETI_PRECISION={_precision!r}: expected one of {sorted(_PRECISIONS)}")

_lib = None


def so_path(precision: str = None) -> str:
    return os.environ.get("VNETI_LIB_PATH") or os.path.join(_HERE, "csrc", _PRECISIONS[precision or _precision][0])


SO_PATH = so_path()


def precision() -> str:
    return _precision


def set_precision(p: str) -> None:
    global _precision, SO_PATH
    if p not in _PRECISIONS:
        raise ValueError(f"precision {p!r}: expected one of {sorted(_PRECISIONS)}")
    if _lib is not None and p != _precision:
        raise RuntimeError(f"libvneti is already loaded in {_precision}; {p} needs its own process")
    _precision = p
    SO_PATH = so_path()


def act_dtype():
    import torch
    return torch.bfloat16 if _precision == "bf16" else torch.float16


_SCALARS = {"int": C.c_int, "long long": C.c_longlong, "float": C.c_float, "unsigned": C.c_uint, "unsigned int": C.c_uint,
            "uint32_t": C.c_uint, "size_t": C.c_size_t}


def _ctype(ctype: str, structs: dict, where: str):
    words = [w for w in ctype.replace("*", " * ").split() if w != "const"]
    stars, base = words.count("*"), " ".join(w for w in words if w != "*")
    if stars == 0 and base in _SCALARS:
        return _SCALARS[base]
    if stars == 1 and base == "char":
        return C.c_char_p
    if stars == 1 and base in structs:
        return C.POINTER(structs[base])
    if stars and (base in _SCALARS or base in ("void", "char")):
        return C.c_void_p
    raise ValueError(f"vneti.h {where}: no ctypes rule for the type {ctype.strip()!r}")


def _declarator(decl: str, where: str):
    m = re.fullmatch(r"(.*[\s*])(\w+)", decl.strip(), re.S)
    if not m:
        raise ValueError(f"vneti.h {where}: cannot read the declaration {' '.join(decl.split())!r}")
    return m.group(1), m.group(2)


def parse_header(text: str):
    blank = lambda m: "\n" * m.group().count("\n")
    text = re.sub(r"/\*.*?\*/|//[^\n]*", blank, text, flags=re.S)
    text = re.sub(r'^[ \t]*#.*$|extern\s+"C"\s*\{|^\}[ \t]*$', "", text, flags=re.M)
    at = lambda src, pos: f"line {src.count(chr(10), 0, pos) + 1}"
    structs, protos = {}, {}
    typedef = r"typedef\s+struct\s+\w*\s*\{(.*?)\}\s*(\w+)\s*;"
    for m in re.finditer(typedef, text, flags=re.S):
        fields = []
        for d in re.finditer(r"[^;\s][^;]*", m.group(1)):
            where = at(text, m.start(1) + d.start())
            first, *more = d.group().split(",")
            ctype, name = _declarator(first, where)
            for n in [name] + [x.strip() for x in more]:
                if not n.isidentifier() or keyword.iskeyword(n):
                    raise ValueError(f"vneti.h {where}: cannot bind the field {n!r}")
                fields.append((n, _ctype(ctype, structs, where)))
        structs[m.group(2)] = type(m.group(2), (C.Structure,), {"_fields_": fields})
    rest = re.sub(typedef, blank, text, flags=re.S)
    for m in re.finditer(r"[^;\s][^;]*", rest):
        p = re.fullmatch(r"(int|long long)\s+(vneti_\w+)\s*\((.*)\)\s*", m.group(), re.S)
        if not p:
            raise ValueError(f"vneti.h {at(rest, m.start())}: cannot read {' '.join(m.group().split())!r} as a prototype")
        argtypes = []
        for x in re.finditer(r"[^,\s][^,]*", "" if p.group(3).strip() == "void" else p.group(3)):
            where = at(rest, m.start() + p.start(3) + x.start())
            argtypes.append(_ctype(_declarator(x.group(), where)[0], structs, where))
        protos[p.group(2)] = (_SCALARS[p.group(1)], argtypes)
    return structs, protos


with open(HEADER_PATH) as _f:
    _STRUCTS, _PROTOS = parse_header(_f.read())
GemmDesc, TransposeDesc = _STRUCTS["vneti_gemm_desc"], _STRUCTS["vneti_transpose_desc"]
SIGNATURES = {n[len("vneti_"):]: argtypes for n, (_, argtypes) in _PROTOS.items()}
VALUE_FUNCS = frozenset({
    "version", "precision", "last_error", "gemm_select_tile", "gemm_select_split", "img_resample_ksize",
    "groupnorm_ws_floats", "lpips_ws_floats", "mapper_num_params", "mapper_save_floats", "mapper_rowgrad_floats",
    "mapper_legacy_input_params"})
_stray = ({n[len("vneti_"):] for n, (res, _) in _PROTOS.items() if res is C.c_longlong} - VALUE_FUNCS) | (VALUE_FUNCS - set(SIGNATURES))
if _stray:
    raise RuntimeError(f"lib.VALUE_FUNCS is out of step with include/vneti.h: {sorted(_stray)}")


def declared_symbols() -> list[str]:
    src = open(HEADER_PATH).read()
    src = re.sub(r"/\*.*?\*/", "", src, flags=re.S)
    return sorted(set(re.findall(r"\b(vneti_[a-z0-9_]+)\s*\(", src)))


def load():
    global _lib
    if _lib is not None:
        return _lib
    if not os.path.exists(SO_PATH):
        raise RuntimeError(
            f"{os.path.basename(SO_PATH)} not found at {SO_PATH}: build it with "
            "`python view_neti_amd/csrc/build.py` (hipcc, gfx950). There is no fallback path.")
    lib = C.CDLL(SO_PATH)
    for name, (restype, argtypes) in _PROTOS.items():
        fn = getattr(lib, name, None)
        if fn is None:
            raise RuntimeError(f"{SO_PATH} does not export {name}, which include/vneti.h declares: rebuild it")
        fn.restype, fn.argtypes = restype, argtypes
    if lib.vneti_precision() != _PRECISIONS[_precision][1]:
        raise RuntimeError(f"{SO_PATH} computes in precision {lib.vneti_precision()}, the process asked for {_precision}")
    _lib = lib
    return lib


def last_error() -> str:
    lib = load()
    buf = C.create_string_buffer(512)
    lib.vneti_last_error(buf, 512)
    return buf.value.decode(errors="replace")


def check(rc: int, what: str = ""):
    if rc != 0:
        raise RuntimeError(f"vneti call failed ({what}) rc={rc}: {last_error()}")


def call(name: str, *args):
    check(getattr(load(), "vneti_" + name)(*args), name)


def query(name: str, *args) -> int:
    if name not in VALUE_FUNCS:
        raise KeyError(f"vneti_{name} returns a status: use call()")
    return int(getattr(load(), "vneti_" + name)(*args))
```

### view_neti_amd/ops.py

```python
from __future__ import annotations

import ctypes as C

import torch

from . import lib as _l

ACT_NONE, ACT_SILU, ACT_QUICK_GELU, ACT_GELU = 0, 1, 2, 3


def stream() -> int:
    return torch.cuda.current_stream().cuda_stream


def _p(t):
    return None if t is None else t.data_ptr()


def _ld(t):
    if t is None:
        return 0
    assert t.stride(-1) == 1, "last dim must be contiguous"
    return t.stride(-2) if t.dim() >= 2 else t.shape[-1]


_default_ws = None


def set_default_gemm_workspace(t):
    global _default_ws
    _default_ws = t


def gemm(A, B, out, *, bias=None, rowadd=None, rows_per_group=1, resid=None, alpha=1.0, act=0,
         tile_hint=0, batch=0, strideA=0, strideB=0, strideC=0, M=None, N=None, K=None, conv=None,
         lda=None, ldc=None, workspace=None, split_k=0, gate=None, gate_act=0, out2=None, act2=0,
         gn_sums=None, gn_hw=0, gn_groups=0, gn_slots=0, geglu=0):
    d = _l.GemmDesc()
    d.A, d.B, d.C = _p(A), _p(B), _p(out)
    d.ldb = _ld(B)
    d.ldc = ldc if ldc is not None else _ld(out)
    d.N = N if N is not None else B.shape[-2]
    d.K = K if K is not None else B.shape[-1]
    if conv is None:
        d.M = M if M is not None else A.shape[-2]
        d.lda = lda if lda is not None else _ld(A)
        d.conv_mode = 0
    else:
        d.M = M
        d.lda = 0
        d.conv_mode = conv["mode"]
        for k in ("Hi", "Wi", "Ci", "Ho", "Wo", "stride", "pad_t", "pad_l", "ups", "ldx"):
            setattr(d, k, int(conv.get(k, 0)))
        d.conv_korder = int(conv.get("korder", 0))
    d.batch = batch
    d.strideA, d.strideB, d.strideC = strideA, strideB, strideC
    d.bias = _p(bias)
    d.rowadd = _p(rowadd)
    d.ld_rowadd = _ld(rowadd) if rowadd is not None else 0
    d.rows_per_group = rows_per_group
    d.resid = _p(resid)
    d.ldr = _ld(resid) if resid is not None else 0
    d.alpha = alpha
    d.act = act
    d.out_f32 = 1 if out.dtype == torch.float32 else 0
    d.tile_hint = tile_hint
    if gate is not None:
        d.gate_src, d.ld_gate, d.gate_act = _p(gate), _ld(gate), gate_act
    if out2 is not None:
        d.C2, d.ldc2, d.act2 = _p(out2), _ld(out2), act2
    if gn_sums is not None:
        d.gn_sums, d.gn_hw, d.gn_groups, d.gn_slots = _p(gn_sums), gn_hw, gn_groups, gn_slots
        d.gn_cpg = d.N // gn_groups
    d.geglu = geglu
    ws = workspace if workspace is not None else _default_ws
    if ws is not None:
        d.workspace = ws.data_ptr()
        d.workspace_bytes = ws.numel() * ws.element_size()
    d.split_k = split_k if ws is not None else 1
    _l.call("gemm_f16", C.byref(d), stream())


def im2col3x3_small(x, out, Bn, Cc, Hi, Wi, Ho, Wo, stride, pad_t, pad_l, strides):
    sb, sc, sy, sx = strides
    _l.call("im2col3x3_small", _p(x), 1 if x.dtype == torch.float32 else 0, sb, sc, sy, sx, _p(out),
            Bn, Cc, Hi, Wi, Ho, Wo, stride, pad_t, pad_l, stream())


def conv3x3_in(x, w_packed, bias, out, Bn, Cc, H, W, strides, gn_sums=None, gn_hw=0, gn_groups=0, gn_slots=0):
    sb, sc, sy, sx = strides
    assert gn_sums is None or gn_hw == H * W
    _l.call("conv3x3_in", _p(x), 1 if x.dtype == torch.float32 else 0, sb, sc, sy, sx, _p(w_packed), _p(bias), _p(out),
            _ld(out), Bn, Cc, H, W, w_packed.shape[0], _p(gn_sums), gn_groups, gn_slots, stream())


def transpose(inp, out, rows, cols, batch, ld_in, stride_in, ld_out, stride_out):
    _l.call("transpose_f16", _p(inp), ld_in, stride_in, _p(out), ld_out, stride_out, rows, cols, batch, stream())


def transpose_multi(items):
    arr = (_l.TransposeDesc * len(items))()
    for d, (inp, out, rows, cols, batch, ld_in, stride_in, ld_out, stride_out) in zip(arr, items):
        d.inp, d.ld_in, d.stride_in = _p(inp), ld_in, stride_in
        d.out, d.ld_out, d.stride_out = _p(out), ld_out, stride_out
        d.rows, d.cols, d.batch = rows, cols, batch
    _l.call("transpose_f16_multi", arr, len(items), stream())


def groupnorm_ws_floats(Bn, HW, Cc, G):
    n = _l.query("groupnorm_ws_floats", Bn, HW, Cc, G)
    if n < 0:
        raise RuntimeError(f"groupnorm: unsupported shape {(Bn, HW, Cc, G)}")
    return n


def groupnorm_fwd(x, y, gamma, beta, mean, rstd, ws, Bn, HW, Cc, G, eps, silu):
    _l.call("groupnorm_fwd", _p(x), _ld(x), _p(y), _ld(y), _p(gamma), _p(beta), _p(mean), _p(rstd), _p(ws),
            Bn, HW, Cc, G, eps, 1 if silu else 0, stream())


def groupnorm_fwd_sums(x, y, gamma, beta, sums, slots, mean, rstd, Bn, HW, Cc, G, eps, silu):
    _l.call("groupnorm_fwd_sums", _p(x), _ld(x), _p(y), _ld(y), _p(gamma), _p(beta), _p(sums), slots, _p(mean), _p(rstd),
            Bn, HW, Cc, G, eps, 1 if silu else 0, stream())


def groupnorm_fwd_2l(x, y, gamma, beta, sums, slots, mean, rstd, Bn, HW, Cc, G, eps, silu):
    _l.call("groupnorm_fwd_2l", _p(x), _ld(x), _p(y), _ld(y), _p(gamma), _p(beta), _p(sums), slots, _p(mean), _p(rstd),
            Bn, HW, Cc, G, eps, 1 if silu else 0, stream())


def groupnorm_bwd_2l(dy, x, gamma, beta, mean, rstd, dx, sums, slots, ws, Bn, HW, Cc, G, silu, accum=None):
    _l.call("groupnorm_bwd_2l", _p(dy), _ld(dy), _p(x), _ld(x), _p(gamma), _p(beta), _p(mean), _p(rstd),
            _p(dx), _ld(dx), _p(accum), _ld(accum) if accum is not None else 0, _p(sums), slots, _p(ws),
            Bn, HW, Cc, G, 1 if silu else 0, stream())


def groupnorm_bwd(dy, x, gamma, beta, mean, rstd, dx, ws, Bn, HW, Cc, G, silu, accum=None):
    _l.call("groupnorm_bwd", _p(dy), _ld(dy), _p(x), _ld(x), _p(gamma), _p(beta), _p(mean), _p(rstd),
            _p(dx), _ld(dx), _p(accum), _ld(accum) if accum is not None else 0, _p(ws),
            Bn, HW, Cc, G, 1 if silu else 0, stream())


def layernorm_fwd(x, y, gamma, beta, mean, rstd, eps):
    rows, Cc = x.shape
    _l.call("layernorm_fwd", _p(x), 1 if x.dtype == torch.float32 else 0, _ld(x), _p(y), _ld(y), _p(gamma),
            _p(beta), _p(mean), _p(rstd), rows, Cc, eps, stream())


def layernorm_bwd(dy, x, gamma, mean, rstd, dx, accum=None, f16_copy=None):
    rows, Cc = x.shape
    _l.call("layernorm_bwd", _p(dy), 1 if dy.dtype == torch.float32 else 0, _ld(dy), _p(x),
            1 if x.dtype == torch.float32 else 0, _ld(x), _p(gamma), _p(mean), _p(rstd), _p(dx),
            1 if dx.dtype == torch.float32 else 0, _ld(dx), _p(accum),
            _ld(accum) if accum is not None else 0, _p(f16_copy), _ld(f16_copy) if f16_copy is not None else 0,
            rows, Cc, stream())


def attn_fwd(Q, K, V, O, lse, Bn, H, Nq, Nk, D, scale, causal):
    _l.call("attn_fwd", _p(Q), _ld(Q), _p(K), _ld(K), _p(V), _ld(V), _p(O), _ld(O), _p(lse), Bn, H, Nq, Nk, D,
            scale, 1 if causal else 0, stream())


def attn_bwd_delta(dO, O, delta, Bn, H, Nq, D):
    _l.call("attn_bwd_delta", _p(dO), _ld(dO), _p(O), _ld(O), _p(delta), Bn, H, Nq, D, stream())


def attn_bwd_dq(Q, K, V, dO, lse, delta, dQ, Bn, H, Nq, Nk, D, scale, causal, O=None):
    _l.call("attn_bwd_dq", _p(Q), _ld(Q), _p(K), _ld(K), _p(V), _ld(V), _p(dO), _ld(dO), _p(lse), _p(delta),
            _p(O), _ld(O) if O is not None else 0, _p(dQ), _ld(dQ), Bn, H, Nq, Nk, D, scale, 1 if causal else 0,
            stream())


def attn_bwd_dkv(Q, K, V, dO, lse, delta, dK, dV, Bn, H, Nq, Nk, D, scale, causal, workspace=None):
    ws = workspace if workspace is not None else _default_ws
    _l.call("attn_bwd_dkv", _p(Q), _ld(Q), _p(K), _ld(K), _p(V), _ld(V), _p(dO), _ld(dO), _p(lse), _p(delta),
            _p(dK), _ld(dK), _p(dV), _ld(dV), Bn, H, Nq, Nk, D, scale, 1 if causal else 0, _p(ws),
            ws.numel() if ws is not None else 0, stream())


def attn_bwd_small_ok(N, D):
    return N <= 96 and D == 64


def attn_bwd_small(Q, K, V, dO, O, lse, dQ, dK, dV, Bn, H, N, D, scale, causal):
    _l.call("attn_bwd_small", _p(Q), _ld(Q), _p(K), _ld(K), _p(V), _ld(V), _p(dO), _ld(dO), _p(O), _ld(O), _p(lse),
            _p(dQ), _ld(dQ), _p(dK), _ld(dK), _p(dV), _ld(dV), Bn, H, N, D, scale, 1 if causal else 0, stream())


def softmax_rows(x, rows, cols):
    _l.call("softmax_rows_f16", _p(x), _ld(x), rows, cols, stream())


def add(a, b, out):
    rows, cols = out.shape
    _l.call("add_f16", _p(a), _ld(a), _p(b), _ld(b), _p(out), _ld(out), rows, cols, stream())


def geglu_fwd(p, out):
    rows, c4 = out.shape
    _l.call("geglu_fwd", _p(p), _ld(p), _p(out), _ld(out), rows, c4, stream())


def geglu_bwd(dy, p, dp):
    rows, c4 = dy.shape
    _l.call("geglu_bwd", _p(dy), _ld(dy), _p(p), _ld(p), _p(dp), _ld(dp), rows, c4, stream())


def act_fwd(x, y, act):
    _l.call("act_fwd_f16", _p(x), _p(y), x.numel(), act, stream())


def act_bwd(dy, x, dx, act):
    _l.call("act_bwd_f16", _p(dy), _p(x), _p(dx), x.numel(), act, stream())


def timestep_embedding(t, out):
    Bn, dim = out.shape
    _l.call("timestep_embedding", _p(t), _p(out), Bn, dim, stream())


def sum2x2(inp, out, Bn, H, W, Cc):
    _l.call("sum2x2_f16", _p(inp), _ld(inp), _p(out), _ld(out), Bn, H, W, Cc, stream())


def rng_fill_normal(out, state, stream_id):
    _l.call("rng_fill_normal", _p(out), out.numel(), _p(state), stream_id, stream())


def rng_fill_randint(out, high, state, stream_id):
    _l.call("rng_fill_randint", _p(out), out.numel(), high, _p(state), stream_id, stream())


def rng_advance(state):
    _l.call("rng_advance", _p(state), stream())


def sample_add_noise(moments, eps, noise, t, ac, scaling, vpred, latents, noisy, target, Bn, Lc, HW):
    _l.call("sample_add_noise", _p(moments), _ld(moments), _p(eps), _p(noise), _p(t), _p(ac), scaling,
            1 if vpred else 0, _p(latents), _p(noisy), _p(target), Bn, Lc, HW, stream())


def gn_sums_decode(sums: torch.Tensor) -> torch.Tensor:
    import numpy as np
    a = sums.detach().cpu().numpy().astype(np.int64)
    out = np.empty(a.shape[:-1] + (2,), dtype=np.float64)
    for q in range(2):
        hi, lo = a[..., 2 * q].astype(object), a[..., 2 * q + 1].astype(object)
        k = np.vectorize(lambda h, l: (h * 2 ** 36 - l + 2 ** 63) // 2 ** 64, otypes=[object])(hi, lo)
        out[..., q] = np.vectorize(lambda l, kk: float(l + kk * 2 ** 64) / 2.0 ** 40, otypes=[np.float64])(lo, k)
    return torch.from_numpy(out)


def latent_sample(moments, eps, scaling, latents, Bn, Lc, HW):
    _l.call("latent_sample", _p(moments), _ld(moments), _p(eps), scaling, _p(latents), Bn, Lc, HW, stream())


def add_noise(latents, noise, t, ac, vpred, noisy, target, Bn, Lc, HW):
    _l.call("add_noise", _p(latents), _p(noise), _p(t), _p(ac), 1 if vpred else 0, _p(noisy), _p(target), Bn, Lc, HW,
            stream())


def cfg_sampler_step(pred, x, m_prev, x_in, Bn, Lc, HW, guidance, alpha_t, sigma_t, cx, c0, c1, v_prediction):
    _l.call("cfg_sampler_step", _p(pred), _ld(pred), _p(x), _p(m_prev), _p(x_in), Bn, Lc, HW, guidance, alpha_t,
            sigma_t, cx, c0, c1, 1 if v_prediction else 0, stream())


def cfg_sampler_step_table(pred, x, m_prev, x_in, Bn, Lc, HW, guidance, coef_table, step, v_prediction):
    _l.call("cfg_sampler_step_table", _p(pred), _ld(pred), _p(x), _p(m_prev), _p(x_in), Bn, Lc, HW, guidance,
            _p(coef_table), _p(step), 1 if v_prediction else 0, stream())


def cfg_sampler_step_noise(pred, x, m_prev, x_in, noise, Bn, Lc, HW, guidance, alpha_t, sigma_t, cx, c0, c1, cn,
                           v_prediction):
    _l.call("cfg_sampler_step_noise", _p(pred), _ld(pred), _p(x), _p(m_prev), _p(x_in), _p(noise), Bn, Lc, HW, guidance,
            alpha_t, sigma_t, cx, c0, c1, cn, 1 if v_prediction else 0, stream())


def cfg_sampler_step_noise_table(pred, x, m_prev, x_in, Bn, Lc, HW, guidance, coef_table, noise_table, step,
                                 v_prediction):
    _l.call("cfg_sampler_step_noise_table", _p(pred), _ld(pred), _p(x), _p(m_prev), _p(x_in), Bn, Lc, HW, guidance,
            _p(coef_table), _p(noise_table), _p(step), 1 if v_prediction else 0, stream())


def table_fill_i64(dst, table, step):
    _l.call("table_fill_i64", _p(dst), dst.numel(), _p(table), _p(step), stream())

# ... 201 lines not shown
```

### view_neti_amd/roofline.py

```python
from __future__ import annotations

import torch

from . import ops

import os as _os

_CSRC = _os.path.join(_os.path.dirname(_os.path.abspath(__file__)), "csrc")
MFMA_PEAK_TFLOPS = 2500.0
HBM_PEAK_TBS = 8.0
PF, TB = MFMA_PEAK_TFLOPS, HBM_PEAK_TBS


def kernel_tree_sha() -> str:
    import hashlib
    import os
    here = _CSRC
    files = sorted(os.path.join(here, f) for f in os.listdir(here) if f.endswith((".hip", ".h")))
    files.append(os.path.join(os.path.dirname(os.path.dirname(here)), "include", "vneti.h"))
    h = hashlib.sha256()
    for f in files:
        h.update(os.path.basename(f).encode())
        h.update(open(f, "rb").read())
    return h.hexdigest()[:16]


def gemm_cost(f):
    kw = f.keywords
    A, Bm = f.args[0], f.args[1]
    M = kw.get("M") or A.shape[-2]
    N, K = kw.get("N") or Bm.shape[-2], kw.get("K") or Bm.shape[-1]
    batch = kw.get("batch") or 1
    conv = kw.get("conv")
    a_bytes = (M // (conv["Ho"] * conv["Wo"])) * conv["Hi"] * conv["Wi"] * conv["Ci"] * 2 if conv else M * K * 2 * batch
    out = f.args[2]
    c_cols = N * (2 if kw.get("geglu") == 2 else 1)
    extra = sum(M * c * 2 for c, key in ((N, "resid"), (N, "out2"), (c_cols, "gate")) if kw.get(key) is not None)
    if kw.get("geglu") == 1:
        extra -= M * N
    nbytes = a_bytes + N * K * 2 * batch + M * c_cols * out.element_size() * batch + extra
    flops = 2.0 * M * N * K * batch
    return M, N, K, batch, flops, nbytes, flops / (MFMA_PEAK_TFLOPS * 1e12), nbytes / (HBM_PEAK_TBS * 1e12)



def cost(f):
    fn, a, kw = getattr(f, "func", None), getattr(f, "args", ()), getattr(f, "keywords", {}) or {}
    if fn is ops.gemm:
        M, N, K, batch, flops, nbytes, t_mfma, t_hbm = gemm_cost(f)
        if t_hbm > t_mfma:
            return ("gemm, below the ridge (short-K linears: HBM-bound)", 0, nbytes)
        return ("gemm / implicit-GEMM conv (MFMA-bound)", flops, 0)
    if fn in (ops.attn_fwd, ops.attn_bwd_dq, ops.attn_bwd_dkv):
        i = {ops.attn_fwd: 5, ops.attn_bwd_dq: 7, ops.attn_bwd_dkv: 8}[fn]
        Bn, H, Nq, Nk, D = a[i:i + 5]
        causal = a[i + 6]
        mm = {ops.attn_fwd: 2, ops.attn_bwd_dq: 3, ops.attn_bwd_dkv: 4}[fn]
        name = {ops.attn_fwd: "attention fwd", ops.attn_bwd_dq: "attention bwd dQ", ops.attn_bwd_dkv: "attention bwd dK/dV"}[fn]
        scores = Bn * H * Nq * Nk * (0.5 if causal else 1.0)
        ks, db = -(-D // 16), -(-D // 32)
        mfma_c = {ops.attn_fwd: ks + 2 * db, ops.attn_bwd_dq: 2 * ks + 2 * db, ops.attn_bwd_dkv: 2 * ks + 4 * db}[fn] * 32 / 1024.0
        valu_c = {ops.attn_fwd: 2.8, ops.attn_bwd_dq: 4.0, ops.attn_bwd_dkv: 4.0}[fn] * 2 / 64.0 + (2 * 5 / 3) / 64.0
        cob = scores * (mfma_c + valu_c) / (1024 * 2.4e9)
        return (name, mm * 2.0 * scores * D, 0, cob)
    if fn is ops.attn_bwd_small:
        Bn, H, N, D = a[9:13]
        return ("attention bwd (short sequences, one launch)", 7 * 2.0 * Bn * H * N * N * D * (0.5 if a[14] else 1.0), 0)
    if fn in (ops.groupnorm_fwd, ops.groupnorm_fwd_sums, ops.groupnorm_fwd_2l):
        Bn, HW, C = (a[7], a[8], a[9]) if fn is ops.groupnorm_fwd else (a[8], a[9], a[10])
        return ("GroupNorm(+SiLU) fwd" + (" (stats in producer)" if fn is ops.groupnorm_fwd_sums else ""), 0, 2.0 * Bn * HW * C * 2)
    if fn is ops.layernorm_fwd:
        x, y = a[0], a[1]
        return ("LayerNorm fwd", 0, x.numel() * x.element_size() + y.numel() * y.element_size())
    if getattr(f, "vn_cost", None) is not None:
        return (f.vn_cost[0], 0, f.vn_cost[1])
    if getattr(fn, "__name__", "") == "_ln_bwd":
        x = a[0]["x"]
        n = x.numel()
        extra = (a[3].numel() * a[3].element_size() if a[3] is not None else 0) + (n * 2 if len(a) > 4 and a[4] is not None else 0)
        return ("LayerNorm bwd", 0, n * x.element_size() + a[1].numel() * a[1].element_size() + a[2].numel() * a[2].element_size() + extra)
    if fn in (ops.groupnorm_bwd, ops.groupnorm_bwd_2l):
        x = a[1]
        return ("GroupNorm(+SiLU) bwd", 0, 5.0 * x.numel() * 2)
    if fn is ops.add:
        return ("elementwise glue (add, 2x2 sum, transposes, noise, loss)", 0, sum(t.numel() * t.element_size() for t in a[:3]))
    if fn is ops.sum2x2:
        return ("elementwise glue (add, 2x2 sum, transposes, noise, loss)", 0, a[0].numel() * 2 + a[1].numel() * 2)
    if fn in (ops.sample_add_noise, ops.mse_loss_grad, getattr(ops, "transpose", None), getattr(ops, "timestep_embedding", None)):
        return ("elementwise glue (add, 2x2 sum, transposes, noise, loss)", 0,
                sum(t.numel() * t.element_size() for t in a if isinstance(t, torch.Tensor)))
    if fn is ops.layernorm_bwd:
        return ("LayerNorm bwd", 0, sum(t.numel() * t.element_size() for t in (a[0], a[1], a[5])))
    if fn is ops.conv3x3_in:
        return ("VAE conv_in (direct)", 0, a[0].numel() * 4 + a[3].numel() * 2)
    if fn is ops.softmax_rows:
        return ("softmax rows (VAE mid attention)", 0, 2.0 * a[0].numel() * 2)
    if fn is ops.geglu_fwd:
        return ("GEGLU fwd", 0, a[0].numel() * 2 + a[1].numel() * 2)
    if fn is ops.geglu_bwd:
        return ("GEGLU bwd", 0, a[0].numel() * 2 + 2 * a[1].numel() * 2)
    return None




def classify(launches):
    classes = {}
    for f in launches:
        c = cost(f)
        if c is None:
            args = list(getattr(f, "args", ())) + list((getattr(f, "keywords", None) or {}).values())
            c = ("small launches (text path, RNG, layout glue)", 0,
                 float(sum(t.numel() * t.element_size() for t in args if isinstance(t, torch.Tensor))) or 1.0)
        d = classes.setdefault(c[0], dict(fs=[], flops=0.0, bytes=0.0, cob=0.0))
        d["fs"].append(f)
        d["flops"] += c[1]
        d["bytes"] += c[2]
        if len(c) > 3:
            d["cob"] += c[3]
    return classes


def time_classes(launches, classes=None, reps: int = 2):
    classes = classes or classify(launches)
    owner = {id(f): name for name, d in classes.items() for f in d["fs"]}
    tot = {name: 0.0 for name in classes}
    for rep in range(reps + 1):
        evs = []
        for f in launches:
            s, e = torch.cuda.Event(enable_timing=True), torch.cuda.Event(enable_timing=True)
            s.record()
            f()
            e.record()
            evs.append((owner[id(f)], s, e))
        torch.cuda.synchronize()
        if rep:
            for name, s, e in evs:
                tot[name] += s.elapsed_time(e)
    out = {}
    for name, d in classes.items():
        ms = tot[name] / reps
        r = dict(launches=len(d["fs"]), ms_per_step=ms)
        if d["flops"]:
            r.update(bound="mfma", algorithmic_gflop=d["flops"] / 1e9, achieved=d["flops"] / (ms * 1e-3) / 1e12, peak=PF,
                     unit="TFLOP/s")
            r["frac"] = r["achieved"] / PF
            if d.get("cob"):
                r["cobound_frac_of_peak"] = d["flops"] / d["cob"] / 1e12 / PF
                r["frac_of_cobound"] = d["cob"] / (ms * 1e-3)
        elif d["bytes"]:
            r.update(bound="hbm", algorithmic_mb=d["bytes"] / 1e6, achieved=d["bytes"] / (ms * 1e-3) / 1e12, peak=TB,
                     unit="TB/s")
            r["frac"] = r["achieved"] / TB
        out[name] = r
    return out
```

Measured before the change: 40.01 steps/s.

## Fuse GroupNorm backward reductions into the producing GEMM epilogue

Adds an epilogue mode to the GEMM kernels that, while writing the gradient dy, reads the GroupNorm input x and accumulates the per-group backward sums (sum of dxhat and dxhat*xhat, including the SiLU derivative). A new groupnorm_bwd_sums kernel then consumes these precomputed sums, so the GroupNorm backward no longer needs its own reduction pass over dy and x. The engine rewrites eligible producer GEMM plus GN-backward pairs when split-K is 1 and the small-GN path is not used. The cost is an extra read of x in the GEMM epilogue and more register pressure in it.

```diff
diff --git a/include/vneti.h b/include/vneti.h
--- a/include/vneti.h
+++ b/include/vneti.h
@@ -47,6 +47,14 @@
   int gn_hw, gn_cpg, gn_groups, gn_slots;
   int geglu;
   int conv_korder;
+  const void* gnb_x;
+  long long gnb_ldx;
+  const float* gnb_mean;
+  const float* gnb_rstd;
+  const float* gnb_gamma;
+  const float* gnb_beta;
+  int gnb_silu;
+  void* gnb_sums;
 } vneti_gemm_desc;
 
 int vneti_gemm_f16(const vneti_gemm_desc* d, void* stream);
@@ -88,6 +96,11 @@
                            const float* beta, const float* mean, const float* rstd, void* dx, long long lddx,
                            const void* dx_accum, long long ldacc, void* sums, int slots, float* ws, int Bn,
                            int HW, int C, int G, int silu, void* stream);
+int vneti_groupnorm_uses_small(int Bn, int HW, int C, int G, int bwd);
+int vneti_groupnorm_bwd_sums(const void* dy, long long lddy, const void* x, long long ldx, const float* gamma,
+                             const float* beta, const float* mean, const float* rstd, void* dx, long long lddx,
+                             const void* dx_accum, long long ldacc, const void* sums, int slots, int Bn, int HW,
+                             int C, int G, int silu, void* stream);
 int vneti_groupnorm_bwd(const void* dy, long long lddy, const void* x, long long ldx,
                         const float* gamma, const float* beta, const float* mean,
                         const float* rstd, void* dx, long long lddx, const void* dx_accum,
diff --git a/view_neti_amd/csrc/gemm8.hip b/view_neti_amd/csrc/gemm8.hip
--- a/view_neti_amd/csrc/gemm8.hip
+++ b/view_neti_amd/csrc/gemm8.hip
@@ -33,7 +33,7 @@
   const int e_geglu = EPI == 2 ? g.geglu : 0;
   const int e_act = EPI == 2 ? g.act : 0;
   float* const e_gn_sums = EPI >= 1 ? g.gn_sums : nullptr;
-  const half_t* const e_rowadd = EPI >= 1 ? g.rowadd : nullptr;
+  const half_t* const e_rowadd = (EPI == 1 || EPI == 2) ? g.rowadd : nullptr;
   const int e_conv = CONV ? g.conv_mode : 0;
   constexpr int GN_BYTES = EPI == 0 ? 0 : GN_IMG * GN_NG * 4 * 8;
   __shared__ __attribute__((aligned(16))) char smem[LDS_BYTES + GN_BYTES];
@@ -594,7 +594,7 @@
   const half_t* Rb = reinterpret_cast<const half_t*>(g.resid);
   if (Rb) Rb += (long long)bz * g.strideC;
   constexpr int CPR = BN / 8;
-  constexpr int U = EPI == 2 ? 2 : (EPI == 1 ? 4 : (BN == 256 ? 8 : 4));
+  constexpr int U = EPI == 2 ? 2 : ((EPI == 1 || EPI == 3) ? 4 : (BN == 256 ? 8 : 4));
   static_assert(NT % CPR == 0 && CPR <= 32 && (BM * CPR) % NT == 0, "a thread keeps one 8-column chunk over all its rows");
   vn_u64* gacc = reinterpret_cast<vn_u64*>(smem + LDS_BYTES);
   const bool gn = e_gn_sums != nullptr;
@@ -634,11 +634,40 @@
   constexpr int RPP = NT / CPR;
   const bool gn_one = HALO && gn && g.gn_hw == g.Ho * g.Wo;
   const bool ra_one = HALO && EPI >= 1 && e_rowadd && g.rows_per_group == g.Ho * g.Wo;
+  float gb_ga[8], gb_be[8], gb_mlo = 0.f, gb_rlo = 0.f, gb_mhi = 0.f, gb_rhi = 0.f;
+  const __amdgpu_buffer_rsrc_t rsX = vn_make_rsrc(EPI == 3 ? g.gnb_x : nullptr, EPI == 3 ? 0x7fffffffu : 0u);
+  auto gnb_stats = [&](const int img) {
+    if (img >= 0 && n < g.N) {
+      const int si = img * g.gn_G + gn_glo;
+      gb_mlo = g.gnb_mean[si];
+      gb_rlo = g.gnb_rstd[si];
+      if (gn_split < 8) {
+        gb_mhi = g.gnb_mean[si + 1];
+        gb_rhi = g.gnb_rstd[si + 1];
+      }
+    }
+  };
+  if constexpr (EPI == 3) {
+    const bool in_n = n < g.N;
+    const f32x4 z4 = {0.f, 0.f, 0.f, 0.f};
+    const f32x4 ga0 = in_n ? *reinterpret_cast<const f32x4*>(g.gnb_gamma + n) : z4;
+    const f32x4 ga1 = in_n ? *reinterpret_cast<const f32x4*>(g.gnb_gamma + n + 4) : z4;
+    const f32x4 be0 = (in_n && g.gnb_silu) ? *reinterpret_cast<const f32x4*>(g.gnb_beta + n) : z4;
+    const f32x4 be1 = (in_n && g.gnb_silu) ? *reinterpret_cast<const f32x4*>(g.gnb_beta + n + 4) : z4;
+#pragma unroll
+    for (int e = 0; e < 4; ++e) {
+      gb_ga[e] = ga0[e];
+      gb_ga[4 + e] = ga1[e];
+      gb_be[e] = be0[e];
+      gb_be[4 + e] = be1[e];
+    }
+    if (gn_one) gnb_stats(hb);
+  }
   half8 av_tile = half8{0, 0, 0, 0, 0, 0, 0, 0};
   if (ra_one) av_tile = as_half8(vn_buf_load16(rsRA, full_chunk ? (uint32_t)(((long long)hb * g.ld_rowadd + n) * 2) : VN_OOB));
   if (gn_one) gn_img = hb;
   for (int it0 = 0; it0 < BM / RPP; it0 += U) {
-    half8 cv[U], rv[U], av[U], gv[U], gv2[U];
+    half8 cv[U], rv[U], av[U], gv[U], gv2[U], xv[U];
 #pragma unroll
     for (int u = 0; u < U; ++u) {
       const int r = r_first + RPP * (it0 + u);
@@ -658,6 +687,7 @@
           av[u] = as_half8(vn_buf_load16(rsRA, ok ? (uint32_t)(((long long)grp * g.ld_rowadd + n) * 2) : VN_OOB));
         }
       }
+      if constexpr (EPI == 3) xv[u] = as_half8(vn_buf_load16(rsX, ok ? (uint32_t)(((long long)m * g.gnb_ldx + n) * 2) : VN_OOB));
       if (EPI == 2 && e_gate) {
         const long long go = (long long)m * g.ld_gate + (e_geglu == 2 ? 2 * n : n);
         gv[u] = as_half8(vn_buf_load16_once(rsG, ok ? (uint32_t)(go * 2) : VN_OOB));
@@ -679,6 +709,7 @@
         if (__any(img != gn_img)) {
           gn_flush();
           gn_img = img;
+          if constexpr (EPI == 3) gnb_stats(img);
         }
       }
       if (!valid) continue;
@@ -719,7 +750,9 @@
           for (int e = 0; e < 4; ++e) o2[e] = (half_t)((float)v[e] * vn_gelu_erf((float)v[4 + e]));
           *reinterpret_cast<half4*>(e_C2 + (long long)m * g.ldc2 + (n >> 1)) = o2;
         }
-        if (gn) {
+        if constexpr (EPI == 3) {
+          vn_gnb_chunk(v, xv[u], gb_ga, gb_be, g.gnb_silu != 0, gn_split, gb_mlo, gb_rlo, gb_mhi, gb_rhi, s_lo, q_lo, s_hi, q_hi);
+        } else if (gn) {
           {
             const half2v one2 = {(half_t)1.f, (half_t)1.f};
 #pragma unroll
@@ -750,7 +783,7 @@
           if (e_gate) x = (float)(half_t)(x * act_grad((float)e_gate[(long long)m * g.ld_gate + n + e], g.gate_act));
           Cb[(long long)m * g.ldc + n + e] = (half_t)x;
           if (e_C2) e_C2[(long long)m * g.ldc2 + n + e] = (half_t)apply_act((float)(half_t)x, g.act2);
-          if (gn) {
+          if (EPI != 3 && gn) {
             const float xs = (float)(half_t)x;
             if (e < gn_split) {
               s_lo += xs;
@@ -808,6 +841,7 @@
 }
 
 inline int epilogue_level8(const GemmArgs& g) {
+  if (g.gnb_x) return 3;
   if (g.gate_src || g.C2 || g.geglu || g.act) return 2;
   return (g.gn_sums || g.rowadd) ? 1 : 0;
 }
@@ -839,11 +873,11 @@
   } while (0)
 #define VN_GO_HALO(E) hipLaunchKernelGGL((gemm8_kernel<128, E, true, true>), grid, block, 0, st, g)
   if (halo) {
-    if (epi == 2) VN_GO_HALO(2); else if (epi == 1) VN_GO_HALO(1); else VN_GO_HALO(0);
+    if (epi == 3) VN_GO_HALO(3); else if (epi == 2) VN_GO_HALO(2); else if (epi == 1) VN_GO_HALO(1); else VN_GO_HALO(0);
   } else if (g.conv_mode) {
-    if (epi == 2) VN_GO(2, true); else if (epi == 1) VN_GO(1, true); else VN_GO(0, true);
+    if (epi == 3) VN_GO(3, true); else if (epi == 2) VN_GO(2, true); else if (epi == 1) VN_GO(1, true); else VN_GO(0, true);
   } else {
-    if (epi == 2) VN_GO(2, false); else if (epi == 1) VN_GO(1, false); else VN_GO(0, false);
+    if (epi == 3) VN_GO(3, false); else if (epi == 2) VN_GO(2, false); else if (epi == 1) VN_GO(1, false); else VN_GO(0, false);
   }
 #undef VN_GO
 #undef VN_GO_HALO
diff --git a/view_neti_amd/csrc/gemm_args.h b/view_neti_amd/csrc/gemm_args.h
--- a/view_neti_amd/csrc/gemm_args.h
+++ b/view_neti_amd/csrc/gemm_args.h
@@ -32,6 +32,13 @@
   int ldx2;
   int korder;
   int tiles_m, tiles_n;
+  const half_t* gnb_x;
+  long long gnb_ldx;
+  const float* gnb_mean;
+  const float* gnb_rstd;
+  const float* gnb_gamma;
+  const float* gnb_beta;
+  int gnb_silu;
 };
 
 __device__ __forceinline__ float apply_act(float v, int act) {
@@ -53,6 +60,31 @@
   return s * (1.f + f * (1.f - s));
 }
 
+__device__ __forceinline__ void vn_gnb_chunk(const half8 dv, const half8 xv, const float (&ga)[8], const float (&be)[8],
+                                             const bool silu, const int split, const float mlo, const float rlo,
+                                             const float mhi, const float rhi, float& s_lo, float& q_lo, float& s_hi,
+                                             float& q_hi) {
+#pragma unroll
+  for (int e = 0; e < 8; ++e) {
+    const bool lo = e < split;
+    const float xh = ((float)xv[e] - (lo ? mlo : mhi)) * (lo ? rlo : rhi);
+    float d = (float)dv[e];
+    if (silu) {
+      const float z = fmaf(xh, ga[e], be[e]);
+      const float s = vn_sigmoid(z);
+      d *= s * fmaf(z, 1.f - s, 1.f);
+    }
+    const float dxh = d * ga[e];
+    if (lo) {
+      s_lo += dxh;
+      q_lo = fmaf(dxh, xh, q_lo);
+    } else {
+      s_hi += dxh;
+      q_hi = fmaf(dxh, xh, q_hi);
+    }
+  }
+}
+
 __device__ __forceinline__ int lds_off(int row, int chunk) {
   return row * 128 + ((chunk ^ ((row >> 1) & 7)) << 4);
 }
diff --git a/view_neti_amd/csrc/gemm_conv.hip b/view_neti_amd/csrc/gemm_conv.hip
--- a/view_neti_amd/csrc/gemm_conv.hip
+++ b/view_neti_amd/csrc/gemm_conv.hip
@@ -29,7 +29,7 @@
   const int e_geglu = EPI == 2 ? g.geglu : 0;
   const int e_act = EPI == 2 ? g.act : 0;
   float* const e_gn_sums = EPI >= 1 ? g.gn_sums : nullptr;
-  const half_t* const e_rowadd = EPI >= 1 ? g.rowadd : nullptr;
+  const half_t* const e_rowadd = (EPI == 1 || EPI == 2) ? g.rowadd : nullptr;
   const int e_conv = CONV ? g.conv_mode : 0;
   constexpr int NWM = BM / WM, NWN = BN / WN;
   constexpr int NT = NWM * NWN * 64;
@@ -409,6 +409,22 @@
     const int gn_split = gn ? (gn_glo + 1) * g.gn_cpg - gn_c : 8;
     int gn_img = -1;
     float s_lo = 0.f, q_lo = 0.f, s_hi = 0.f, q_hi = 0.f;
+    float gb_ga[8], gb_be[8], gb_mlo = 0.f, gb_rlo = 0.f, gb_mhi = 0.f, gb_rhi = 0.f;
+    if constexpr (EPI == 3) {
+      const bool in_n = gn_c < g.N;
+      const f32x4 z4 = {0.f, 0.f, 0.f, 0.f};
+      const f32x4 ga0 = in_n ? *reinterpret_cast<const f32x4*>(g.gnb_gamma + gn_c) : z4;
+      const f32x4 ga1 = in_n ? *reinterpret_cast<const f32x4*>(g.gnb_gamma + gn_c + 4) : z4;
+      const f32x4 be0 = (in_n && g.gnb_silu) ? *reinterpret_cast<const f32x4*>(g.gnb_beta + gn_c) : z4;
+      const f32x4 be1 = (in_n && g.gnb_silu) ? *reinterpret_cast<const f32x4*>(g.gnb_beta + gn_c + 4) : z4;
+#pragma unroll
+      for (int e = 0; e < 4; ++e) {
+        gb_ga[e] = ga0[e];
+        gb_ga[4 + e] = ga1[e];
+        gb_be[e] = be0[e];
+        gb_be[4 + e] = be1[e];
+      }
+    }
     auto gn_flush = [&]() {
       const int iref = __builtin_amdgcn_readfirstlane(gn_img);
       const bool uni = __all(gn_img == iref) && iref >= 0;
@@ -438,10 +454,23 @@
         if (__any(img != gn_img)) {
           gn_flush();
           gn_img = img;
+          if constexpr (EPI == 3) {
+            if (img >= 0 && n < g.N) {
+              const int si = img * g.gn_G + gn_glo;
+              gb_mlo = g.gnb_mean[si];
+              gb_rlo = g.gnb_rstd[si];
+              if (gn_split < 8) {
+                gb_mhi = g.gnb_mean[si + 1];
+                gb_rhi = g.gnb_rstd[si + 1];
+              }
+            }
+          }
         }
       }
       if (!valid) continue;
       half8 v = as_half8(*reinterpret_cast<const u32x4*>(smem + ((size_t)r * CS_LD + c) * 2));
+      half8 gb_x;
+      if constexpr (EPI == 3) gb_x = *reinterpret_cast<const half8*>(g.gnb_x + (long long)m * g.gnb_ldx + n);
       int ra_rem;
       const half_t* radd = e_rowadd ? e_rowadd + (long long)vn_divmod(m, g.rows_per_group, rcp_rpg, ra_rem) * g.ld_rowadd + n : nullptr;
       if (n + 8 <= g.N) {
@@ -484,7 +513,9 @@
           for (int e = 0; e < 4; ++e) o2[e] = (half_t)((float)v[e] * vn_gelu_erf((float)v[4 + e]));
           *reinterpret_cast<half4*>(e_C2 + (long long)m * g.ldc2 + (n >> 1)) = o2;
         }
-        if (gn) {
+        if constexpr (EPI == 3) {
+          vn_gnb_chunk(v, gb_x, gb_ga, gb_be, g.gnb_silu != 0, gn_split, gb_mlo, gb_rlo, gb_mhi, gb_rhi, s_lo, q_lo, s_hi, q_hi);
+        } else if (gn) {
 #pragma unroll
           for (int e = 0; e < 8; ++e) {
             const float x = (float)v[e];
@@ -511,7 +542,7 @@
           if (e_gate) x = (float)(half_t)(x * act_grad((float)e_gate[(long long)m * g.ld_gate + n + e], g.gate_act));
           Cb[(long long)m * g.ldc + n + e] = (half_t)x;
           if (e_C2) e_C2[(long long)m * g.ldc2 + n + e] = (half_t)apply_act((float)(half_t)x, g.act2);
-          if (gn) {
+          if (EPI != 3 && gn) {
             const float xs = (float)(half_t)x;
             if (e < gn_split) {
               s_lo += xs;
@@ -643,6 +674,7 @@
 }
 
 inline int epilogue_level(const GemmArgs& g) {
+  if (g.gnb_x) return 3;
   if (g.gate_src || g.C2 || g.geglu || g.act) return 2;
   return (g.gn_sums || g.rowadd) ? 1 : 0;
 }
@@ -658,6 +690,11 @@
     else { if (g.act) VN_GO(2, false); else VN_GO(0, false); }
   } else {
     const int epi = epilogue_level(g);
+    constexpr bool GNB = !(BM == 256 && BN == 256);
+    if (epi == 3) {
+      if constexpr (GNB) { if (g.conv_mode) VN_GO(3, true); else VN_GO(3, false); }
+      return;
+    }
     if (g.conv_mode) { if (epi == 2) VN_GO(2, true); else if (epi == 1) VN_GO(1, true); else VN_GO(0, true); }
     else { if (epi == 2) VN_GO(2, false); else if (epi == 1) VN_GO(1, false); else VN_GO(0, false); }
   }
@@ -778,6 +815,16 @@
   g.gn_G = d->gn_groups;
   g.gn_slots = d->gn_slots;
   g.geglu = d->geglu;
+  if (d->gnb_sums) {
+    g.gn_sums = (float*)d->gnb_sums;
+    g.gnb_x = (const half_t*)d->gnb_x;
+    g.gnb_ldx = d->gnb_ldx;
+    g.gnb_mean = d->gnb_mean;
+    g.gnb_rstd = d->gnb_rstd;
+    g.gnb_gamma = d->gnb_gamma;
+    g.gnb_beta = d->gnb_beta;
+    g.gnb_silu = d->gnb_silu ? 1 : 0;
+  }
   g.lda = d->lda;
   g.ldb = d->ldb;
   g.ldc = d->ldc;
@@ -854,7 +901,14 @@
       VN_REQUIRE(d->ldc % 8 == 0, "gemm: geglu backward writes [M][2N]: ldc %% 8");
     }
   }
-  if (d->gn_sums) {
+  if (d->gnb_sums) {
+    VN_REQUIRE(!d->gn_sums && !d->rowadd && !d->gate_src && !d->C2 && !d->geglu && !d->act,
+               "gemm: gnb_sums goes with bias / residual only (no gn_sums, row-add, gate, second output, GEGLU or activation)");
+    VN_REQUIRE(d->gnb_x && d->gnb_mean && d->gnb_rstd && d->gnb_gamma && (d->gnb_beta || !d->gnb_silu) && d->gnb_ldx % 8 == 0,
+               "gemm: gnb_sums needs gnb_x (ld %% 8 == 0), gnb_mean, gnb_rstd, gnb_gamma, and gnb_beta with gnb_silu");
+    VN_REQUIRE(d->N % 8 == 0, "gemm: gnb_sums needs N %% 8 == 0");
+  }
+  if (d->gn_sums || d->gnb_sums) {
     VN_REQUIRE(!f32 && batch == 1, "gemm: gn_sums needs f16 output and batch 1");
     VN_REQUIRE(d->gn_hw >= 64 && d->gn_cpg >= 4 && d->gn_groups > 0 && d->gn_slots > 0 && d->N == d->gn_cpg * d->gn_groups &&
                    d->M % d->gn_hw == 0 && (d->gn_cpg >= 8 || d->gn_cpg == 4),
@@ -877,11 +931,12 @@
   if (cfg == 18 && d->gn_sums && (d->gn_cpg & 1)) cfg = 17;
   if ((cfg == 16 || cfg == 17) && (!dma || (d->conv_mode && (d->ups || (d->conv_mode == 2 && d->stride == 2))) ||
                     (d->gn_sums && (d->gn_cpg & 1)) ||
-                    (d->M >= (1 << 24) && (d->conv_mode || d->rowadd || d->gn_sums)))) cfg = cfg == 16 ? 5 : 7;
+                    (d->M >= (1 << 24) && (d->conv_mode || d->rowadd || d->gn_sums || d->gnb_sums)))) cfg = cfg == 16 ? 5 : 7;
   if ((cfg == 5 || cfg == 16) && f32) cfg = 4;
   if (cfg == 17 && f32) cfg = 7;
   if ((cfg == 6 || cfg == 7) && !dma) cfg = 4;
   if (cfg >= 10 && !dma) cfg = kTiles[cfg].bm == 128 ? (kTiles[cfg].bn == 128 ? 1 : 2) : 3;
+  VN_REQUIRE(!(d->gnb_sums && cfg == 5), "gemm: gnb_sums is not available in the 256x256 generic tile (tile_hint 5)");
   long long ws_floats = d->workspace ? d->workspace_bytes / 4 : 0;
   int ks = d->split_k;
   if (ks == 0) ks = select_ksplit(d->M, d->N, d->K, batch, cfg, ws_floats);
diff --git a/view_neti_amd/csrc/norms.hip b/view_neti_amd/csrc/norms.hip
--- a/view_neti_amd/csrc/norms.hip
+++ b/view_neti_amd/csrc/norms.hip
@@ -924,6 +924,36 @@
   return vneti_check_launch("groupnorm_bwd_2l");
 }
 
+extern "C" int vneti_groupnorm_uses_small(int Bn, int HW, int C, int G, int bwd) {
+  GNGeom g;
+  return gn_geom(g, Bn, HW, C, G) == 0 && gn_use_small(Bn, HW, C, G, bwd != 0) ? 1 : 0;
+}
+
+extern "C" int vneti_groupnorm_bwd_sums(const void* dy, long long lddy, const void* x, long long ldx, const float* gamma,
+                                        const float* beta, const float* mean, const float* rstd, void* dx, long long lddx,
+                                        const void* dx_accum, long long ldacc, const void* sums_v, int slots, int Bn,
+                                        int HW, int C, int G, int silu, void* stream) {
+  const float* sums = reinterpret_cast<const float*>(sums_v);
+  GNGeom g;
+  VN_REQUIRE(gn_geom(g, Bn, HW, C, G) == 0, "groupnorm: unsupported shape B=%d HW=%d C=%d G=%d", Bn, HW, C, G);
+  VN_REQUIRE(dy && x && gamma && beta && mean && rstd && dx && sums && slots > 0, "groupnorm_bwd_sums: null pointer");
+  VN_REQUIRE(ldx % 8 == 0 && lddy % 8 == 0 && lddx % 8 == 0 && ldacc % 8 == 0, "groupnorm_bwd_sums: ld % 8 != 0");
+  VN_REQUIRE_OUT("groupnorm_bwd_sums", vn_out_bytes((long long)Bn * HW, lddx, C, 2));
+  hipStream_t st = (hipStream_t)stream;
+  dim3 grid(g.nslab, Bn);
+#define GN_BWD_SUMS(S)                                                                                                   \
+  hipLaunchKernelGGL((gn_apply_kernel<true, S, true>), grid, dim3(256), 0, st, g, (const half_t*)x, ldx, (const half_t*)dy, \
+                     lddy, gamma, beta, mean, rstd, (const float*)nullptr, (const float*)nullptr, (half_t*)dx, lddx,      \
+                     (const half_t*)dx_accum, ldacc, sums, slots, 0.f, (float*)nullptr, (float*)nullptr)
+  if (silu) {
+    GN_BWD_SUMS(true);
+  } else {
+    GN_BWD_SUMS(false);
+  }
+#undef GN_BWD_SUMS
+  return vneti_check_launch("groupnorm_bwd_sums");
+}
+
 extern "C" int vneti_layernorm_fwd(const void* x, int x_is_f32, long long ldx, void* y, long long ldy,
                                    const float* gamma, const float* beta, float* mean, float* rstd, int rows,
                                    int C, float eps, void* stream) {
diff --git a/view_neti_amd/engine/schedule.py b/view_neti_amd/engine/schedule.py
--- a/view_neti_amd/engine/schedule.py
+++ b/view_neti_amd/engine/schedule.py
@@ -47,6 +47,7 @@
         self._side_stream = None
         self._gn_fusable: List[dict] = []
         self.gn_sums = None
+        self.gn_bwd_fused = 0
         if ops._default_ws is None or ops._default_ws.device != torch.device(device, torch.cuda.current_device()):
             ops.set_default_gemm_workspace(torch.empty(16 * 2 ** 20, dtype=torch.float32, device=device))
 
@@ -268,6 +269,7 @@
 
     def fuse_gn_stats(self, fuse: bool = True):
         n = self._fuse_gn_stats() if fuse else 0
+        self.gn_bwd_fused = self._fuse_gn_bwd_stats() if fuse else 0
         if getattr(self, "_gn2_used", 0):
             self.fwd.insert(0, self._gn2_arena[:self._gn2_used].zero_)
         return n
@@ -316,6 +318,53 @@
         self.fwd.insert(0, arena.zero_)
         self._gn_fusable = []
         return len(todo)
+
+    def _fuse_gn_bwd_stats(self):
+        import os
+        if os.environ.get("VNETI_NO_GN_BWD_FUSE") or os.environ.get("VNETI_GN_BWD_FUSE") != "1":
+            return 0
+        S, G, B = self.GN_SLOTS, self.groups, self.B
+        n = 0
+        for idx, p in enumerate(self.bwd):
+            info = getattr(getattr(p, "func", None), "vn_gnb", None)
+            if info is None or info["prod"] is None:
+                continue
+            rec, dy = info["rec"], info["dy"]
+            f = self.bwd[info["prod"]]
+            if getattr(f, "func", None) is not ops.gemm or f.args[2] is not dy:
+                continue
+            kw = f.keywords
+            x, hw = rec["x"], rec["hw"]
+            Cc = x.cols
+            cpg = Cc // G
+            if kw.get("batch") or kw.get("act") or kw.get("geglu") or dy.dtype == torch.float32 or \
+                    any(kw.get(k) is not None for k in ("rowadd", "gate", "out2", "gn_sums", "gnb")):
+                continue
+            if (kw.get("tile_hint") or 0) % 100 == 5:
+                continue
+            sk = kw.get("split_k") or 0
+            if sk > 1:
+                continue
+            if sk == 0:
+                M_, N_, K_ = self._gemm_key(f)[:3]
+                ws = kw.get("workspace")
+                wsb = ws.numel() * ws.element_size() if ws is not None else 0
+                if ops.gemm_select_split(M_, N_, K_, 1, kw.get("tile_hint") or 0, wsb) != 1:
+                    continue
+            if hw < 64 or not (cpg >= 8 or cpg == 4) or Cc % 8 or ops.groupnorm_uses_small(B, hw, Cc, G, True):
+                continue
+            kw = dict(kw)
+            kw.update(split_k=1, gnb=dict(x=x.v, mean=rec["mean"], rstd=rec["rstd"], gamma=rec["gamma"], beta=rec["beta"],
+                                          silu=rec["silu"], sums=rec["bsums"], hw=hw, groups=G, slots=S))
+            self.bwd[info["prod"]] = self._rebound(f, ops.gemm, kw)
+            out, accum = p.args
+            q = partial(ops.groupnorm_bwd_sums, dy, x.v, rec["gamma"], rec["beta"], rec["mean"], rec["rstd"], out,
+                        rec["bsums"], S, B, hw, Cc, G, rec["silu"], accum=accum)
+            if getattr(p, "side", False):
+                q.side = True
+            self.bwd[idx] = q
+            n += 1
+        return n
 
     def _gn(self, x: T, name, w, eps, silu):
         Cc = x.cols
@@ -338,7 +387,7 @@
                                          eps=eps, silu=silu))
         return y, rec
 
-    def _gn_bwd_fn(self, rec, dy):
+    def _gn_bwd_fn(self, rec, dy, prod=None):
         x = rec["x"]
         if "bsums" not in rec:
             fn = lambda out, accum: ops.groupnorm_bwd(dy, x.v, rec["gamma"], rec["beta"], rec["mean"], rec["rstd"], out,
@@ -348,6 +397,7 @@
             fn = lambda out, accum: ops.groupnorm_bwd_2l(dy, x.v, rec["gamma"], rec["beta"], rec["mean"], rec["rstd"], out,
                                                          rec["bsums"], self.GN_SLOTS, self.gn_ws, self.B, rec["hw"], x.cols,
                                                          self.groups, rec["silu"], accum=accum)
+            fn.vn_gnb = dict(rec=rec, dy=dy, prod=prod)
         fn.vn_cost = ("GroupNorm(+SiLU) bwd", 5.0 * self.B * rec["hw"] * x.cols * 2)
         return fn
 
@@ -405,15 +455,16 @@
         self.bwd.append(partial(ops.gemm, dout, r["w2d"], dn2, M=M,
                                 conv=self._conv_desc(h, wd, cout, h, wd, 1, 1, 0, dout.stride(0), mode=2)))
         dh1 = self._tmp("dB", M, cout)
-        self.bwd.append(partial(self._gn_bwd_fn(r["gn2"], dn2), dh1, None))
+        self.bwd.append(partial(self._gn_bwd_fn(r["gn2"], dn2, len(self.bwd) - 1), dh1, None))
         dn1 = self._tmp("dC", M, cin)
         self.bwd.append(partial(ops.gemm, dh1, r["w1d"], dn1, M=M,
                                 conv=self._conv_desc(h, wd, cout, h, wd, 1, 1, 0, cout, mode=2)))
+        prod = len(self.bwd) - 1
         if "wscd" in r:
             self._contrib_gemm(x, dout, r["wscd"])
-            self._contrib(x, self._gn_bwd_fn(r["gn1"], dn1))
+            self._contrib(x, self._gn_bwd_fn(r["gn1"], dn1, prod))
         else:
-            self._contrib(x, self._gn_bwd_fn(r["gn1"], dn1), extra=dout)
+            self._contrib(x, self._gn_bwd_fn(r["gn1"], dn1, prod), extra=dout)
 
     def _ln(self, xv, name, w):
         rows, Cc = xv.shape
diff --git a/view_neti_amd/engine/unet.py b/view_neti_amd/engine/unet.py
--- a/view_neti_amd/engine/unet.py
+++ b/view_neti_amd/engine/unet.py
@@ -241,7 +241,7 @@
         bw.append(partial(self._ln_bwd, r["ln1"], dn1, dh0, dh1))
         dg = self._tmp("tA", M, Cc)
         bw.append(partial(ops.gemm, dh0, r["w_ind"], dg))
-        self._contrib(x, self._gn_bwd_fn(r["gn"], dg), extra=dout)
+        self._contrib(x, self._gn_bwd_fn(r["gn"], dg, len(bw) - 1), extra=dout)
 
     def _upsample(self, x: T, Cc, name, w, out_view, h, wd):
         M = x.rows * 4
@@ -391,7 +391,7 @@
                                 self.W, 1, 1, 1, (self.H * self.W * ld, 1, self.W * ld, ld)))
         dn = self._tmp("dA", M0, x.cols)
         self.bwd.append(partial(ops.gemm, col, r["wd_"], dn))
-        self._contrib(x, self._gn_bwd_fn(r["gn"], dn))
+        self._contrib(x, self._gn_bwd_fn(r["gn"], dn, len(self.bwd) - 1))
 
     def _build_backward(self):
         for r in reversed(self.tape):
diff --git a/view_neti_amd/lib.py b/view_neti_amd/lib.py
--- a/view_neti_amd/lib.py
+++ b/view_neti_amd/lib.py
@@ -104,7 +104,7 @@
 SIGNATURES = {n[len("vneti_"):]: argtypes for n, (_, argtypes) in _PROTOS.items()}
 VALUE_FUNCS = frozenset({
     "version", "precision", "last_error", "gemm_select_tile", "gemm_select_split", "img_resample_ksize",
-    "groupnorm_ws_floats", "lpips_ws_floats", "mapper_num_params", "mapper_save_floats", "mapper_rowgrad_floats",
+    "groupnorm_ws_floats", "groupnorm_uses_small", "lpips_ws_floats", "mapper_num_params", "mapper_save_floats", "mapper_rowgrad_floats",
     "mapper_legacy_input_params"})
 _stray = ({n[len("vneti_"):] for n, (res, _) in _PROTOS.items() if res is C.c_longlong} - VALUE_FUNCS) | (VALUE_FUNCS - set(SIGNATURES))
 if _stray:
diff --git a/view_neti_amd/ops.py b/view_neti_amd/ops.py
--- a/view_neti_amd/ops.py
+++ b/view_neti_amd/ops.py
@@ -35,7 +35,7 @@
 def gemm(A, B, out, *, bias=None, rowadd=None, rows_per_group=1, resid=None, alpha=1.0, act=0,
          tile_hint=0, batch=0, strideA=0, strideB=0, strideC=0, M=None, N=None, K=None, conv=None,
          lda=None, ldc=None, workspace=None, split_k=0, gate=None, gate_act=0, out2=None, act2=0,
-         gn_sums=None, gn_hw=0, gn_groups=0, gn_slots=0, geglu=0):
+         gn_sums=None, gn_hw=0, gn_groups=0, gn_slots=0, geglu=0, gnb=None):
     d = _l.GemmDesc()
     d.A, d.B, d.C = _p(A), _p(B), _p(out)
     d.ldb = _ld(B)
@@ -72,6 +72,11 @@
     if gn_sums is not None:
         d.gn_sums, d.gn_hw, d.gn_groups, d.gn_slots = _p(gn_sums), gn_hw, gn_groups, gn_slots
         d.gn_cpg = d.N // gn_groups
+    if gnb is not None:
+        d.gnb_x, d.gnb_ldx, d.gnb_mean, d.gnb_rstd = _p(gnb["x"]), _ld(gnb["x"]), _p(gnb["mean"]), _p(gnb["rstd"])
+        d.gnb_gamma, d.gnb_beta, d.gnb_silu, d.gnb_sums = _p(gnb["gamma"]), _p(gnb["beta"]), 1 if gnb["silu"] else 0, _p(gnb["sums"])
+        d.gn_hw, d.gn_groups, d.gn_slots = gnb["hw"], gnb["groups"], gnb["slots"]
+        d.gn_cpg = d.N // gnb["groups"]
     d.geglu = geglu
     ws = workspace if workspace is not None else _default_ws
     if ws is not None:
@@ -114,6 +119,10 @@
     return n
 
 
+def groupnorm_uses_small(Bn, HW, Cc, G, bwd):
+    return bool(_l.query("groupnorm_uses_small", Bn, HW, Cc, G, 1 if bwd else 0))
+
+
 def groupnorm_fwd(x, y, gamma, beta, mean, rstd, ws, Bn, HW, Cc, G, eps, silu):
     _l.call("groupnorm_fwd", _p(x), _ld(x), _p(y), _ld(y), _p(gamma), _p(beta), _p(mean), _p(rstd), _p(ws),
             Bn, HW, Cc, G, eps, 1 if silu else 0, stream())
@@ -132,6 +141,12 @@
 def groupnorm_bwd_2l(dy, x, gamma, beta, mean, rstd, dx, sums, slots, ws, Bn, HW, Cc, G, silu, accum=None):
     _l.call("groupnorm_bwd_2l", _p(dy), _ld(dy), _p(x), _ld(x), _p(gamma), _p(beta), _p(mean), _p(rstd),
             _p(dx), _ld(dx), _p(accum), _ld(accum) if accum is not None else 0, _p(sums), slots, _p(ws),
+            Bn, HW, Cc, G, 1 if silu else 0, stream())
+
+
+def groupnorm_bwd_sums(dy, x, gamma, beta, mean, rstd, dx, sums, slots, Bn, HW, Cc, G, silu, accum=None):
+    _l.call("groupnorm_bwd_sums", _p(dy), _ld(dy), _p(x), _ld(x), _p(gamma), _p(beta), _p(mean), _p(rstd),
+            _p(dx), _ld(dx), _p(accum), _ld(accum) if accum is not None else 0, _p(sums), slots,
             Bn, HW, Cc, G, 1 if silu else 0, stream())
 
 
diff --git a/view_neti_amd/roofline.py b/view_neti_amd/roofline.py
--- a/view_neti_amd/roofline.py
+++ b/view_neti_amd/roofline.py
@@ -38,6 +38,8 @@
     extra = sum(M * c * 2 for c, key in ((N, "resid"), (N, "out2"), (c_cols, "gate")) if kw.get(key) is not None)
     if kw.get("geglu") == 1:
         extra -= M * N
+    if kw.get("gnb") is not None:
+        extra += M * N * 2
     nbytes = a_bytes + N * K * 2 * batch + M * c_cols * out.element_size() * batch + extra
     flops = 2.0 * M * N * K * batch
     return M, N, K, batch, flops, nbytes, flops / (MFMA_PEAK_TFLOPS * 1e12), nbytes / (HBM_PEAK_TBS * 1e12)
@@ -79,6 +81,8 @@
         n = x.numel()
         extra = (a[3].numel() * a[3].element_size() if a[3] is not None else 0) + (n * 2 if len(a) > 4 and a[4] is not None else 0)
         return ("LayerNorm bwd", 0, n * x.element_size() + a[1].numel() * a[1].element_size() + a[2].numel() * a[2].element_size() + extra)
+    if fn is ops.groupnorm_bwd_sums:
+        return ("GroupNorm(+SiLU) bwd (stats in producer)", 0, 3.0 * a[1].numel() * 2)
     if fn in (ops.groupnorm_bwd, ops.groupnorm_bwd_2l):
         x = a[1]
         return ("GroupNorm(+SiLU) bwd", 0, 5.0 * x.numel() * 2)
```

Measured after the change: 40.05 steps/s, median of 3. No clear change (+0.1%).
